# OpenRobotLab/EmbodiedScan

Measured on NVIDIA H100. Metric: training scans/sec mv-3ddet 20-view (ResNet-50/16 + MinkResNet34, 480x640, 100k pts), higher is better.
Workload: dtype bf16

## Files before the change

### embodiedscan_b200/_ffi.py

```python
import ctypes
import os

import torch

_HERE = os.path.dirname(os.path.abspath(__file__))
LIB_PATH = os.path.join(_HERE, 'libesb200.so')

_CT = {'p': ctypes.c_void_p, 'q': ctypes.c_longlong, 'i': ctypes.c_int, 'f': ctypes.c_float, 'z': ctypes.c_size_t}

SIGNATURES = {
    'esb_last_error': ('', 'p'),
    'esb_voxelize_points': ('pqiifpp', 'i'),
    'esb_hash_capacity': ('q', 'q'),
    'esb_coord_unique_workspace_bytes': ('q', 'z'),
    'esb_coord_unique': ('pqippqppppzp', 'i'),
    'esb_hash_build': ('pqppqp', 'i'),
    'esb_hash_lookup': ('pqppqpp', 'i'),
    'esb_interp_features': ('pqppqpiiipp', 'i'),
    'esb_kernel_map': ('pqpippqpp', 'i'),
    'esb_kernel_map_transpose': ('piqqpp', 'i'),
    'esb_kmap_pairs_workspace_bytes': ('iq', 'z'),
    'esb_kmap_pairs': ('piqppppzp', 'i'),
    'esb_generative_children': ('pqipp', 'i'),
    'esb_spconv_fwd': ('ppppqiiiiip', 'i'),
    'esb_spconv_wgrad': ('ppppppqiiiip', 'i'),
    'esb_kmap_tile_masks': ('piqpp', 'i'),
    'esb_spconv_tc_fwd': ('pppppqiiiip', 'i'),
    'esb_spconv_tc_wgrad': ('ppppppqiiip', 'i'),
    'esb_maxpool_fwd': ('ppppqiiip', 'i'),
    'esb_maxpool_bwd': ('pppqiip', 'i'),
    'esb_norm_fwd': ('ppppiqiippfppfipppip', 'i'),
    'esb_batchnorm_fwd_fused': ('ppqippfppfippip', 'i'),
    'esb_norm_apply': ('pppqippppipip', 'i'),
    'esb_norm_bwd': ('pppppiqiipppippppiip', 'i'),
    'esb_bias_act_fwd': ('ppppqiiip', 'i'),
    'esb_act_bwd': ('pppqiip', 'i'),
    'esb_gather2_rows': ('ppqpppqiip', 'i'),
    'esb_conv2d_tma_fwd': ('ppppp' + 'iiiiiiiiii' + 'p', 'i'),
    'esb_conv2d_tma_wgrad': ('ppp' + 'iiiiiiiii' + 'p', 'i'),
    'esb_conv2d_tma_dgrad': ('ppp' + 'iiiiiiiii' + 'p', 'i'),
    'esb_conv3d_tma_fwd': ('ppppp' + 'iiiiiiiiii' + 'p', 'i'),
    'esb_conv3d_tma_dgrad': ('ppp' + 'iiiiiiiii' + 'p', 'i'),
    'esb_conv3d_tma_wgrad': ('ppp' + 'iiiiiiiii' + 'p', 'i'),
    'esb_stem7x7_tc': ('pppp' + 'iiii' + 'p', 'i'),
    'esb_conv2d_direct_fwd': ('ppppp' + 'iiiiiiiiiii' + 'p', 'i'),
    'esb_conv2d_direct_dgrad': ('ppp' + 'iiiiiiiiii' + 'p', 'i'),
    'esb_conv2d_direct_wgrad': ('ppp' + 'iiiiiiiiii' + 'p', 'i'),
    'esb_maxpool2d_nhwc': ('pp' + 'iiiiiiii' + 'p', 'i'),
    'esb_attn_fwd': ('pppppp' + 'iiii' + 'f' + 'p', 'i'),
    'esb_attn_bwd': ('ppppppppppp' + 'iiii' + 'f' + 'p', 'i'),
    'esb_paint_meta_bytes': ('', 'i'),
    'esb_paint_fwd': ('pppqfppipiiiffppip', 'i'),
    'esb_paint_bwd': ('pppqfppipiiiffpip', 'i'),
    'esb_fcaf3d_targets_workspace_bytes': ('iii', 'z'),
    'esb_fcaf3d_targets': ('ppiippppp' + 'iiiii' + 'pppp' + 'pzp', 'i'),
    'esb_focal_loss_fwd': ('ppqiffppip', 'i'),
    'esb_focal_loss_bwd': ('ppqiffpppip', 'i'),
    'esb_bbox_cd_loss': ('pppppippp', 'i'),
    'esb_nms_bev_segmented': ('ppiifipp', 'i'),
    'esb_iou_bev_pairwise': ('pipiipp', 'i'),
    'esb_box3d_overlap': ('pipippp', 'i'),
    'esb_hungarian_batch': ('ppiiippp', 'i'),
    'esb_img_normalize': ('piiiiippiipip', 'i'),
    'esb_unproject_depth_workspace_bytes': ('iii', 'z'),
    'esb_unproject_depth': ('piiifpppppzp', 'i'),
    'esb_grad_clip_coef': ('pqffpp', 'i'),
    'esb_adamw_step': ('pppppqfffffifpp', 'i'),
    'esb_cast_f32_to_bf16': ('ppqp', 'i'),
}

_lib = None

KERNELS_PER_CALL = {
    'esb_voxelize_points': 1, 'esb_coord_unique': 6, 'esb_hash_build': 2, 'esb_hash_lookup': 1, 'esb_kernel_map': 1,
    'esb_kernel_map_transpose': 2, 'esb_kmap_pairs': 3, 'esb_generative_children': 1, 'esb_spconv_fwd': 1,
    'esb_spconv_wgrad': 1, 'esb_maxpool_fwd': 1, 'esb_maxpool_bwd': 1, 'esb_norm_fwd': 5, 'esb_norm_apply': 1,
    'esb_norm_bwd': 2, 'esb_batchnorm_fwd_fused': 2, 'esb_paint_fwd': 1, 'esb_paint_bwd': 1, 'esb_fcaf3d_targets': 5,
    'esb_focal_loss_fwd': 1, 'esb_focal_loss_bwd': 1, 'esb_nms_bev_segmented': 1, 'esb_iou_bev_pairwise': 1,
    'esb_img_normalize': 1, 'esb_unproject_depth': 3, 'esb_grad_clip_coef': 2, 'esb_adamw_step': 1,
    'esb_cast_f32_to_bf16': 1, 'esb_spconv_tc_fwd': 1, 'esb_spconv_tc_wgrad': 1, 'esb_kmap_tile_masks': 1,
}
launch_counter = {'kernels': 0, 'calls': 0, 'by_name': {}}


def exported_symbols():
    return list(SIGNATURES.keys())


def lib():
    global _lib
    if _lib is None:
        if not os.path.exists(LIB_PATH):
            raise RuntimeError(
                f'{LIB_PATH} is missing: run `python -c "import __graft_entry__ as g; g.build()"` '
                '(esb200 has no CPU fallback)')
        handle = ctypes.CDLL(LIB_PATH)
        for name, (args, ret) in SIGNATURES.items():
            fn = getattr(handle, name)
            fn.argtypes = [_CT[c] for c in args]
            fn.restype = _CT[ret]
        _lib = handle
    return _lib


def last_error():
    p = lib().esb_last_error()
    return ctypes.cast(p, ctypes.c_char_p).value.decode() if p else ''


def ptr(t):
    if t is None:
        return None
    return t.data_ptr()


def stream():
    return torch._C._cuda_getCurrentRawStream(torch._C._cuda_getDevice())


def call(name, *args):
    launch_counter['calls'] += 1
    launch_counter['kernels'] += KERNELS_PER_CALL.get(name, 1)
    launch_counter['by_name'][name] = launch_counter['by_name'].get(name, 0) + 1
    rc = getattr(lib(), name)(*args)
    if rc != 0:
        raise RuntimeError(f'{name} failed ({rc}): {last_error()}')


def query(name, *args):
    return getattr(lib(), name)(*args)


def dtype_code(dtype):
    if dtype == torch.float32:
        return 0
    if dtype == torch.bfloat16:
        return 1
    raise TypeError(f'esb200 kernels take float32 or bfloat16 features, got {dtype}')
```

### embodiedscan_b200/csrc/attn_tc.cu

```cuda
#include "tc_common.cuh"

using namespace esb_tc;

namespace {

constexpr int AT_D = 32;
constexpr int AT_CONS = 256;
constexpr int AT_THREADS = AT_CONS + 32;
constexpr float LOG2E = 1.4426950408889634f;

__device__ __forceinline__ uint32_t swz128(uint32_t row, uint32_t piece) { return row * 128u + ((piece ^ (row & 7u)) << 4); }
__device__ __forceinline__ uint32_t tile_off(int row, int col) {
  return (uint32_t)(col >> 6) * 16384u + swz128((uint32_t)row, (uint32_t)((col & 63) >> 3)) + (uint32_t)(col & 7) * 2u;
}

__global__ void __launch_bounds__(AT_THREADS, 1)
attn_fwd_kernel(const __grid_constant__ CUtensorMap tmq, const __grid_constant__ CUtensorMap tmk,
                const __grid_constant__ CUtensorMap tmv, const unsigned char* __restrict__ key_pad,
                __nv_bfloat16* __restrict__ o, float* __restrict__ lse, int H, int Lq, int Lk, float scale) {
  extern __shared__ __align__(1024) uint8_t smem_raw[];
  uint8_t* smem = (uint8_t*)(((uintptr_t)smem_raw + 1023) & ~(uintptr_t)1023);
  uint8_t* q_s = smem;
  uint8_t* k_s = smem + 8192;
  uint8_t* v_s = smem + 8192 * 3;
  uint8_t* p_s = smem + 8192 * 5;
  uint64_t* bars = (uint64_t*)(p_s + 32768);
  uint64_t *q_full = bars, *kv_full = bars + 1, *kv_empty = bars + 3;

  const int warp = threadIdx.x >> 5, lane = threadIdx.x & 31;
  const int bh = blockIdx.y, b = bh / H;
  const int q0 = blockIdx.x * 128;
  const int n_kt = (Lk + 127) / 128;

  if (threadIdx.x == 0) {
    mbar_init(q_full, 1);
    for (int s = 0; s < 2; ++s) { mbar_init(&kv_full[s], 1); mbar_init(&kv_empty[s], AT_CONS / 32); }
    asm volatile("fence.mbarrier_init.release.cluster;" ::: "memory");
    tma_prefetch_desc(&tmq); tma_prefetch_desc(&tmk); tma_prefetch_desc(&tmv);
  }
  __syncthreads();

  if (threadIdx.x >= AT_CONS) {
    if (lane == 0) {
      mbar_expect_tx(q_full, 8192);
      tma_load_2d(&tmq, q_full, smem_u32(q_s), 0, bh * Lq + q0);
      for (int j = 0; j < n_kt; ++j) {
        const int s = j & 1;
        mbar_wait(&kv_empty[s], ((j >> 1) & 1) ^ 1);
        mbar_expect_tx(&kv_full[s], 16384);
        tma_load_2d(&tmk, &kv_full[s], smem_u32(k_s + s * 8192), 0, bh * Lk + j * 128);
        tma_load_2d(&tmv, &kv_full[s], smem_u32(v_s + s * 8192), 0, bh * Lk + j * 128);
      }
    }
    return;
  }
  const int wg = threadIdx.x >> 7;
  const int ra = wg * 64 + 16 * (warp & 3) + (lane >> 2);
  const int cq = 2 * (lane & 3);
  const float sc2 = scale * LOG2E;
  float m[2] = {-INFINITY, -INFINITY}, l[2] = {0.f, 0.f};
  float acc[AT_D / 2], sacc[64], oacc[AT_D / 2];
#pragma unroll
  for (int e = 0; e < AT_D / 2; ++e) acc[e] = 0.f;
  mbar_wait(q_full, 0);
  const uint32_t qa = smem_u32(q_s) + wg * 4096, pa = smem_u32(p_s) + wg * 8192;
  for (int j = 0; j < n_kt; ++j) {
    const int s = j & 1;
    mbar_wait(&kv_full[s], (j >> 1) & 1);
    const uint32_t ka = smem_u32(k_s + s * 8192), va = smem_u32(v_s + s * 8192);
    wgmma_fence();
#pragma unroll
    for (int kk = 0; kk < 2; ++kk)
      wgmma_bf16<128, 0, 0>(sacc, make_desc_sw(qa + kk * 32, 16, 512, SW64), make_desc_sw(ka + kk * 32, 16, 512, SW64), kk > 0);
    wgmma_commit();
    wgmma_wait<0>();
    acc_fence<64>(sacc);
    uint32_t dead = 0;
#pragma unroll
    for (int jb = 0; jb < 16; ++jb)
#pragma unroll
      for (int u = 0; u < 2; ++u) {
        const int kj = j * 128 + 8 * jb + cq + u;
        if (kj >= Lk || (key_pad != nullptr && key_pad[(long long)b * Lk + kj])) dead |= 1u << (2 * jb + u);
      }
    float alpha[2], m_use[2];
#pragma unroll
    for (int h = 0; h < 2; ++h) {
      float mx = m[h];
#pragma unroll
      for (int jb = 0; jb < 16; ++jb)
#pragma unroll
        for (int u = 0; u < 2; ++u)
          if (!((dead >> (2 * jb + u)) & 1)) mx = fmaxf(mx, sacc[4 * jb + 2 * h + u] * sc2);
      mx = fmaxf(mx, __shfl_xor_sync(0xffffffffu, mx, 1));
      mx = fmaxf(mx, __shfl_xor_sync(0xffffffffu, mx, 2));
      m_use[h] = mx == -INFINITY ? 0.f : mx;
      alpha[h] = exp2f(m[h] - m_use[h]);
      m[h] = mx;
    }
    float rs[2] = {0.f, 0.f};
#pragma unroll
    for (int jb = 0; jb < 16; ++jb)
#pragma unroll
      for (int h = 0; h < 2; ++h) {
        const float p0 = ((dead >> (2 * jb)) & 1) ? 0.f : exp2f(sacc[4 * jb + 2 * h] * sc2 - m_use[h]);
        const float p1 = ((dead >> (2 * jb + 1)) & 1) ? 0.f : exp2f(sacc[4 * jb + 2 * h + 1] * sc2 - m_use[h]);
        rs[h] += p0 + p1;
        *reinterpret_cast<uint32_t*>(p_s + tile_off(ra + 8 * h, 8 * jb + cq)) = pack_bf16(__float_as_uint(p0), __float_as_uint(p1));
      }
#pragma unroll
    for (int h = 0; h < 2; ++h) l[h] = l[h] * alpha[h] + rs[h];
    fence_proxy_async();
    asm volatile("bar.sync %0, 128;" ::"r"(1 + wg) : "memory");
    wgmma_fence();
#pragma unroll
    for (int kk = 0; kk < 8; ++kk)
      wgmma_bf16<AT_D, 0, 1>(oacc, make_desc_sw(pa + (kk >> 2) * 16384 + (kk & 3) * 32, 16, 1024, SW128),
                             make_desc_sw(va + kk * 1024, 2048, 512, SW64), kk > 0);
    wgmma_commit();
    wgmma_wait<0>();
    acc_fence<AT_D / 2>(oacc);
    if (lane == 0) mbar_arrive(&kv_empty[s]);
#pragma unroll
    for (int e = 0; e < AT_D / 2; ++e) acc[e] = acc[e] * alpha[(e >> 1) & 1] + oacc[e];
  }
#pragma unroll
  for (int h = 0; h < 2; ++h) {
    l[h] += __shfl_xor_sync(0xffffffffu, l[h], 1);
    l[h] += __shfl_xor_sync(0xffffffffu, l[h], 2);
    const int qi = q0 + ra + 8 * h;
    if (qi < Lq) {
      const float inv = l[h] > 0.f ? 1.f / l[h] : 0.f;
      __nv_bfloat16* dst = o + ((long long)bh * Lq + qi) * AT_D;
#pragma unroll
      for (int jb = 0; jb < AT_D / 8; ++jb)
        *reinterpret_cast<uint32_t*>(dst + 8 * jb + cq) =
            pack_bf16(__float_as_uint(acc[4 * jb + 2 * h] * inv), __float_as_uint(acc[4 * jb + 2 * h + 1] * inv));
      if ((lane & 3) == 0) lse[(long long)bh * Lq + qi] = l[h] > 0.f ? (m[h] + log2f(l[h])) * 0.6931471805599453f : -INFINITY;
    }
  }
}

__global__ void attn_delta_kernel(const __nv_bfloat16* __restrict__ o, const __nv_bfloat16* __restrict__ dout,
                                  float* __restrict__ delta, long long rows) {
  const long long i = (long long)blockIdx.x * blockDim.x + threadIdx.x;
  if (i >= rows) return;
  float s = 0.f;
  const uint4* a = reinterpret_cast<const uint4*>(o + i * AT_D);
  const uint4* g = reinterpret_cast<const uint4*>(dout + i * AT_D);
#pragma unroll
  for (int h = 0; h < 4; ++h) {
    const uint4 x = a[h], y = g[h];
    const __nv_bfloat162* xp = reinterpret_cast<const __nv_bfloat162*>(&x);
    const __nv_bfloat162* yp = reinterpret_cast<const __nv_bfloat162*>(&y);
#pragma unroll
    for (int e = 0; e < 4; ++e) {
      const float2 xf = __bfloat1622float2(xp[e]), yf = __bfloat1622float2(yp[e]);
      s = fmaf(xf.x, yf.x, s);
      s = fmaf(xf.y, yf.y, s);
    }
  }
  delta[i] = s;
}

__global__ void __launch_bounds__(AT_THREADS, 1)
attn_bwd_kernel(const __grid_constant__ CUtensorMap tmq, const __grid_constant__ CUtensorMap tmk,
                const __grid_constant__ CUtensorMap tmv, const __grid_constant__ CUtensorMap tmdo,
                const unsigned char* __restrict__ key_pad, const float* __restrict__ lse, const float* __restrict__ delta,
                float* __restrict__ dq, __nv_bfloat16* __restrict__ dk, __nv_bfloat16* __restrict__ dv, int H, int Lq, int Lk,
                float scale) {
  extern __shared__ __align__(1024) uint8_t smem_raw[];
  uint8_t* smem = (uint8_t*)(((uintptr_t)smem_raw + 1023) & ~(uintptr_t)1023);
  uint8_t* k_s = smem;
  uint8_t* v_s = smem + 8192;
  uint8_t* q_s = smem + 16384;
  uint8_t* do_s = smem + 32768;
  uint8_t* pt_s = smem + 49152;
  uint8_t* ds_s = smem + 49152 + 32768;
  float* lse2_all = (float*)(smem + 49152 + 65536);
  float* delta_all = lse2_all + 256;
  uint64_t* bars = (uint64_t*)(delta_all + 256);
  uint64_t *kv_full = bars, *qd_full = bars + 1, *qd_empty = bars + 3;

  const int warp = threadIdx.x >> 5, lane = threadIdx.x & 31;
  const int bh = blockIdx.y, b = bh / H;
  const int k0 = blockIdx.x * 128;
  const int n_qt = (Lq + 127) / 128;

  if (threadIdx.x == 0) {
    mbar_init(kv_full, 1);
    for (int s = 0; s < 2; ++s) { mbar_init(&qd_full[s], 1); mbar_init(&qd_empty[s], AT_CONS / 32); }
    asm volatile("fence.mbarrier_init.release.cluster;" ::: "memory");
    tma_prefetch_desc(&tmq); tma_prefetch_desc(&tmk); tma_prefetch_desc(&tmv); tma_prefetch_desc(&tmdo);
  }
  __syncthreads();

  if (threadIdx.x >= AT_CONS) {
    if (lane == 0) {
      mbar_expect_tx(kv_full, 16384);
      tma_load_2d(&tmk, kv_full, smem_u32(k_s), 0, bh * Lk + k0);
      tma_load_2d(&tmv, kv_full, smem_u32(v_s), 0, bh * Lk + k0);
      for (int i = 0; i < n_qt; ++i) {
        const int s = i & 1;
        mbar_wait(&qd_empty[s], ((i >> 1) & 1) ^ 1);
        mbar_expect_tx(&qd_full[s], 16384);
        tma_load_2d(&tmq, &qd_full[s], smem_u32(q_s + s * 8192), 0, bh * Lq + i * 128);
        tma_load_2d(&tmdo, &qd_full[s], smem_u32(do_s + s * 8192), 0, bh * Lq + i * 128);
      }
    }
    return;
  }
  const int t = threadIdx.x, wg = t >> 7;
  const int ra = wg * 64 + 16 * (warp & 3) + (lane >> 2);
  const int cq = 2 * (lane & 3);
  bool k_dead[2];
#pragma unroll
  for (int h = 0; h < 2; ++h) {
    const int kj = k0 + ra + 8 * h;
    k_dead[h] = kj >= Lk || (key_pad != nullptr && key_pad[(long long)b * Lk + kj]);
  }
  const float sc2 = scale * LOG2E;
  float sacc[64], pacc[64], dvacc[AT_D / 2], dkacc[AT_D / 2], dqacc[AT_D / 2];
  const uint32_t ka = smem_u32(k_s), va = smem_u32(v_s), pa = smem_u32(pt_s), sa = smem_u32(ds_s);
  mbar_wait(kv_full, 0);
  for (int i = 0; i < n_qt; ++i) {
    const int s = i & 1;
    float* lse2_s = lse2_all + (i & 1) * 128;
    float* delta_s = delta_all + (i & 1) * 128;
    if (t < 128) {
      const int qi = i * 128 + t;
      lse2_s[t] = qi < Lq ? lse[(long long)bh * Lq + qi] * LOG2E : INFINITY;
      delta_s[t] = qi < Lq ? delta[(long long)bh * Lq + qi] : 0.f;
    }
    asm volatile("bar.sync 1, %0;" ::"n"(AT_CONS) : "memory");
    mbar_wait(&qd_full[s], (i >> 1) & 1);
    const uint32_t qa = smem_u32(q_s + s * 8192), da = smem_u32(do_s + s * 8192);
    wgmma_fence();
#pragma unroll
    for (int kk = 0; kk < 2; ++kk)
      wgmma_bf16<128, 0, 0>(sacc, make_desc_sw(ka + wg * 4096 + kk * 32, 16, 512, SW64), make_desc_sw(qa + kk * 32, 16, 512, SW64),
                            kk > 0);
#pragma unroll
    for (int kk = 0; kk < 2; ++kk)
      wgmma_bf16<128, 0, 0>(pacc, make_desc_sw(va + wg * 4096 + kk * 32, 16, 512, SW64), make_desc_sw(da + kk * 32, 16, 512, SW64),
                            kk > 0);
    wgmma_commit();
    wgmma_wait<0>();
    acc_fence<64>(sacc);
    acc_fence<64>(pacc);
#pragma unroll
    for (int jb = 0; jb < 16; ++jb)
#pragma unroll
      for (int h = 0; h < 2; ++h) {
        float p[2], ds[2];
#pragma unroll
        for (int u = 0; u < 2; ++u) {
          const int c = 8 * jb + cq + u, e = 4 * jb + 2 * h + u;
          const float ex = k_dead[h] ? 0.f : exp2f(sacc[e] * sc2 - lse2_s[c]);
          p[u] = ex;
          ds[u] = ex * (pacc[e] - delta_s[c]) * scale;
        }
        const uint32_t off = tile_off(ra + 8 * h, 8 * jb + cq);
        *reinterpret_cast<uint32_t*>(pt_s + off) = pack_bf16(__float_as_uint(p[0]), __float_as_uint(p[1]));
        *reinterpret_cast<uint32_t*>(ds_s + off) = pack_bf16(__float_as_uint(ds[0]), __float_as_uint(ds[1]));
      }
    fence_proxy_async();
    asm volatile("bar.sync 1, %0;" ::"n"(AT_CONS) : "memory");
    wgmma_fence();
#pragma unroll
    for (int kk = 0; kk < 8; ++kk) {
      const uint32_t a_off = wg * 8192 + (kk >> 2) * 16384 + (kk & 3) * 32;
      wgmma_bf16<AT_D, 0, 1>(dvacc, make_desc_sw(pa + a_off, 16, 1024, SW128), make_desc_sw(da + kk * 1024, 2048, 512, SW64),
                             i > 0 || kk > 0);
      wgmma_bf16<AT_D, 0, 1>(dkacc, make_desc_sw(sa + a_off, 16, 1024, SW128), make_desc_sw(qa + kk * 1024, 2048, 512, SW64),
                             i > 0 || kk > 0);
    }
#pragma unroll
    for (int kk = 0; kk < 8; ++kk)
      wgmma_bf16<AT_D, 1, 1>(dqacc, make_desc_sw(sa + wg * 16384 + kk * 2048, 16384, 1024, SW128),
                             make_desc_sw(ka + kk * 1024, 2048, 512, SW64), kk > 0);
    wgmma_commit();
    wgmma_wait<0>();
    acc_fence<AT_D / 2>(dvacc);
    acc_fence<AT_D / 2>(dkacc);
    acc_fence<AT_D / 2>(dqacc);
    if (lane == 0) mbar_arrive(&qd_empty[s]);
#pragma unroll
    for (int h = 0; h < 2; ++h) {
      const int qi = i * 128 + ra + 8 * h;
      if (qi < Lq) {
        float* dst = dq + (((long long)blockIdx.x * gridDim.y + bh) * Lq + qi) * AT_D;
#pragma unroll
        for (int jb = 0; jb < AT_D / 8; ++jb)
          *reinterpret_cast<float2*>(dst + 8 * jb + cq) = make_float2(dqacc[4 * jb + 2 * h], dqacc[4 * jb + 2 * h + 1]);
      }
    }
  }
#pragma unroll
  for (int h = 0; h < 2; ++h) {
    const int kj = k0 + ra + 8 * h;
    if (kj < Lk) {
      __nv_bfloat16* pv = dv + ((long long)bh * Lk + kj) * AT_D;
      __nv_bfloat16* pk = dk + ((long long)bh * Lk + kj) * AT_D;
#pragma unroll
      for (int jb = 0; jb < AT_D / 8; ++jb) {
        *reinterpret_cast<uint32_t*>(pv + 8 * jb + cq) =
            pack_bf16(__float_as_uint(dvacc[4 * jb + 2 * h]), __float_as_uint(dvacc[4 * jb + 2 * h + 1]));
        *reinterpret_cast<uint32_t*>(pk + 8 * jb + cq) =
            pack_bf16(__float_as_uint(dkacc[4 * jb + 2 * h]), __float_as_uint(dkacc[4 * jb + 2 * h + 1]));
      }
    }
  }
}

int rows32_map(CUtensorMap* tm, const void* base, long long rows) {
  unsigned long long dims[2] = {AT_D, (unsigned long long)(rows > 0 ? rows : 1)};
  unsigned long long str[1] = {AT_D * 2};
  unsigned box[2] = {AT_D, 128};
  return esb_tma_encode(tm, base, 2, dims, str, box, nullptr, 64);
}

}

extern "C" int esb_attn_fwd(const void* q, const void* k, const void* v, const unsigned char* key_pad, void* o, float* lse, int B,
                            int H, int Lq, int Lk, float scale, void* stream_) {
  ESB_CHECK_ARG(B > 0 && H > 0 && Lq > 0 && Lk > 0, "esb_attn_fwd: empty problem");
  CUtensorMap tmq, tmk, tmv;
  int rc = rows32_map(&tmq, q, (long long)B * H * Lq);
  if (rc == ESB_OK) rc = rows32_map(&tmk, k, (long long)B * H * Lk);
  if (rc == ESB_OK) rc = rows32_map(&tmv, v, (long long)B * H * Lk);
  if (rc != ESB_OK) return rc;
  const size_t smem = 8192 * 5 + 32768 + 8 * 8 + 1024;
  cudaError_t e = cudaFuncSetAttribute(attn_fwd_kernel, cudaFuncAttributeMaxDynamicSharedMemorySize, (int)smem);
  if (e != cudaSuccess) { esb_set_error("esb_attn_fwd: smem attr: %s", cudaGetErrorString(e)); return ESB_ECUDA; }
  dim3 grid((Lq + 127) / 128, B * H);
  attn_fwd_kernel<<<grid, AT_THREADS, smem, (cudaStream_t)stream_>>>(tmq, tmk, tmv, key_pad, (__nv_bfloat16*)o, lse, H, Lq, Lk, scale);
  ESB_CUDA_LAUNCH_CHECK("attn_fwd_kernel");
  return ESB_OK;
}

extern "C" int esb_attn_bwd(const void* q, const void* k, const void* v, const unsigned char* key_pad, const void* o,
                            const void* dout, const float* lse, float* delta, float* dq, void* dk, void* dv, int B, int H, int Lq,
                            int Lk, float scale, void* stream_) {
  cudaStream_t stream = (cudaStream_t)stream_;
  ESB_CHECK_ARG(B > 0 && H > 0 && Lq > 0 && Lk > 0, "esb_attn_bwd: empty problem");
  CUtensorMap tmq, tmk, tmv, tmdo;
  int rc = rows32_map(&tmq, q, (long long)B * H * Lq);
  if (rc == ESB_OK) rc = rows32_map(&tmk, k, (long long)B * H * Lk);
  if (rc == ESB_OK) rc = rows32_map(&tmv, v, (long long)B * H * Lk);
  if (rc == ESB_OK) rc = rows32_map(&tmdo, dout, (long long)B * H * Lq);
  if (rc != ESB_OK) return rc;
  const long long rows = (long long)B * H * Lq;
  attn_delta_kernel<<<esb_div_up(rows, 256), 256, 0, stream>>>((const __nv_bfloat16*)o, (const __nv_bfloat16*)dout, delta, rows);
  ESB_CUDA_LAUNCH_CHECK("attn_delta_kernel");
  const size_t smem = 49152 + 65536 + 2048 + 8 * 8 + 1024;
  cudaError_t e = cudaFuncSetAttribute(attn_bwd_kernel, cudaFuncAttributeMaxDynamicSharedMemorySize, (int)smem);
  if (e != cudaSuccess) { esb_set_error("esb_attn_bwd: smem attr: %s", cudaGetErrorString(e)); return ESB_ECUDA; }
  dim3 grid((Lk + 127) / 128, B * H);
  const long long width = rows * AT_D;
  float* part = nullptr;
  ESB_CUDA_CALL(esb_scratch_alloc((void**)&part, sizeof(float) * grid.x * width, stream));
  attn_bwd_kernel<<<grid, AT_THREADS, smem, stream>>>(tmq, tmk, tmv, tmdo, key_pad, lse, delta, part, (__nv_bfloat16*)dk,
                                                      (__nv_bfloat16*)dv, H, Lq, Lk, scale);
  ESB_CUDA_LAUNCH_CHECK("attn_bwd_kernel");
  rc = esb_sum_partial_rows(part, (int)grid.x, width, dq, 1, stream);
  ESB_CUDA_CALL(esb_scratch_free(part, stream));
  return rc;
}
```

### embodiedscan_b200/csrc/common.cuh

```cuda
#pragma once
#include <cuda_runtime.h>
#include <cuda_bf16.h>
#include <stdint.h>
#include <stdio.h>
#include <stdarg.h>
#include "../../include/esb200.h"

void esb_set_error(const char* fmt, ...);

#define ESB_CHECK_ARG(cond, ...)                      \
  do {                                                \
    if (!(cond)) {                                    \
      esb_set_error(__VA_ARGS__);                     \
      return ESB_EINVAL;                              \
    }                                                 \
  } while (0)

#define ESB_CUDA_LAUNCH_CHECK(name)                                        \
  do {                                                                     \
    cudaError_t _e = cudaPeekAtLastError();                                \
    if (_e != cudaSuccess) {                                               \
      esb_set_error("%s: CUDA error %s", name, cudaGetErrorString(_e));    \
      return ESB_ECUDA;                                                    \
    }                                                                      \
  } while (0)

#define ESB_CUDA_CALL(expr)                                                \
  do {                                                                     \
    cudaError_t _e = (expr);                                               \
    if (_e != cudaSuccess) {                                               \
      esb_set_error("%s: CUDA error %s", #expr, cudaGetErrorString(_e));   \
      return ESB_ECUDA;                                                    \
    }                                                                      \
  } while (0)

static inline int esb_div_up(long long a, long long b) { return (int)((a + b - 1) / b); }
static inline size_t esb_align(size_t x, size_t a = 256) { return (x + a - 1) / a * a; }
cudaError_t esb_scratch_alloc(void** p, size_t bytes, cudaStream_t s);
cudaError_t esb_scratch_free(void* p, cudaStream_t s);
int esb_sum_partial_rows(const float* part, int n_parts, long long width, float* out, int accumulate, cudaStream_t s);

int esb_sm_count();


#define ESB_EMPTY_KEY 0xFFFFFFFFFFFFFFFFull
#define ESB_COORD_BIAS 32768

__host__ __device__ __forceinline__ uint64_t esb_pack_key(int b, int x, int y, int z) {
  return ((uint64_t)(uint16_t)b << 48) | ((uint64_t)(uint16_t)(x + ESB_COORD_BIAS) << 32) |
         ((uint64_t)(uint16_t)(y + ESB_COORD_BIAS) << 16) | (uint64_t)(uint16_t)(z + ESB_COORD_BIAS);
}
__host__ __device__ __forceinline__ bool esb_coord_in_range(int b, int x, int y, int z) {
  return b >= 0 && b < 65535 && x >= -ESB_COORD_BIAS && x < ESB_COORD_BIAS && y >= -ESB_COORD_BIAS &&
         y < ESB_COORD_BIAS && z >= -ESB_COORD_BIAS && z < ESB_COORD_BIAS;
}
__host__ __device__ __forceinline__ uint32_t esb_hash64(uint64_t k) {
  k ^= k >> 33;
  k *= 0xff51afd7ed558ccdull;
  k ^= k >> 33;
  k *= 0xc4ceb9fe1a85ec53ull;
  k ^= k >> 33;
  return (uint32_t)k;
}

#ifdef __CUDACC__
__device__ __forceinline__ int esb_floor_div(int a, int d) {
  int q = a / d;
  return (a % d != 0 && a < 0) ? q - 1 : q;
}

__device__ __forceinline__ int esb_hash_find(const unsigned long long* __restrict__ keys,
                                             const int* __restrict__ vals, uint32_t mask, uint64_t key) {
  uint32_t slot = esb_hash64(key) & mask;
  for (uint32_t probe = 0; probe <= mask; ++probe) {
    unsigned long long k = keys[slot];
    if (k == key) return vals[slot];
    if (k == ESB_EMPTY_KEY) return -1;
    slot = (slot + 1) & mask;
  }
  return -1;
}

template <typename T>
__device__ __forceinline__ float esb_to_float(T v);
template <>
__device__ __forceinline__ float esb_to_float<float>(float v) { return v; }
template <>
__device__ __forceinline__ float esb_to_float<__nv_bfloat16>(__nv_bfloat16 v) { return __bfloat162float(v); }

template <typename T>
__device__ __forceinline__ T esb_from_float(float v);
template <>
__device__ __forceinline__ float esb_from_float<float>(float v) { return v; }
template <>
__device__ __forceinline__ __nv_bfloat16 esb_from_float<__nv_bfloat16>(float v) { return __float2bfloat16_rn(v); }

__device__ __forceinline__ float esb_warp_sum(float v) {
#pragma unroll
  for (int o = 16; o > 0; o >>= 1) v += __shfl_xor_sync(0xffffffffu, v, o);
  return v;
}
__device__ __forceinline__ float esb_warp_max(float v) {
#pragma unroll
  for (int o = 16; o > 0; o >>= 1) v = fmaxf(v, __shfl_xor_sync(0xffffffffu, v, o));
  return v;
}
#endif
```

### embodiedscan_b200/csrc/conv_tma.cu

```cuda
#include "tc_common.cuh"

using namespace esb_tc;

namespace {

struct ConvGeom {
  int tiles_w, tiles_h, tiles_d, tiles_n, n_blocks;
  int TW, TH, TD, TN;
  int Wo, Ho, Do, N;
  int stride;
  int cin, bc, nchunk, group;
  int cout, relu;
  int stages;
  int ntaps;
  short tap_dx[27], tap_dy[27], tap_dz[27], tap_w[27];
};

constexpr int EPI_THREADS = 128;
constexpr int NCONS = 256;
constexpr int PROD0 = NCONS, EPI0 = NCONS + 32;
constexpr int THREADS = EPI0 + EPI_THREADS;

__device__ __forceinline__ uint32_t swz(uint32_t off, uint32_t mask) { return off ^ (((off >> 7) & mask) << 4); }

// ... 399 lines not shown

extern "C" int esb_conv2d_tma_dgrad(const void* dy, const void* w_ohwi, void* dx, int n_img, int H, int W, int cin, int cout,
                                    int kh, int kw, int stride, int pad, void* stream_) {
  return conv_dgrad_any("esb_conv2d_tma_dgrad", dy, w_ohwi, dx, n_img, 1, H, W, cin, cout, 1, kh, kw, stride, pad,
                        (cudaStream_t)stream_);
}

extern "C" int esb_conv3d_tma_dgrad(const void* dy, const void* w_odhwi, void* dx, int n, int D, int H, int W, int cin, int cout,
                                    int k, int stride, int pad, void* stream_) {
  return conv_dgrad_any("esb_conv3d_tma_dgrad", dy, w_odhwi, dx, n, D, H, W, cin, cout, k, k, k, stride, pad,
                        (cudaStream_t)stream_);
}

namespace {

constexpr int ST_TW = 16, ST_TH = 8;
constexpr int ST_PW = 112, ST_PH = 2 * ST_TH + 5;
constexpr int ST_K = 147, ST_KPAD = 160;

__global__ void __launch_bounds__(128)
stem7x7_tc_kernel(const __nv_bfloat16* __restrict__ x, const __nv_bfloat16* __restrict__ w, const float* __restrict__ bias,
                  __nv_bfloat16* __restrict__ y, int n_img, int H, int W, int Ho, int Wo, int relu) {
  extern __shared__ __align__(1024) uint8_t smem_raw[];
  uint8_t* smem = (uint8_t*)(((uintptr_t)smem_raw + 1023) & ~(uintptr_t)1023);
  uint8_t* a_tile = smem;
  uint8_t* b_tile = smem + 3 * 16384;
  __nv_bfloat16* patch = (__nv_bfloat16*)(b_tile + 3 * 2048);
  float* acc_img = reinterpret_cast<float*>(a_tile);
  constexpr int PITCH = 20;

  const int t = threadIdx.x;
  for (int i = t; i < 16 * 24; i += 128) {
    const int n = i / 24, j = i - n * 24;
    uint32_t v[4] = {0u, 0u, 0u, 0u};
    __nv_bfloat16* vp = reinterpret_cast<__nv_bfloat16*>(v);
    for (int e = 0; e < 8; ++e) {
      const int k = j * 8 + e;
      if (k < ST_K) vp[e] = w[n * ST_K + k];
    }
    const int c = j >> 3, jj = j & 7;
    *reinterpret_cast<uint4*>(b_tile + c * 2048 + n * 128 + ((jj ^ (n & 7)) << 4)) = make_uint4(v[0], v[1], v[2], v[3]);
  }
  __syncthreads();

  const int tiles_w = (Wo + ST_TW - 1) / ST_TW, tiles_h = (Ho + ST_TH - 1) / ST_TH;
  const int n_tiles = tiles_w * tiles_h * n_img;
  const int tx = t & 15, ty = t >> 4;
  for (int tile = blockIdx.x; tile < n_tiles; tile += gridDim.x) {
    int r = tile;
    const int twi = r % tiles_w; r /= tiles_w;
    const int thi = r % tiles_h;
    const int img = r / tiles_h;
    const int ox0 = twi * ST_TW, oy0 = thi * ST_TH;
    const int g0 = (2 * ox0 - 3) * 3 - 1;
    const __nv_bfloat16* ximg = x + (long long)img * H * W * 3;
    for (int i = t; i < ST_PH * (ST_PW / 2); i += 128) {
      const int pr = i / (ST_PW / 2), pw = i - pr * (ST_PW / 2);
      const int iy = 2 * oy0 - 3 + pr, g = g0 + 2 * pw;
      uint32_t v = 0u;
      if (iy >= 0 && iy < H && g >= 0 && g + 1 < W * 3) v = *reinterpret_cast<const uint32_t*>(ximg + (long long)iy * W * 3 + g);
      reinterpret_cast<uint32_t*>(patch)[pr * (ST_PW / 2) + pw] = v;
    }
    __syncthreads();
    {
      const __nv_bfloat16* base = patch + (2 * ty) * ST_PW + 6 * tx + 1;
      const uint32_t row_off = (uint32_t)((t >> 3) * 1024 + (t & 7) * 128);
#pragma unroll
      for (int j = 0; j < ST_KPAD / 8; ++j) {
        uint32_t v[4];
#pragma unroll
        for (int h = 0; h < 4; ++h) {
          const int k0 = j * 8 + 2 * h, k1 = k0 + 1;
          const uint32_t lo = k0 < ST_K ? (uint32_t)__bfloat16_as_ushort(base[(k0 / 21) * ST_PW + (k0 % 21)]) : 0u;
          const uint32_t hi = k1 < ST_K ? (uint32_t)__bfloat16_as_ushort(base[(k1 / 21) * ST_PW + (k1 % 21)]) : 0u;
          v[h] = lo | (hi << 16);
        }
        const int c = j >> 3, jj = j & 7;
        *reinterpret_cast<uint4*>(a_tile + c * 16384 + row_off + ((jj ^ (t & 7)) << 4)) = make_uint4(v[0], v[1], v[2], v[3]);
      }
    }
    fence_proxy_async();
    __syncthreads();
    {
      const uint32_t a_addr = smem_u32(a_tile), b_addr = smem_u32(b_tile);
      float acc[2][8];
      wgmma_fence();
#pragma unroll
      for (int h = 0; h < 2; ++h)
#pragma unroll
        for (int kk = 0; kk < ST_KPAD / 16; ++kk)
          wgmma_bf16<16, 0, 0>(acc[h], make_desc(a_addr + h * 8192 + (kk >> 2) * 16384 + (kk & 3) * 32, 16, 1024),
                               make_desc(b_addr + (kk >> 2) * 2048 + (kk & 3) * 32, 16, 1024), kk > 0);
      wgmma_commit();
      wgmma_wait<0>();
      acc_fence<8>(acc[0]);
      acc_fence<8>(acc[1]);
      __syncthreads();
      acc_store<16>(acc[0], acc_img, PITCH, 0, t);
      acc_store<16>(acc[1], acc_img, PITCH, 64, t);
      __syncthreads();
    }
    uint32_t v[32];
    img_ld<16>(acc_img, PITCH, t, 0, v);
    const int ox = ox0 + tx, oy = oy0 + ty;
    if (ox < Wo && oy < Ho) {
      uint32_t o[8];
#pragma unroll
      for (int h = 0; h < 8; ++h) {
        float f0 = __uint_as_float(v[2 * h]) + bias[2 * h], f1 = __uint_as_float(v[2 * h + 1]) + bias[2 * h + 1];
        if (relu) { f0 = fmaxf(f0, 0.f); f1 = fmaxf(f1, 0.f); }
        o[h] = pack_bf16(__float_as_uint(f0), __float_as_uint(f1));
      }
      uint4* dst = reinterpret_cast<uint4*>(y + (((long long)img * Ho + oy) * Wo + ox) * 16);
      dst[0] = make_uint4(o[0], o[1], o[2], o[3]);
      dst[1] = make_uint4(o[4], o[5], o[6], o[7]);
    }
    __syncthreads();
  }
}

}

extern "C" int esb_stem7x7_tc(const void* x, const void* w_ohwi, const float* bias, void* y, int n_img, int H, int W, int relu,
                              void* stream_) {
  ESB_CHECK_ARG(n_img >= 0 && H > 0 && W > 0 && (W * 3) % 2 == 0, "esb_stem7x7_tc: W*3 must be even (4-byte patch loads)");
  ESB_CHECK_ARG(bias != nullptr, "esb_stem7x7_tc: bias (16 fp32) is required");
  if (n_img == 0) return ESB_OK;
  const int Ho = (H + 6 - 7) / 2 + 1, Wo = (W + 6 - 7) / 2 + 1;
  const size_t smem = 3 * 16384 + 3 * 2048 + ((ST_PH * ST_PW * 2 + 15) & ~15) + 1024;
  cudaError_t e = cudaFuncSetAttribute(stem7x7_tc_kernel, cudaFuncAttributeMaxDynamicSharedMemorySize, (int)smem);
  if (e != cudaSuccess) { esb_set_error("esb_stem7x7_tc: smem attr: %s", cudaGetErrorString(e)); return ESB_ECUDA; }
  const long long n_tiles = (long long)esb_div_up(Wo, ST_TW) * esb_div_up(Ho, ST_TH) * n_img;
  long long grid = (long long)esb_sm_count() * 3;
  if (grid > n_tiles) grid = n_tiles;
  stem7x7_tc_kernel<<<(unsigned)grid, 128, smem, (cudaStream_t)stream_>>>(
      (const __nv_bfloat16*)x, (const __nv_bfloat16*)w_ohwi, bias, (__nv_bfloat16*)y, n_img, H, W, Ho, Wo, relu);
  ESB_CUDA_LAUNCH_CHECK("stem7x7_tc_kernel");
  return ESB_OK;
}

namespace {

struct WgradGeom {
  int tiles_w, tiles_h, tiles_d, tiles_n;
  int TW, TH, TD, TN;
  int kd, kh, kw, stride, sd, pad, pd;
  int cin, cout, aw, atoms_per_slice, chunks_per_tap;
  int stages, tiles_per_cta;
};

template <int N_TILE>
__global__ void __launch_bounds__(THREADS, 1)
conv_tma_wgrad_kernel(const __grid_constant__ CUtensorMap tmx, const __grid_constant__ CUtensorMap tmdy,
                      float* __restrict__ dw, const WgradGeom g) {
  constexpr int NA = N_TILE < 64 ? N_TILE : 64;
  constexpr int A_BYTES = 64 * 256;
  constexpr int B_BYTES = 64 * N_TILE * 2;
  constexpr int STAGE_BYTES = A_BYTES + B_BYTES;
  constexpr int PITCH = N_TILE + 4;
  extern __shared__ __align__(1024) uint8_t smem_raw[];
  uint8_t* smem = (uint8_t*)(((uintptr_t)smem_raw + 1023) & ~(uintptr_t)1023);
  const int STAGES = g.stages;
  uint64_t* full_bar = (uint64_t*)(smem + STAGES * STAGE_BYTES);
  uint64_t* empty_bar = full_bar + STAGES;
  uint64_t* accum_bar = empty_bar + STAGES;
  float* img = reinterpret_cast<float*>(smem);

  const int lane = threadIdx.x & 31;
  const int taps = g.kd * g.kh * g.kw;
  const int n_tiles = g.tiles_w * g.tiles_h * g.tiles_d * g.tiles_n;
  const int t_beg = blockIdx.x * g.tiles_per_cta;
  const int t_end = min(n_tiles, t_beg + g.tiles_per_cta);
  if (t_beg >= n_tiles) return;
  const int total = t_end - t_beg;
  const int slice = blockIdx.y, co0 = blockIdx.z * N_TILE;
  const int awb = g.aw * 2;
  const int atom0 = slice * g.atoms_per_slice;
  const int n_atoms_total = taps * g.chunks_per_tap;
  const int n_valid = min(g.atoms_per_slice, n_atoms_total - atom0);
  const uint32_t a_atom_bytes = 64u * awb;

  if (threadIdx.x == 0) {
    for (int s = 0; s < STAGES; ++s) {
      mbar_init(&full_bar[s], 1);
      mbar_init(&empty_bar[s], NCONS / 32);
    }
    mbar_init(accum_bar, NCONS);
    asm volatile("fence.mbarrier_init.release.cluster;" ::: "memory");
    tma_prefetch_desc(&tmx);
    tma_prefetch_desc(&tmdy);
  }
  __syncthreads();

  if (threadIdx.x >= PROD0 && threadIdx.x < EPI0) {
    if (lane == 0) {
      for (int it = 0; it < total; ++it) {
        int t = t_beg + it;
        const int tw = t % g.tiles_w; t /= g.tiles_w;
        const int th = t % g.tiles_h; t /= g.tiles_h;
        const int td = t % g.tiles_d; t /= g.tiles_d;
        const int ox0 = tw * g.TW, oy0 = th * g.TH, oz0 = td * g.TD, img0 = t * g.TN;
        const int s = it % STAGES;
        mbar_wait(&empty_bar[s], ((it / STAGES) & 1) ^ 1);
        mbar_expect_tx(&full_bar[s], (uint32_t)n_valid * a_atom_bytes + B_BYTES);
        const uint32_t a_base = smem_u32(smem + s * STAGE_BYTES);
        const uint32_t b_base = a_base + A_BYTES;
        for (int a = 0; a < n_valid; ++a) {
          const int ga = atom0 + a;
          const int tap = ga / g.chunks_per_tap, ch0 = (ga - tap * g.chunks_per_tap) * g.aw;
          const int kz = tap / (g.kh * g.kw), kr = tap - kz * (g.kh * g.kw);
          const int ky = kr / g.kw, kx = kr - ky * g.kw;
          tma_load_5d(&tmx, &full_bar[s], a_base + a * a_atom_bytes, ch0, ox0 * g.stride - g.pad + kx, oy0 * g.stride - g.pad + ky,
                      oz0 * g.sd - g.pd + kz, img0);
        }
#pragma unroll
        for (int b = 0; b < N_TILE / NA; ++b)
          tma_load_5d(&tmdy, &full_bar[s], b_base + b * (64 * NA * 2), co0 + b * NA, ox0, oy0, oz0, img0);
      }
    }
  } else if (threadIdx.x < NCONS) {
    const int wg = threadIdx.x >> 7;
    const uint32_t a_layout = mma_layout_of(awb), b_layout = mma_layout_of(NA * 2);
    float acc[N_TILE / 2];
    for (int it = 0; it < total; ++it) {
      const int s = it % STAGES;
      mbar_wait(&full_bar[s], (it / STAGES) & 1);
      const uint32_t a_addr = smem_u32(smem + s * STAGE_BYTES) + wg * (64 / g.aw) * a_atom_bytes;
      const uint32_t b_addr = smem_u32(smem + s * STAGE_BYTES) + A_BYTES;
      wgmma_fence();
#pragma unroll
      for (int kk = 0; kk < 4; ++kk)
        wgmma_bf16<N_TILE, 1, 1>(acc, make_desc_sw(a_addr + kk * 16 * awb, a_atom_bytes, 8 * awb, a_layout),
                                 make_desc_sw(b_addr + kk * 16 * (NA * 2), 64 * NA * 2, 8 * (NA * 2), b_layout), it > 0 || kk > 0);
      wgmma_commit();
      wgmma_wait<1>();
      if (it > 0 && lane == 0) mbar_arrive(&empty_bar[(it - 1) % STAGES]);
    }
    wgmma_wait<0>();
    acc_fence<N_TILE / 2>(acc);
    asm volatile("bar.sync 2, %0;" ::"n"(NCONS) : "memory");
    acc_store<N_TILE>(acc, img, PITCH, wg * 64, threadIdx.x & 127);
    mbar_arrive(accum_bar);
  } else {
    const int quad = (threadIdx.x - EPI0) >> 5;
    mbar_wait(accum_bar, 0);
    const float* stg = img;
    const int rows_valid = n_valid * g.aw;
    for (int rr = 0; rr < 32; ++rr) {
      const int r = quad * 32 + rr;
      if (r >= rows_valid) break;
      const int ga = atom0 + r / g.aw;
      const int tap = ga / g.chunks_per_tap, ch = (ga - tap * g.chunks_per_tap) * g.aw + (r % g.aw);
      float* dwrow = dw + (((long long)blockIdx.x * g.kd * g.kh * g.kw + tap) * g.cin + ch) * g.cout + co0;
      for (int c = lane * 4; c < N_TILE; c += 128)
        *reinterpret_cast<float4*>(dwrow + c) = *reinterpret_cast<const float4*>(stg + r * PITCH + c);
    }
  }
}

template <int N_TILE>
int launch_wgrad_tma(const CUtensorMap& tmx, const CUtensorMap& tmdy, float* dw, WgradGeom g, int slices, int n_blocks,
                     cudaStream_t stream) {
  constexpr int STAGE_BYTES = 64 * 256 + 64 * N_TILE * 2;
  int stages = (100 * 1024) / STAGE_BYTES;
  const int need = (128 * (N_TILE + 4) * 4 + STAGE_BYTES - 1) / STAGE_BYTES;
  stages = stages < need ? need : stages > 6 ? 6 : stages;
  g.stages = stages;
  const size_t smem = (size_t)stages * STAGE_BYTES + (2 * stages + 1) * 8 + 16 + 1024;
  auto kern = conv_tma_wgrad_kernel<N_TILE>;
  cudaError_t e = cudaFuncSetAttribute(kern, cudaFuncAttributeMaxDynamicSharedMemorySize, (int)smem);
  if (e != cudaSuccess) { esb_set_error("conv_tma_wgrad: smem attr: %s", cudaGetErrorString(e)); return ESB_ECUDA; }
  const long long n_tiles = (long long)g.tiles_w * g.tiles_h * g.tiles_d * g.tiles_n;
  long long splits = (2LL * esb_sm_count() + (long long)slices * n_blocks - 1) / ((long long)slices * n_blocks);
  if (splits > n_tiles) splits = n_tiles;
  if (splits < 1) splits = 1;
  g.tiles_per_cta = (int)((n_tiles + splits - 1) / splits);
  dim3 grid((unsigned)((n_tiles + g.tiles_per_cta - 1) / g.tiles_per_cta), slices, n_blocks);
  const long long width = (long long)g.kd * g.kh * g.kw * g.cin * g.cout;
  float* part = nullptr;
  ESB_CUDA_CALL(esb_scratch_alloc((void**)&part, sizeof(float) * grid.x * width, stream));
  kern<<<grid, THREADS, smem, stream>>>(tmx, tmdy, part, g);
  int rc = esb_sum_partial_rows(part, (int)grid.x, width, dw, 1, stream);
  ESB_CUDA_CALL(esb_scratch_free(part, stream));
  return rc;
}

}

namespace {

int conv_wgrad_any(const char* who, const void* x, const void* dy, float* dw_t, int n_img, int D, int H, int W, int cin, int cout,
                   int kd, int kh, int kw, int stride, int pad, cudaStream_t stream) {
  if (!(channels_ok(cin) && channels_ok(cout))) { esb_set_error("%s: channels must be 16, 32 or a multiple of 64", who); return ESB_EINVAL; }
  if (!(kd >= 1 && kh >= 1 && kw >= 1 && stride >= 1 && stride <= 8 && pad >= 0)) { esb_set_error("%s: bad filter geometry", who); return ESB_EINVAL; }
  const int pd = kd > 1 ? pad : 0, sd = D > 1 ? stride : 1;
  const int Do = (D + 2 * pd - kd) / sd + 1, Ho = (H + 2 * pad - kh) / stride + 1, Wo = (W + 2 * pad - kw) / stride + 1;
  if (Do <= 0 || Ho <= 0 || Wo <= 0) { esb_set_error("%s: empty output", who); return ESB_EINVAL; }
  if (n_img == 0) return ESB_OK;
  WgradGeom g{};
  g.kd = kd; g.kh = kh; g.kw = kw; g.stride = stride; g.sd = sd; g.pad = pad; g.pd = pd; g.cin = cin; g.cout = cout;
  g.aw = cin < 64 ? cin : 64;
  g.atoms_per_slice = 128 / g.aw;
  g.chunks_per_tap = cin / g.aw;
  double best = -1.0;
  for (int tw = 1; tw <= 64; tw *= 2)
    for (int th = 1; tw * th <= 64; th *= 2)
      for (int td = 1; tw * th * td <= 64; td *= 2) {
        const int tn = 64 / (tw * th * td);
        if (tn > 1 && (tw < Wo || th < Ho || td < Do)) continue;
        if (td > 1 && Do == 1) continue;
        const double tiles = (double)esb_div_up(Wo, tw) * esb_div_up(Ho, th) * esb_div_up(Do, td) * esb_div_up(n_img, tn);
        const double eff = (double)Wo * Ho * Do * n_img / (tiles * 64.0) + 1e-6 * tw;
        if (eff > best) { best = eff; g.TW = tw; g.TH = th; g.TD = td; g.TN = tn; }
      }
  g.tiles_w = esb_div_up(Wo, g.TW); g.tiles_h = esb_div_up(Ho, g.TH); g.tiles_d = esb_div_up(Do, g.TD);
  g.tiles_n = esb_div_up(n_img, g.TN);
  const int n_tile = cout >= 128 ? 128 : cout;
  const int n_blocks = cout / n_tile;
  const int slices = esb_div_up(kd * kh * kw * g.chunks_per_tap, g.atoms_per_slice);
  CUtensorMap tmx, tmdy;
  {
    unsigned long long dims[5] = {(unsigned long long)cin, (unsigned long long)W, (unsigned long long)H, (unsigned long long)D,
                                  (unsigned long long)n_img};
    unsigned long long str[4] = {(unsigned long long)cin * 2, (unsigned long long)W * cin * 2, (unsigned long long)H * W * cin * 2,
                                 (unsigned long long)D * H * W * cin * 2};
    unsigned box[5] = {(unsigned)g.aw, (unsigned)((g.TW - 1) * stride + 1), (unsigned)((g.TH - 1) * stride + 1),
                       (unsigned)((g.TD - 1) * sd + 1), (unsigned)g.TN};
    unsigned es[5] = {1, (unsigned)stride, (unsigned)stride, (unsigned)sd, 1};
    int rc = esb_tma_encode(&tmx, x, 5, dims, str, box, es, g.aw * 2);
    if (rc != ESB_OK) return rc;
  }
  {
    const int na = n_tile < 64 ? n_tile : 64;
    unsigned long long dims[5] = {(unsigned long long)cout, (unsigned long long)Wo, (unsigned long long)Ho, (unsigned long long)Do,
                                  (unsigned long long)n_img};
    unsigned long long str[4] = {(unsigned long long)cout * 2, (unsigned long long)Wo * cout * 2,
                                 (unsigned long long)Ho * Wo * cout * 2, (unsigned long long)Do * Ho * Wo * cout * 2};
    unsigned box[5] = {(unsigned)na, (unsigned)g.TW, (unsigned)g.TH, (unsigned)g.TD, (unsigned)g.TN};
    int rc = esb_tma_encode(&tmdy, dy, 5, dims, str, box, nullptr, na * 2);
    if (rc != ESB_OK) return rc;
  }
  int rc;
  switch (n_tile) {
    case 16: rc = launch_wgrad_tma<16>(tmx, tmdy, dw_t, g, slices, n_blocks, stream); break;
    case 32: rc = launch_wgrad_tma<32>(tmx, tmdy, dw_t, g, slices, n_blocks, stream); break;
    case 64: rc = launch_wgrad_tma<64>(tmx, tmdy, dw_t, g, slices, n_blocks, stream); break;
    case 128: rc = launch_wgrad_tma<128>(tmx, tmdy, dw_t, g, slices, n_blocks, stream); break;
    default: esb_set_error("%s: unsupported Cout %d", who, cout); return ESB_EINVAL;
  }
  if (rc != ESB_OK) return rc;
  ESB_CUDA_LAUNCH_CHECK("conv_tma_wgrad_kernel");
  return ESB_OK;
}

}

extern "C" int esb_conv2d_tma_wgrad(const void* x, const void* dy, float* dw_t, int n_img, int H, int W, int cin, int cout,
                                    int kh, int kw, int stride, int pad, void* stream_) {
  return conv_wgrad_any("esb_conv2d_tma_wgrad", x, dy, dw_t, n_img, 1, H, W, cin, cout, 1, kh, kw, stride, pad,
                        (cudaStream_t)stream_);
}

extern "C" int esb_conv3d_tma_wgrad(const void* x, const void* dy, float* dw_t, int n, int D, int H, int W, int cin, int cout, int k,
                                    int stride, int pad, void* stream_) {
  return conv_wgrad_any("esb_conv3d_tma_wgrad", x, dy, dw_t, n, D, H, W, cin, cout, k, k, k, stride, pad, (cudaStream_t)stream_);
}
```

### embodiedscan_b200/csrc/head.cu

```cuda
#include "common.cuh"

namespace {

struct FaceDist { float d[6]; };

__device__ __forceinline__ FaceDist face_distances(const float* __restrict__ box, const float* __restrict__ R, float px,
                                                   float py, float pz) {
  float sx = __fsub_rn(px, box[0]), sy = __fsub_rn(py, box[1]), sz = __fsub_rn(pz, box[2]);
  float rx = __fadd_rn(__fadd_rn(__fmul_rn(sx, R[0]), __fmul_rn(sy, R[1])), __fmul_rn(sz, R[2]));
  float ry = __fadd_rn(__fadd_rn(__fmul_rn(sx, R[3]), __fmul_rn(sy, R[4])), __fmul_rn(sz, R[5]));
  float rz = __fadd_rn(__fadd_rn(__fmul_rn(sx, R[6]), __fmul_rn(sy, R[7])), __fmul_rn(sz, R[8]));
  float cx = __fadd_rn(box[0], rx), cy = __fadd_rn(box[1], ry), cz = __fadd_rn(box[2], rz);
  float hx = __fdiv_rn(box[3], 2.f), hy = __fdiv_rn(box[4], 2.f), hz = __fdiv_rn(box[5], 2.f);
  FaceDist f;
  f.d[0] = __fadd_rn(__fsub_rn(cx, box[0]), hx);
  f.d[1] = __fsub_rn(__fadd_rn(box[0], hx), cx);
  f.d[2] = __fadd_rn(__fsub_rn(cy, box[1]), hy);
  f.d[3] = __fsub_rn(__fadd_rn(box[1], hy), cy);
  f.d[4] = __fadd_rn(__fsub_rn(cz, box[2]), hz);
  f.d[5] = __fsub_rn(__fadd_rn(box[2], hz), cz);
  return f;
}
__device__ __forceinline__ bool inside_box(const FaceDist& f) {
  float m = fminf(fminf(fminf(f.d[0], f.d[1]), fminf(f.d[2], f.d[3])), fminf(f.d[4], f.d[5]));
// ... 34 lines not shown
  int b = blockIdx.x * blockDim.x + threadIdx.x;
  if (b >= Ng) return;
  int first = -1;
  for (int l = 0; l < L; ++l)
    if (counts[l * Ng + b] < assign_thr) { first = l; break; }
  int lower_index = (first < 0 ? 0 : first) - 1;
  if (lower_index < 0) lower_index = 0;
  best[b] = first < 0 ? L - 1 : lower_index;
}

constexpr int TOPK_CAP = 4096;

constexpr int TOPK_THREADS = 1024;

__global__ void __launch_bounds__(TOPK_THREADS)
topk_threshold_kernel(const float* __restrict__ pts, const int* __restrict__ level_off, const int* __restrict__ pt_batch,
                      const int* __restrict__ n_pts_of_scan, const float* __restrict__ boxes,
                      const float* __restrict__ rneg, const int* __restrict__ box_off, int B,
                      const int* __restrict__ best, int kth, float* __restrict__ top) {
  __shared__ float c_val[TOPK_CAP];
  __shared__ int c_idx[TOPK_CAP];
  __shared__ float s_val[TOPK_THREADS];
  __shared__ int s_idx[TOPK_THREADS];
  __shared__ float prev_v;
  __shared__ int prev_i;
  __shared__ int n_cand;
  const int g = blockIdx.x, tid = threadIdx.x;
  int scan = 0;
  while (scan + 1 < B && g >= box_off[scan + 1]) ++scan;
  const int lvl = best[g];
  const int p_beg = level_off[lvl], p_end = level_off[lvl + 1];
  const float* box = boxes + g * 9;
  const float* R = rneg + g * 9;
  const int k_eff = min(kth, n_pts_of_scan[scan]);
  if (tid == 0) { prev_v = INFINITY; prev_i = -1; n_cand = 0; }
  __syncthreads();
  for (int p = p_beg + tid; p < p_end; p += TOPK_THREADS) {
    if (pt_batch && pt_batch[p] != scan) continue;
    FaceDist f = face_distances(box, R, pts[3 * p], pts[3 * p + 1], pts[3 * p + 2]);
    if (!inside_box(f)) continue;
    int slot = atomicAdd(&n_cand, 1);
    if (slot < TOPK_CAP) { c_val[slot] = centerness_of(f); c_idx[slot] = p; }
  }
  __syncthreads();
  const int nc = n_cand;
  if (nc < k_eff) {
    if (tid == 0) top[g] = -1.f;
    return;
  }
  const bool in_smem = nc <= TOPK_CAP;
  for (int round = 0; round < k_eff; ++round) {
    float bv = -INFINITY;
    int bi = -1;
    const float pv = prev_v;
    const int pi = prev_i;
    if (in_smem) {
      for (int c = tid; c < nc; c += TOPK_THREADS) {
        float v = c_val[c];
        int p = c_idx[c];
        bool after = (v < pv) || (v == pv && p > pi);
        if (after && (bi < 0 || v > bv || (v == bv && p < bi))) { bv = v; bi = p; }
      }
    } else {
      for (int p = p_beg + tid; p < p_end; p += TOPK_THREADS) {
        if (pt_batch && pt_batch[p] != scan) continue;
        FaceDist f = face_distances(box, R, pts[3 * p], pts[3 * p + 1], pts[3 * p + 2]);
        if (!inside_box(f)) continue;
        float v = centerness_of(f);
        bool after = (v < pv) || (v == pv && p > pi);
        if (after && (bi < 0 || v > bv || (v == bv && p < bi))) { bv = v; bi = p; }
      }
    }
    s_val[tid] = bv;
    s_idx[tid] = bi;
    __syncthreads();
    for (int s = TOPK_THREADS / 2; s > 0; s >>= 1) {
      if (tid < s) {
        float ov = s_val[tid + s];
        int oi = s_idx[tid + s];
        bool take = oi >= 0 && (s_idx[tid] < 0 || ov > s_val[tid] || (ov == s_val[tid] && oi < s_idx[tid]));
        if (take) { s_val[tid] = ov; s_idx[tid] = oi; }
      }
      __syncthreads();
    }
    if (tid == 0) { prev_v = s_val[0]; prev_i = s_idx[0]; }
    __syncthreads();
  }
  if (tid == 0) top[g] = prev_v;
}

__global__ void count_scan_points_kernel(const int* __restrict__ pt_batch, int Np, int B, int* __restrict__ n_pts_of_scan) {
  __shared__ int hist[64];
  for (int i = threadIdx.x; i < 64; i += blockDim.x) hist[i] = 0;
  __syncthreads();
  int p = blockIdx.x * blockDim.x + threadIdx.x;
  if (p < Np) {
    int b = pt_batch ? pt_batch[p] : 0;
    if (b < 64) atomicAdd(&hist[b], 1); else atomicAdd(&n_pts_of_scan[b], 1);
  }
  __syncthreads();
  for (int i = threadIdx.x; i < min(B, 64); i += blockDim.x)
    if (hist[i]) atomicAdd(&n_pts_of_scan[i], hist[i]);
}

__global__ void assign_kernel(const float* __restrict__ pts, const int* __restrict__ level_off, int L, int Np,
                              const int* __restrict__ pt_batch, const float* __restrict__ boxes,
                              const float* __restrict__ rneg, const long long* __restrict__ labels,
                              const int* __restrict__ box_off, const int* __restrict__ best,
                              const float* __restrict__ top, float* __restrict__ center_t, float* __restrict__ bbox_t,
                              long long* __restrict__ cls_t, int* __restrict__ box_idx) {
  int p = blockIdx.x * blockDim.x + threadIdx.x;
  if (p >= Np) return;
  const int lvl = level_of(level_off, L, p);
  const int b = pt_batch ? pt_batch[p] : 0;
  const int g_beg = box_off[b], g_end = box_off[b + 1];
  float px = pts[3 * p], py = pts[3 * p + 1], pz = pts[3 * p + 2];
  const float FMAX = 1e8f;
  float min_vol = FMAX;
  int min_ind = g_beg;
  float cent_sel = -1.f, cent0 = -1.f;
  for (int g = g_beg; g < g_end; ++g) {
    const float* box = boxes + g * 9;
    FaceDist f = face_distances(box, rneg + g * 9, px, py, pz);
    bool in = inside_box(f);
    bool lv = best[g] == lvl;
    float c = (in && lv) ? centerness_of(f) : -1.f;
    if (g == g_beg) cent0 = c;
    if (in && lv && c > top[g]) {
      float vol = __fmul_rn(__fmul_rn(box[3], box[4]), box[5]);
      if (vol < min_vol) { min_vol = vol; min_ind = g; cent_sel = c; }
    }
  }
  bool pos = min_vol < FMAX;
  if (g_end == g_beg) {
    center_t[p] = 0.f;
#pragma unroll
    for (int j = 0; j < 9; ++j) bbox_t[p * 9 + j] = 0.f;
    cls_t[p] = -1;
    if (box_idx) box_idx[p] = -1;
    return;
  }
  center_t[p] = pos ? cent_sel : cent0;
#pragma unroll
  for (int j = 0; j < 9; ++j) bbox_t[p * 9 + j] = boxes[min_ind * 9 + j];
  cls_t[p] = pos ? labels[min_ind] : -1;
  if (box_idx) box_idx[p] = pos ? min_ind : -1;
}

__device__ __forceinline__ float sigmoidf(float x) { return 1.f / (1.f + expf(-x)); }
__device__ __forceinline__ float pow_gamma(float x, float gamma) { return gamma == 2.f ? x * x : powf(x, gamma); }

template <typename T>
__global__ void focal_fwd_kernel(const T* __restrict__ logits, const long long* __restrict__ target, long long n, int C,
                                 float gamma, float alpha, const float* __restrict__ row_w, float* __restrict__ loss_sum) {
  long long t = blockIdx.x * (long long)blockDim.x + threadIdx.x;
  float l = 0.f;
  if (t < n * C) {
    long long r = t / C;
    int c = (int)(t - r * C);
    float p = sigmoidf(esb_to_float<T>(logits[t]));
    if (target[r] == c)
      l = -alpha * pow_gamma(1.f - p, gamma) * logf(fmaxf(p, 1.17549435e-38f));
    else
      l = -(1.f - alpha) * pow_gamma(p, gamma) * logf(fmaxf(1.f - p, 1.17549435e-38f));
    if (row_w) l *= row_w[r];
  }
  l = esb_warp_sum(l);
  __shared__ float red[8];
  if ((threadIdx.x & 31) == 0) red[threadIdx.x >> 5] = l;
  __syncthreads();
  if (threadIdx.x == 0) {
    float s = 0.f;
    for (int i = 0; i < (int)(blockDim.x >> 5); ++i) s += red[i];
    loss_sum[blockIdx.x] = s;
  }
}

template <typename T>
__global__ void focal_bwd_kernel(const T* __restrict__ logits, const long long* __restrict__ target, long long n, int C,
                                 float gamma, float alpha, const float* __restrict__ row_w,
                                 const float* __restrict__ scale, T* __restrict__ grad) {
  long long t = blockIdx.x * (long long)blockDim.x + threadIdx.x;
  if (t >= n * C) return;
  long long r = t / C;
  int c = (int)(t - r * C);
  float p = sigmoidf(esb_to_float<T>(logits[t]));
  float g;
  if (target[r] == c)
    g = -alpha * pow_gamma(1.f - p, gamma) * (1.f - p - gamma * p * logf(fmaxf(p, 1.17549435e-38f)));
  else
    g = -(1.f - alpha) * pow_gamma(p, gamma) * (gamma * (1.f - p) * logf(fmaxf(1.f - p, 1.17549435e-38f)) - p);
  grad[t] = esb_from_float<T>(g * scale[0] * (row_w ? row_w[r] : 1.f));
}


struct Dual {
  float v;
  float d[12];
};
__device__ __forceinline__ Dual dconst(float v) {
  Dual r; r.v = v;
#pragma unroll
  for (int i = 0; i < 12; ++i) r.d[i] = 0.f;
  return r;
}
__device__ __forceinline__ Dual dvar(float v, int idx) { Dual r = dconst(v); r.d[idx] = 1.f; return r; }
__device__ __forceinline__ Dual operator+(const Dual& a, const Dual& b) {
  Dual r; r.v = a.v + b.v;
#pragma unroll
  for (int i = 0; i < 12; ++i) r.d[i] = a.d[i] + b.d[i];
  return r;
}
__device__ __forceinline__ Dual operator-(const Dual& a, const Dual& b) {
  Dual r; r.v = a.v - b.v;
#pragma unroll
  for (int i = 0; i < 12; ++i) r.d[i] = a.d[i] - b.d[i];
  return r;
}
__device__ __forceinline__ Dual operator-(const Dual& a) {
  Dual r; r.v = -a.v;
#pragma unroll
  for (int i = 0; i < 12; ++i) r.d[i] = -a.d[i];
  return r;
}
__device__ __forceinline__ Dual operator*(const Dual& a, const Dual& b) {
  Dual r; r.v = a.v * b.v;
#pragma unroll
  for (int i = 0; i < 12; ++i) r.d[i] = a.d[i] * b.v + a.v * b.d[i];
  return r;
}
__device__ __forceinline__ Dual operator*(const Dual& a, float s) {
  Dual r; r.v = a.v * s;
#pragma unroll
  for (int i = 0; i < 12; ++i) r.d[i] = a.d[i] * s;
  return r;
}
__device__ __forceinline__ Dual operator+(const Dual& a, float s) { Dual r = a; r.v += s; return r; }
__device__ __forceinline__ Dual operator/(const Dual& a, const Dual& b) {
  Dual r;
  float inv = 1.f / b.v;
  r.v = a.v * inv;
#pragma unroll
  for (int i = 0; i < 12; ++i) r.d[i] = (a.d[i] - r.v * b.d[i]) * inv;
  return r;
}
__device__ __forceinline__ Dual dsqrt(const Dual& a) {
  Dual r; r.v = sqrtf(a.v);
  float g = a.v > 0.f ? 0.5f / r.v : 0.f;
#pragma unroll
  for (int i = 0; i < 12; ++i) r.d[i] = a.d[i] * g;
  return r;
}
__device__ __forceinline__ Dual dsin(const Dual& a) { float c = cosf(a.v); Dual r = a * c; r.v = sinf(a.v); return r; }
__device__ __forceinline__ Dual dcos(const Dual& a) { float s = -sinf(a.v); Dual r = a * s; r.v = cosf(a.v); return r; }
__device__ __forceinline__ Dual dasin(const Dual& a) {
  float g = rsqrtf(fmaxf(1.f - a.v * a.v, 1e-12f));
  Dual r = a * g; r.v = asinf(a.v); return r;
}
__device__ __forceinline__ Dual datan2(const Dual& y, const Dual& x) {
  float inv = 1.f / fmaxf(x.v * x.v + y.v * y.v, 1e-30f);
  Dual r; r.v = atan2f(y.v, x.v);
#pragma unroll
  for (int i = 0; i < 12; ++i) r.d[i] = (x.v * y.d[i] - y.v * x.d[i]) * inv;
  return r;
}
struct Dual3 { Dual x, y, z; };
__device__ __forceinline__ Dual3 dcross(const Dual3& a, const Dual3& b) {
  Dual3 r;
  r.x = a.y * b.z - a.z * b.y;
  r.y = a.z * b.x - a.x * b.z;
  r.z = a.x * b.y - a.y * b.x;
  return r;
}
__device__ __forceinline__ Dual3 dnormalize(const Dual3& a) {
  Dual n = dsqrt(a.x * a.x + a.y * a.y + a.z * a.z) + 1e-8f;
  Dual3 r; r.x = a.x / n; r.y = a.y / n; r.z = a.z / n;
  return r;
}
__device__ __forceinline__ void euler_to_mat(const Dual& a, const Dual& b, const Dual& c, Dual m[9]) {
  Dual ca = dcos(a), sa = dsin(a), cb = dcos(b), sb = dsin(b), cc = dcos(c), sc = dsin(c);
  Dual a00 = ca, a01 = -(sa * cb), a02 = sa * sb;
  Dual a10 = sa, a11 = ca * cb, a12 = -(ca * sb);
  Dual a21 = sb, a22 = cb;
  m[0] = a00 * cc - a02 * sc; m[1] = a01; m[2] = a00 * sc + a02 * cc;
  m[3] = a10 * cc - a12 * sc; m[4] = a11; m[5] = a10 * sc + a12 * cc;
  m[6] = -(a22 * sc);         m[7] = a21; m[8] = a22 * cc;
}
__device__ __forceinline__ void euler_to_mat_f(float a, float b, float c, float m[9]) {
  float ca = cosf(a), sa = sinf(a), cb = cosf(b), sb = sinf(b), cc = cosf(c), sc = sinf(c);
  float a00 = ca, a01 = -sa * cb, a02 = sa * sb, a10 = sa, a11 = ca * cb, a12 = -ca * sb, a21 = sb, a22 = cb;
  m[0] = a00 * cc - a02 * sc; m[1] = a01; m[2] = a00 * sc + a02 * cc;
  m[3] = a10 * cc - a12 * sc; m[4] = a11; m[5] = a10 * sc + a12 * cc;
  m[6] = -a22 * sc;           m[7] = a21; m[8] = a22 * cc;
}
__device__ Dual corner_chamfer(const Dual ctr[3], const Dual size[3], const Dual eul[3], const float dst[24]) {
  Dual m[9];
  euler_to_mat(eul[0], eul[1], eul[2], m);
  Dual total = dconst(0.f);
  const float sx[8] = {1, 1, 1, 1, -1, -1, -1, -1}, sy[8] = {1, 1, -1, -1, 1, 1, -1, -1}, sz[8] = {1, -1, 1, -1, 1, -1, 1, -1};
#pragma unroll 1
  for (int i = 0; i < 8; ++i) {
    Dual hx = size[0] * (0.5f * sx[i]), hy = size[1] * (0.5f * sy[i]), hz = size[2] * (0.5f * sz[i]);
    Dual cx = ctr[0] + (hx * m[0] + hy * m[1] + hz * m[2]);
    Dual cy = ctr[1] + (hx * m[3] + hy * m[4] + hz * m[5]);
    Dual cz = ctr[2] + (hx * m[6] + hy * m[7] + hz * m[8]);
    float best = INFINITY;
    int bj = 0;
    for (int j = 0; j < 8; ++j) {
      float dsum = fabsf(cx.v - dst[3 * j]) + fabsf(cy.v - dst[3 * j + 1]) + fabsf(cz.v - dst[3 * j + 2]);
      if (dsum < best) { best = dsum; bj = j; }
    }
    float gx = cx.v > dst[3 * bj] ? 1.f : (cx.v < dst[3 * bj] ? -1.f : 0.f);
    float gy = cy.v > dst[3 * bj + 1] ? 1.f : (cy.v < dst[3 * bj + 1] ? -1.f : 0.f);
    float gz = cz.v > dst[3 * bj + 2] ? 1.f : (cz.v < dst[3 * bj + 2] ? -1.f : 0.f);
    total.v += best;
#pragma unroll
    for (int q = 0; q < 12; ++q) total.d[q] += gx * cx.d[q] + gy * cy.d[q] + gz * cz.d[q];
  }
  return total;
}

__global__ void __launch_bounds__(64)
bbox_cd_loss_kernel(const float* __restrict__ points, const float* __restrict__ bbox_pred, const float* __restrict__ tgt,
                    const float* __restrict__ row_w, float w0, float w1, float w2, float w3, int P,
                    float* __restrict__ loss_out, float* __restrict__ grad) {
  int p = blockIdx.x * blockDim.x + threadIdx.x;
  float lval = 0.f;
  if (p < P) {
    Dual in[12];
#pragma unroll
    for (int i = 0; i < 12; ++i) in[i] = dvar(bbox_pred[p * 12 + i], i);
    Dual3 shift;
    shift.x = (in[1] - in[0]) * 0.5f; shift.y = (in[3] - in[2]) * 0.5f; shift.z = (in[5] - in[4]) * 0.5f;
    Dual3 xr{in[6], in[7], in[8]}, yr{in[9], in[10], in[11]};
    Dual3 y = dnormalize(yr);
    Dual3 z = dnormalize(dcross(xr, y));
    Dual3 x = dcross(y, z);
    Dual eul[3];
    eul[1] = dasin(y.z);
    eul[0] = datan2(-y.x, y.y);
    eul[2] = datan2(-x.z, z.z);
    Dual m[9];
    euler_to_mat(eul[0], eul[1], eul[2], m);
    Dual pc[3], ps[3];
    pc[0] = (shift.x * m[0] + shift.y * m[1] + shift.z * m[2]) + points[3 * p];
    pc[1] = (shift.x * m[3] + shift.y * m[4] + shift.z * m[5]) + points[3 * p + 1];
    pc[2] = (shift.x * m[6] + shift.y * m[7] + shift.z * m[8]) + points[3 * p + 2];
    ps[0] = in[0] + in[1]; ps[1] = in[2] + in[3]; ps[2] = in[4] + in[5];
    const float* t = tgt + p * 9;
    float tm[9], dst[24];
    euler_to_mat_f(t[6], t[7], t[8], tm);
    const float sx[8] = {1, 1, 1, 1, -1, -1, -1, -1}, sy[8] = {1, 1, -1, -1, 1, 1, -1, -1}, sz[8] = {1, -1, 1, -1, 1, -1, 1, -1};
    for (int j = 0; j < 8; ++j) {
      float hx = 0.5f * sx[j] * t[3], hy = 0.5f * sy[j] * t[4], hz = 0.5f * sz[j] * t[5];
      dst[3 * j] = t[0] + hx * tm[0] + hy * tm[1] + hz * tm[2];
      dst[3 * j + 1] = t[1] + hx * tm[3] + hy * tm[4] + hz * tm[5];
      dst[3 * j + 2] = t[2] + hx * tm[6] + hy * tm[7] + hz * tm[8];
    }
    Dual tc[3] = {dconst(t[0]), dconst(t[1]), dconst(t[2])};
    Dual ts[3] = {dconst(t[3]), dconst(t[4]), dconst(t[5])};
    Dual te[3] = {dconst(t[6]), dconst(t[7]), dconst(t[8])};
    Dual acc = dconst(0.f);
    if (w0 != 0.f) acc = acc + corner_chamfer(pc, ts, te, dst) * w0;
    if (w1 != 0.f) acc = acc + corner_chamfer(tc, ps, te, dst) * w1;
    if (w2 != 0.f) acc = acc + corner_chamfer(tc, ts, eul, dst) * w2;
    if (w3 != 0.f) acc = acc + corner_chamfer(pc, ps, eul, dst) * w3;
    float w = row_w[p];
    lval = acc.v * w;
#pragma unroll
    for (int i = 0; i < 12; ++i) grad[p * 12 + i] = acc.d[i] * w;
  }
  lval = esb_warp_sum(lval);
  __shared__ float red[2];
  if ((threadIdx.x & 31) == 0) red[threadIdx.x >> 5] = lval;
  __syncthreads();
  if (threadIdx.x == 0) loss_out[blockIdx.x] = red[0] + red[1];
}

}

extern "C" size_t esb_fcaf3d_targets_workspace_bytes(int L, int NgT, int B) {
  return esb_align((size_t)L * NgT * 4) + 2 * esb_align((size_t)NgT * 4) + esb_align((size_t)B * 4);
}

extern "C" int esb_fcaf3d_targets(const float* points, const int* level_off, int L, int Np, const int* pt_batch,
                                  const float* boxes, const float* rneg, const long long* labels, const int* box_off,
                                  int B, int NgT, int max_ng, int assign_thr, int center_thr, float* center_t,
                                  float* bbox_t, long long* cls_t, int* box_idx, void* ws, size_t ws_bytes,
                                  void* stream_) {
  cudaStream_t stream = (cudaStream_t)stream_;
  ESB_CHECK_ARG(L >= 1 && Np >= 0 && B >= 1 && NgT >= 0, "esb_fcaf3d_targets: bad sizes");
  if (ws_bytes < esb_fcaf3d_targets_workspace_bytes(L, NgT, B)) {
    esb_set_error("esb_fcaf3d_targets: workspace too small");
    return ESB_ENOMEM;
  }
  if (Np == 0) return ESB_OK;
  char* p = (char*)ws;
  int* counts = (int*)p;      p += esb_align((size_t)L * NgT * 4);
  int* best = (int*)p;        p += esb_align((size_t)NgT * 4);
  float* top = (float*)p;     p += esb_align((size_t)NgT * 4);
  int* n_pts_of_scan = (int*)p;
  if (NgT > 0) {
    ESB_CUDA_CALL(cudaMemsetAsync(counts, 0, (size_t)L * NgT * 4, stream));
    ESB_CUDA_CALL(cudaMemsetAsync(n_pts_of_scan, 0, (size_t)B * 4, stream));
    dim3 g1(esb_div_up(Np, 256), max_ng > 0 ? max_ng : 1);
    count_inside_kernel<<<g1, 256, 0, stream>>>(points, level_off, L, Np, pt_batch, boxes, rneg, box_off, NgT, counts);
    count_scan_points_kernel<<<esb_div_up(Np, 1024), 1024, 0, stream>>>(pt_batch, Np, B, n_pts_of_scan);
    best_level_kernel<<<esb_div_up(NgT, 128), 128, 0, stream>>>(counts, L, NgT, assign_thr, best);
    topk_threshold_kernel<<<NgT, TOPK_THREADS, 0, stream>>>(points, level_off, pt_batch, n_pts_of_scan, boxes, rneg, box_off, B,
                                                    best, center_thr + 1, top);
  }
  assign_kernel<<<esb_div_up(Np, 128), 128, 0, stream>>>(points, level_off, L, Np, pt_batch, boxes, rneg, labels, box_off,
                                                          best, top, center_t, bbox_t, cls_t, box_idx);
  ESB_CUDA_LAUNCH_CHECK("esb_fcaf3d_targets");
  return ESB_OK;
}

extern "C" int esb_focal_loss_fwd(const void* logits, const long long* target, long long n, int C, float gamma,
                                  float alpha, const float* row_w, float* loss_sum, int dtype, void* stream) {
  if (n == 0) return ESB_OK;
  cudaStream_t s = (cudaStream_t)stream;
  int grid = esb_div_up(n * C, 256);
  float* part = nullptr;
  ESB_CUDA_CALL(esb_scratch_alloc((void**)&part, (size_t)grid * sizeof(float), s));
  if (dtype == ESB_F32)
    focal_fwd_kernel<float><<<grid, 256, 0, s>>>((const float*)logits, target, n, C, gamma, alpha, row_w, part);
  else
    focal_fwd_kernel<__nv_bfloat16><<<grid, 256, 0, s>>>((const __nv_bfloat16*)logits, target, n, C, gamma, alpha, row_w, part);
  ESB_CUDA_LAUNCH_CHECK("focal_fwd_kernel");
  int rc = esb_sum_partial_rows(part, grid, 1, loss_sum, 1, s);
  ESB_CUDA_CALL(esb_scratch_free(part, s));
  return rc;
}

extern "C" int esb_focal_loss_bwd(const void* logits, const long long* target, long long n, int C, float gamma,
                                  float alpha, const float* row_w, const float* scale_dev, void* grad, int dtype,
                                  void* stream) {
  if (n == 0) return ESB_OK;
  int grid = esb_div_up(n * C, 256);
  if (dtype == ESB_F32)
    focal_bwd_kernel<float><<<grid, 256, 0, (cudaStream_t)stream>>>((const float*)logits, target, n, C, gamma, alpha,
                                                                     row_w, scale_dev, (float*)grad);
  else
    focal_bwd_kernel<__nv_bfloat16><<<grid, 256, 0, (cudaStream_t)stream>>>((const __nv_bfloat16*)logits, target, n, C, gamma,
                                                                             alpha, row_w, scale_dev, (__nv_bfloat16*)grad);
  ESB_CUDA_LAUNCH_CHECK("focal_bwd_kernel");
  return ESB_OK;
}

extern "C" int esb_bbox_cd_loss(const float* points, const float* bbox_pred, const float* targets, const float* row_w,
                                const float* w4_host, int P, float* loss_out, float* grad, void* stream) {
  if (P == 0) return ESB_OK;
  cudaStream_t s = (cudaStream_t)stream;
  const int grid = esb_div_up(P, 64);
  float* part = nullptr;
  ESB_CUDA_CALL(esb_scratch_alloc((void**)&part, (size_t)grid * sizeof(float), s));
  bbox_cd_loss_kernel<<<grid, 64, 0, s>>>(points, bbox_pred, targets, row_w, w4_host[0], w4_host[1], w4_host[2], w4_host[3], P,
                                          part, grad);
  ESB_CUDA_LAUNCH_CHECK("bbox_cd_loss_kernel");
  int rc = esb_sum_partial_rows(part, grid, 1, loss_out, 1, s);
  ESB_CUDA_CALL(esb_scratch_free(part, s));
  return rc;
}
```

### embodiedscan_b200/csrc/optim.cu

```cuda
#include "common.cuh"

namespace {

__global__ void sumsq_kernel(const float* __restrict__ g, long long n, float* __restrict__ out) {
  float acc = 0.f;
  long long stride = (long long)gridDim.x * blockDim.x * 4;
  for (long long i = (blockIdx.x * (long long)blockDim.x + threadIdx.x) * 4; i < n; i += stride) {
    if (i + 3 < n) {
      float4 v = *reinterpret_cast<const float4*>(g + i);
      acc += v.x * v.x + v.y * v.y + v.z * v.z + v.w * v.w;
    } else {
      for (long long j = i; j < n; ++j) acc += g[j] * g[j];
    }
  }
  acc = esb_warp_sum(acc);
  __shared__ float red[32];
  if ((threadIdx.x & 31) == 0) red[threadIdx.x >> 5] = acc;
  __syncthreads();
  if (threadIdx.x < 32) {
    float v = threadIdx.x < (blockDim.x >> 5) ? red[threadIdx.x] : 0.f;
    v = esb_warp_sum(v);
    if (threadIdx.x == 0) out[blockIdx.x] = v;
  }
}

__global__ void clip_coef_kernel(float* state, float max_norm, float world_scale) {
  float norm = sqrtf(state[0]) * world_scale;
  state[1] = norm;
  float coef = max_norm / (norm + 1e-6f);
  state[2] = max_norm > 0.f ? fminf(coef, 1.f) : 1.f;
}

__global__ void adamw_kernel(float* __restrict__ p, const float* __restrict__ g, float* __restrict__ m,
                             float* __restrict__ v, const float* __restrict__ lr_mult, long long n, float lr, float beta1,
                             float beta2, float eps, float wd, float bc1, float bc2_sqrt, float grad_scale,
                             const float* __restrict__ state) {
  long long i = blockIdx.x * (long long)blockDim.x + threadIdx.x;
  if (i >= n) return;
  float scale = grad_scale * (state ? state[2] : 1.f);
  float lm = lr_mult ? lr_mult[i] : 1.f;
  if (lm == 0.f) return;
  float gi = g[i] * scale;
  float mi = beta1 * m[i] + (1.f - beta1) * gi;
  float vi = beta2 * v[i] + (1.f - beta2) * gi * gi;
  m[i] = mi;
  v[i] = vi;
  float l = lr * lm;
  float pi = p[i] * (1.f - l * wd);
  float denom = sqrtf(vi) / bc2_sqrt + eps;
  p[i] = pi - (l / bc1) * (mi / denom);
}

template <typename T>
__global__ void cast_kernel(const float* __restrict__ src, T* __restrict__ dst, long long n) {
  long long i = blockIdx.x * (long long)blockDim.x + threadIdx.x;
  if (i < n) dst[i] = esb_from_float<T>(src[i]);
}

}

extern "C" int esb_grad_clip_coef(const float* grad, long long n, float max_norm, float world_scale, float* state,
                                  void* stream_) {
  cudaStream_t stream = (cudaStream_t)stream_;
  ESB_CUDA_CALL(cudaMemsetAsync(state, 0, 3 * sizeof(float), stream));
  if (n > 0) {
    int grid = esb_div_up(n, 256 * 4 * 8);
    if (grid > esb_sm_count() * 8) grid = esb_sm_count() * 8;
    if (grid < 1) grid = 1;
    float* part = nullptr;
    ESB_CUDA_CALL(esb_scratch_alloc((void**)&part, (size_t)grid * sizeof(float), stream));
    sumsq_kernel<<<grid, 256, 0, stream>>>(grad, n, part);
    int rc = esb_sum_partial_rows(part, grid, 1, state, 0, stream);
    ESB_CUDA_CALL(esb_scratch_free(part, stream));
    if (rc != ESB_OK) return rc;
  }
  clip_coef_kernel<<<1, 1, 0, stream>>>(state, max_norm, world_scale);
  ESB_CUDA_LAUNCH_CHECK("esb_grad_clip_coef");
  return ESB_OK;
}

extern "C" int esb_adamw_step(float* param, const float* grad, float* exp_avg, float* exp_avg_sq, const float* lr_mult,
                              long long n, float lr, float beta1, float beta2, float eps, float weight_decay, int step,
                              float grad_scale, const float* clip_state, void* stream) {
  ESB_CHECK_ARG(step >= 1, "esb_adamw_step: step counts from 1");
  if (n == 0) return ESB_OK;
  float bc1 = 1.f - powf(beta1, (float)step);
  float bc2_sqrt = sqrtf(1.f - powf(beta2, (float)step));
  adamw_kernel<<<esb_div_up(n, 256), 256, 0, (cudaStream_t)stream>>>(param, grad, exp_avg, exp_avg_sq, lr_mult, n, lr, beta1,
                                                                      beta2, eps, weight_decay, bc1, bc2_sqrt,
                                                                      grad_scale, clip_state);
  ESB_CUDA_LAUNCH_CHECK("adamw_kernel");
  return ESB_OK;
}

extern "C" int esb_cast_f32_to_bf16(const float* src, void* dst, long long n, void* stream) {
  if (n == 0) return ESB_OK;
  cast_kernel<__nv_bfloat16><<<esb_div_up(n, 256), 256, 0, (cudaStream_t)stream>>>(src, (__nv_bfloat16*)dst, n);
  ESB_CUDA_LAUNCH_CHECK("cast_kernel");
  return ESB_OK;
}
```

### embodiedscan_b200/csrc/scratch.cu

```cuda
#include <mutex>

#include "common.cuh"

namespace {

__global__ void sum_partial_rows_kernel(const float* __restrict__ part, int n_parts, long long width, float* __restrict__ out,
                                        int accumulate) {
  const long long j = blockIdx.x * (long long)blockDim.x + threadIdx.x;
  if (j >= width) return;
  float s = accumulate ? out[j] : 0.f;
  for (int p = 0; p < n_parts; ++p) s += part[(long long)p * width + j];
  out[j] = s;
}

}

int esb_sm_count() {
  static int sms[64] = {};
  int dev = 0;
  cudaGetDevice(&dev);
  if (dev >= 64) return 132;
  if (sms[dev] == 0) {
    int n = 132;
    cudaDeviceGetAttribute(&n, cudaDevAttrMultiProcessorCount, dev);
    sms[dev] = n;
  }
  return sms[dev];
}

namespace {
constexpr unsigned long long kScratchKeepBytes = 512ull << 20;
std::mutex g_pool_mutex;
cudaMemPool_t g_pool[64] = {};

cudaMemPool_t scratch_pool(int dev, cudaStream_t s) {
  if (dev < 0 || dev >= 64) return nullptr;
  std::lock_guard<std::mutex> lock(g_pool_mutex);
  if (g_pool[dev] == nullptr) {
    cudaStreamCaptureStatus st = cudaStreamCaptureStatusNone;
    cudaStreamIsCapturing(s, &st);
    if (st != cudaStreamCaptureStatusNone) return nullptr;
    cudaMemPoolProps props = {};
    props.allocType = cudaMemAllocationTypePinned;
    props.location.type = cudaMemLocationTypeDevice;
    props.location.id = dev;
    cudaMemPool_t pool = nullptr;
    if (cudaMemPoolCreate(&pool, &props) != cudaSuccess) return nullptr;
    unsigned long long keep = kScratchKeepBytes;
    cudaMemPoolSetAttribute(pool, cudaMemPoolAttrReleaseThreshold, &keep);
    g_pool[dev] = pool;
  }
  return g_pool[dev];
}
}

cudaError_t esb_scratch_alloc(void** p, size_t bytes, cudaStream_t s) {
  int dev = 0;
  cudaGetDevice(&dev);
  const size_t n = bytes > 0 ? bytes : 16;
  cudaMemPool_t pool = scratch_pool(dev, s);
  return pool != nullptr ? cudaMallocFromPoolAsync(p, n, pool, s) : cudaMallocAsync(p, n, s);
}

cudaError_t esb_scratch_free(void* p, cudaStream_t s) { return cudaFreeAsync(p, s); }

int esb_sum_partial_rows(const float* part, int n_parts, long long width, float* out, int accumulate, cudaStream_t s) {
  if (width == 0) return ESB_OK;
  sum_partial_rows_kernel<<<esb_div_up(width, 256), 256, 0, s>>>(part, n_parts, width, out, accumulate);
  ESB_CUDA_LAUNCH_CHECK("sum_partial_rows_kernel");
  return ESB_OK;
}
```

### embodiedscan_b200/csrc/spconv.cu

```cuda
#include "common.cuh"

namespace {

constexpr int TM = 64;
constexpr int TN = 64;
constexpr int KC = 16;

template <typename T>
__device__ __forceinline__ void load4(const T* p, bool vec, int valid, float out[4]);

template <>
__device__ __forceinline__ void load4<float>(const float* p, bool vec, int valid, float out[4]) {
  if (vec && valid >= 4) {
    float4 v = *reinterpret_cast<const float4*>(p);
    out[0] = v.x; out[1] = v.y; out[2] = v.z; out[3] = v.w;
  } else {
#pragma unroll
    for (int j = 0; j < 4; ++j) out[j] = j < valid ? p[j] : 0.f;
  }
}
template <>
__device__ __forceinline__ void load4<__nv_bfloat16>(const __nv_bfloat16* p, bool vec, int valid, float out[4]) {
  if (vec && valid >= 4) {
    uint2 v = *reinterpret_cast<const uint2*>(p);
    __nv_bfloat162 a = *reinterpret_cast<__nv_bfloat162*>(&v.x);
    __nv_bfloat162 b = *reinterpret_cast<__nv_bfloat162*>(&v.y);
    out[0] = __low2float(a); out[1] = __high2float(a); out[2] = __low2float(b); out[3] = __high2float(b);
  } else {
#pragma unroll
    for (int j = 0; j < 4; ++j) out[j] = j < valid ? __bfloat162float(p[j]) : 0.f;
  }
}

template <typename T, bool WT>
__global__ void __launch_bounds__(256, WT ? 6 : 0)
spconv_fwd_kernel(const T* __restrict__ x, const T* __restrict__ w, const int* __restrict__ nbr, T* __restrict__ y,
                  int n_out, int cin, int cout, int K) {
  __shared__ __align__(16) float As[KC][TM + 4];
  __shared__ __align__(16) float Bs[KC][TN + 4];
  __shared__ int rows[TM];

  const int tid = threadIdx.x;
  const int tx = tid & 15, ty = tid >> 4;
  const int m0 = blockIdx.x * TM, n0 = blockIdx.y * TN;
  const bool vec_in = (cin & 3) == 0, vec_out = (cout & 3) == 0;

  float acc[4][4];
#pragma unroll
  for (int i = 0; i < 4; ++i)
#pragma unroll
    for (int j = 0; j < 4; ++j) acc[i][j] = 0.f;

  for (int k = 0; k < K; ++k) {
    int r = -1;
    if (tid < TM && m0 + tid < n_out) r = nbr[(long long)k * n_out + m0 + tid];
    if (tid < TM) rows[tid] = r;
    if (!__syncthreads_or(r >= 0)) continue;
    const T* wk = w + (long long)k * cin * cout;
    for (int c0 = 0; c0 < cin; c0 += KC) {
      {
        int row = tid >> 2, ch = (tid & 3) * 4;
        float v[4] = {0.f, 0.f, 0.f, 0.f};
        int src = rows[row];
        int valid = cin - (c0 + ch);
        if (src >= 0 && valid > 0) load4<T>(x + (long long)src * cin + c0 + ch, vec_in, valid, v);
#pragma unroll
        for (int j = 0; j < 4; ++j) As[ch + j][row] = v[j];
      }
      if (!WT) {
        int kc = tid >> 4, col = (tid & 15) * 4;
        float v[4] = {0.f, 0.f, 0.f, 0.f};
        int valid = cout - (n0 + col);
        if (c0 + kc < cin && valid > 0) load4<T>(wk + (long long)(c0 + kc) * cout + n0 + col, vec_out, valid, v);
#pragma unroll
        for (int j = 0; j < 4; ++j) Bs[kc][col + j] = v[j];
      } else {
        int col = tid >> 2, kc = (tid & 3) * 4;
        float v[4] = {0.f, 0.f, 0.f, 0.f};
        int valid = cin - (c0 + kc);
        if (n0 + col < cout && valid > 0) load4<T>(wk + (long long)(n0 + col) * cin + c0 + kc, vec_in, valid, v);
#pragma unroll
        for (int j = 0; j < 4; ++j) Bs[kc + j][col] = v[j];
      }
      __syncthreads();
#pragma unroll
      for (int kc = 0; kc < KC; ++kc) {
        float4 a = *reinterpret_cast<const float4*>(&As[kc][ty * 4]);
        float4 b = *reinterpret_cast<const float4*>(&Bs[kc][tx * 4]);
        float av[4] = {a.x, a.y, a.z, a.w}, bv[4] = {b.x, b.y, b.z, b.w};
#pragma unroll
        for (int i = 0; i < 4; ++i)
#pragma unroll
          for (int j = 0; j < 4; ++j) acc[i][j] = fmaf(av[i], bv[j], acc[i][j]);
      }
      __syncthreads();
    }
  }
#pragma unroll
  for (int i = 0; i < 4; ++i) {
    int row = m0 + ty * 4 + i;
    if (row >= n_out) continue;
#pragma unroll
    for (int j = 0; j < 4; ++j) {
      int col = n0 + tx * 4 + j;
      if (col < cout) y[(long long)row * cout + col] = esb_from_float<T>(acc[i][j]);
    }
  }
}

template <typename T>
__global__ void __launch_bounds__(256)
spconv_wgrad_kernel(const T* __restrict__ x, const T* __restrict__ dy, const int* __restrict__ pair_in,
                    const int* __restrict__ pair_out, const int* __restrict__ k_offsets, float* __restrict__ dw,
                    int cin, int cout, int splits) {
  __shared__ __align__(16) float As[KC][TM + 4];
  __shared__ __align__(16) float Bs[KC][TN + 4];
  const int tid = threadIdx.x;
  const int tx = tid & 15, ty = tid >> 4;
  const int k = blockIdx.x / splits, sp = blockIdx.x - k * splits;
  const int ci0 = blockIdx.y * TM, co0 = blockIdx.z * TN;
  const int p_beg = k_offsets[k], p_end = k_offsets[k + 1];
  const int np = p_end - p_beg;
  if (np <= 0) return;
  const int per = (np + splits - 1) / splits;
  const int s_beg = p_beg + sp * per;
  const int s_end = min(p_end, s_beg + per);
  if (s_beg >= s_end) return;
  const bool vec_in = (cin & 3) == 0, vec_out = (cout & 3) == 0;

  float acc[4][4];
#pragma unroll
  for (int i = 0; i < 4; ++i)
#pragma unroll
    for (int j = 0; j < 4; ++j) acc[i][j] = 0.f;

  for (int p0 = s_beg; p0 < s_end; p0 += KC) {
    {
      int pp = tid >> 4, ch = (tid & 15) * 4;
      float va[4] = {0.f, 0.f, 0.f, 0.f}, vb[4] = {0.f, 0.f, 0.f, 0.f};
      if (p0 + pp < s_end) {
        int ri = pair_in[p0 + pp], ro = pair_out[p0 + pp];
        int valid_a = cin - (ci0 + ch), valid_b = cout - (co0 + ch);
        if (valid_a > 0) load4<T>(x + (long long)ri * cin + ci0 + ch, vec_in, valid_a, va);
        if (valid_b > 0) load4<T>(dy + (long long)ro * cout + co0 + ch, vec_out, valid_b, vb);
      }
      *reinterpret_cast<float4*>(&As[pp][ch]) = make_float4(va[0], va[1], va[2], va[3]);
      *reinterpret_cast<float4*>(&Bs[pp][ch]) = make_float4(vb[0], vb[1], vb[2], vb[3]);
    }
    __syncthreads();
#pragma unroll
    for (int kc = 0; kc < KC; ++kc) {
      float4 a = *reinterpret_cast<const float4*>(&As[kc][ty * 4]);
      float4 b = *reinterpret_cast<const float4*>(&Bs[kc][tx * 4]);
      float av[4] = {a.x, a.y, a.z, a.w}, bv[4] = {b.x, b.y, b.z, b.w};
#pragma unroll
      for (int i = 0; i < 4; ++i)
#pragma unroll
        for (int j = 0; j < 4; ++j) acc[i][j] = fmaf(av[i], bv[j], acc[i][j]);
    }
    __syncthreads();
  }
  float* dwk = dw + ((long long)sp * gridDim.x / splits + k) * cin * cout;
#pragma unroll
  for (int i = 0; i < 4; ++i) {
    int ci = ci0 + ty * 4 + i;
    if (ci >= cin) continue;
#pragma unroll
    for (int j = 0; j < 4; ++j) {
      int co = co0 + tx * 4 + j;
      if (co < cout) dwk[(long long)ci * cout + co] = acc[i][j];
    }
  }
}

}

extern "C" int esb_spconv_fwd(const void* x, const void* w, const int* nbr, void* y, long long n_out, int cin, int cout,
                              int K, int w_transposed, int dtype, void* stream_) {
  cudaStream_t stream = (cudaStream_t)stream_;
  ESB_CHECK_ARG(cin > 0 && cout > 0 && K > 0, "esb_spconv_fwd: bad channel/kernel sizes");
  ESB_CHECK_ARG(dtype == ESB_F32 || dtype == ESB_BF16, "esb_spconv_fwd: dtype must be f32 or bf16");
  if (n_out == 0) return ESB_OK;
  dim3 grid(esb_div_up(n_out, TM), esb_div_up(cout, TN));
#define LAUNCH(T, WT) \
  spconv_fwd_kernel<T, WT><<<grid, 256, 0, stream>>>((const T*)x, (const T*)w, nbr, (T*)y, (int)n_out, cin, cout, K)
  if (dtype == ESB_F32) {
    if (w_transposed) LAUNCH(float, true); else LAUNCH(float, false);
  } else {
    if (w_transposed) LAUNCH(__nv_bfloat16, true); else LAUNCH(__nv_bfloat16, false);
  }
#undef LAUNCH
  ESB_CUDA_LAUNCH_CHECK("spconv_fwd_kernel");
  return ESB_OK;
}

extern "C" int esb_spconv_wgrad(const void* x, const void* dy, const int* pair_in, const int* pair_out,
                                const int* k_offsets, float* dw, long long n_pairs_hint, int cin, int cout, int K,
                                int dtype, void* stream_) {
  cudaStream_t stream = (cudaStream_t)stream_;
  ESB_CHECK_ARG(cin > 0 && cout > 0 && K > 0, "esb_spconv_wgrad: bad channel/kernel sizes");
  ESB_CHECK_ARG(dtype == ESB_F32 || dtype == ESB_BF16, "esb_spconv_wgrad: dtype must be f32 or bf16");
  int ci_t = esb_div_up(cin, TM), co_t = esb_div_up(cout, TN);
  long long per_k = n_pairs_hint / K + 1;
  int splits = (int)(4LL * esb_sm_count() / ((long long)K * ci_t * co_t));
  int max_by_pairs = (int)(per_k / 256) + 1;
  if (splits > max_by_pairs) splits = max_by_pairs;
  if (splits < 1) splits = 1;
  if (splits > 64) splits = 64;
  dim3 grid(K * splits, ci_t, co_t);
  const long long width = (long long)K * cin * cout;
  float* part = nullptr;
  ESB_CUDA_CALL(esb_scratch_alloc((void**)&part, sizeof(float) * splits * width, stream));
  ESB_CUDA_CALL(cudaMemsetAsync(part, 0, sizeof(float) * splits * width, stream));
  if (dtype == ESB_F32)
    spconv_wgrad_kernel<float><<<grid, 256, 0, stream>>>((const float*)x, (const float*)dy, pair_in, pair_out,
                                                          k_offsets, part, cin, cout, splits);
  else
    spconv_wgrad_kernel<__nv_bfloat16><<<grid, 256, 0, stream>>>((const __nv_bfloat16*)x, (const __nv_bfloat16*)dy,
                                                                  pair_in, pair_out, k_offsets, part, cin, cout, splits);
  ESB_CUDA_LAUNCH_CHECK("spconv_wgrad_kernel");
  int rc = esb_sum_partial_rows(part, splits, width, dw, 1, stream);
  ESB_CUDA_CALL(esb_scratch_free(part, stream));
  return rc;
}
```

### embodiedscan_b200/csrc/spconv_tc.cu

```cuda
#include "tc_common.cuh"

using namespace esb_tc;

namespace {

__global__ void tile_mask_kernel(const int* __restrict__ nbr, int K, int n, uint32_t* __restrict__ masks) {
  const int tile = blockIdx.x, r = threadIdx.x;
  const int row = tile * TC_M + r;
  uint32_t m = 0;
  if (row < n)
    for (int k = 0; k < K; ++k)
      if (nbr[(long long)k * n + row] >= 0) m |= 1u << k;
  m = __reduce_or_sync(0xffffffffu, m);
  __shared__ uint32_t s[4];
  if ((r & 31) == 0) s[r >> 5] = m;
  __syncthreads();
  if (r == 0) masks[tile] = s[0] | s[1] | s[2] | s[3];
}

template <int N_TILE, int STAGES, bool B_MN>
__global__ void __launch_bounds__(384, 1)
spconv_tc_fwd_kernel(const __nv_bfloat16* __restrict__ x, const __grid_constant__ CUtensorMap tmw,
                     const int* __restrict__ nbr, const uint32_t* __restrict__ masks, __nv_bfloat16* __restrict__ y,
                     int n_out, int cin, int cout, int K) {
  constexpr int A_BYTES = A_STAGE_BYTES;
  constexpr int B_STAGE_BYTES = N_TILE * 128;
  constexpr int STAGE_BYTES = A_BYTES + B_STAGE_BYTES;
  constexpr int LAG = STAGES - 2;
  constexpr int NPROD = 128;
  constexpr int NCONS = 256;
  constexpr int PITCH = N_TILE + 4;
  static_assert(TC_M * PITCH * 4 <= STAGES * STAGE_BYTES, "the accumulator image reuses the stage buffers");
  extern __shared__ __align__(1024) uint8_t smem_raw[];
  uint8_t* smem = (uint8_t*)(((uintptr_t)smem_raw + 1023) & ~(uintptr_t)1023);
  uint64_t* full_bar = (uint64_t*)(smem + STAGES * STAGE_BYTES);
  uint64_t* empty_bar = full_bar + STAGES;
  uint64_t* accum_bar = empty_bar + STAGES;
  float* img = reinterpret_cast<float*>(smem);
  __shared__ int idx_s[2][NPROD];

  const int tile = blockIdx.x;
  const int n0 = blockIdx.y * N_TILE;
  const uint32_t mask = masks[tile];
  const int nchunk = cin / TC_BK;
  const int total = __popc(mask) * nchunk;

  if (threadIdx.x == 0) {
    for (int s = 0; s < STAGES; ++s) {
      mbar_init(&full_bar[s], NPROD + 1);
      mbar_init(&empty_bar[s], NCONS / 32);
    }
    mbar_init(accum_bar, NCONS);
    asm volatile("fence.mbarrier_init.release.cluster;" ::: "memory");
    tma_prefetch_desc(&tmw);
  }
  __syncthreads();

  if (threadIdx.x >= NCONS) {
    const int t = threadIdx.x - NCONS;
    const int sub = t & 7, rgrp = t >> 3;
    const uint32_t sw = (uint32_t)(rgrp & 7);
    const uint32_t a_thread_off = (uint32_t)((rgrp >> 3) * 1024 + (rgrp & 7) * 128) + ((sub ^ sw) << 4);
    int it = 0, kcount = 0;
    const int my_row = tile * TC_M + t;
    int v_next = (mask && my_row < n_out) ? nbr[(long long)(__ffs(mask) - 1) * n_out + my_row] : -1;
    for (uint32_t mk = mask; mk; mk &= mk - 1, ++kcount) {
      const int k = __ffs(mk) - 1;
      int* idx_buf = idx_s[kcount & 1];
      idx_buf[t] = v_next;
      asm volatile("bar.sync 1, %0;" ::"n"(NPROD) : "memory");
      {
        const uint32_t rest = mk & (mk - 1);
        v_next = (rest && my_row < n_out) ? nbr[(long long)(__ffs(rest) - 1) * n_out + my_row] : -1;
      }
      int src[8];
#pragma unroll
      for (int i = 0; i < 8; ++i) src[i] = idx_buf[rgrp + 16 * i];
      for (int c = 0; c < nchunk; ++c, ++it) {
        const int s = it % STAGES;
        if (it >= STAGES) mbar_wait(&empty_bar[s], ((it / STAGES) - 1) & 1);
        const uint32_t stage_base = smem_u32(smem + s * STAGE_BYTES);
        if (t == 0) {
          mbar_expect_tx(&full_bar[s], B_STAGE_BYTES);
          const uint32_t b_base = stage_base + A_BYTES;
          if (B_MN) {
#pragma unroll
            for (int a = 0; a < N_TILE / 64; ++a) tma_load_2d(&tmw, &full_bar[s], b_base + a * 8192, n0 + a * 64, k * cin + c * TC_BK);
          } else {
            tma_load_2d(&tmw, &full_bar[s], b_base, c * TC_BK, k * cout + n0);
          }
        }
        const uint32_t a_base = stage_base + a_thread_off;
#pragma unroll
        for (int i = 0; i < 8; ++i)
          cp_async16_ca(a_base + i * 2048, x + (long long)(src[i] >= 0 ? src[i] : 0) * cin + c * TC_BK + sub * 8,
                        src[i] >= 0 ? 16 : 0);
        cp_async_commit();
        if (it >= LAG) {
          cp_async_wait<LAG>();
          fence_proxy_async();
          mbar_arrive(&full_bar[(it - LAG) % STAGES]);
        }
      }
    }
    cp_async_wait<0>();
    fence_proxy_async();
    for (int d = (total > LAG ? total - LAG : 0); d < total; ++d) mbar_arrive(&full_bar[d % STAGES]);

    const int row = tile * TC_M + t;
    if (total > 0) mbar_wait(accum_bar, 0);
    __nv_bfloat16* yrow = y + (long long)row * cout + n0;
#pragma unroll 1
    for (int c0 = 0; c0 < N_TILE; c0 += 32) {
      uint32_t v[32];
      if (total > 0) {
        img_ld<32>(img, PITCH, t, c0, v);
      } else {
#pragma unroll
        for (int i = 0; i < 32; ++i) v[i] = 0u;
      }
      if (row < n_out) {
#pragma unroll
        for (int q = 0; q < 4; ++q) {
          uint4 o;
          o.x = pack_bf16(v[8 * q + 0], v[8 * q + 1]);
          o.y = pack_bf16(v[8 * q + 2], v[8 * q + 3]);
          o.z = pack_bf16(v[8 * q + 4], v[8 * q + 5]);
          o.w = pack_bf16(v[8 * q + 6], v[8 * q + 7]);
          *reinterpret_cast<uint4*>(yrow + c0 + 8 * q) = o;
        }
      }
    }
  } else if (total > 0) {
    const int wg = threadIdx.x >> 7;
    float acc[N_TILE / 2];
    for (int it = 0; it < total; ++it) {
      const int s = it % STAGES;
      mbar_wait(&full_bar[s], (it / STAGES) & 1);
      const uint32_t a_addr = smem_u32(smem + s * STAGE_BYTES) + wg * 8192;
      const uint32_t b_addr = smem_u32(smem + s * STAGE_BYTES) + A_BYTES;
      wgmma_fence();
#pragma unroll
      for (int kk = 0; kk < TC_BK / 16; ++kk) {
        const uint64_t bd = B_MN ? make_desc(b_addr + kk * 2048, 8192, 1024) : make_desc(b_addr + kk * 32, 16, 1024);
        wgmma_bf16<N_TILE, 0, B_MN ? 1 : 0>(acc, make_desc(a_addr + kk * 32, 16, 1024), bd, it > 0 || kk > 0);
      }
      wgmma_commit();
      wgmma_wait<1>();
      if (it > 0 && (threadIdx.x & 31) == 0) mbar_arrive(&empty_bar[(it - 1) % STAGES]);
    }
    wgmma_wait<0>();
    acc_fence<N_TILE / 2>(acc);
    asm volatile("bar.sync 2, %0;" ::"n"(NCONS) : "memory");
    acc_store<N_TILE>(acc, img, PITCH, wg * 64, threadIdx.x & 127);
    mbar_arrive(accum_bar);
  }
}

template <int N_TILE, int STAGES>
__global__ void __launch_bounds__(384, 1)
spconv_tc_wgrad_kernel(const __nv_bfloat16* __restrict__ x, const __nv_bfloat16* __restrict__ dy,
                       const int* __restrict__ pair_in, const int* __restrict__ pair_out,
                       const int* __restrict__ k_offsets, float* __restrict__ part, int cin, int cout, int K,
                       int chunk_pairs) {
  constexpr int A_BYTES = 64 * 256;
  constexpr int B_BYTES = 64 * N_TILE * 2;
  constexpr int STAGE_BYTES = A_BYTES + B_BYTES;
  constexpr int LAG = STAGES - 2;
  constexpr int NCONS = 256;
  constexpr int PITCH = N_TILE + 4;
  static_assert(128 * PITCH * 4 <= STAGES * STAGE_BYTES, "the accumulator image reuses the stage buffers");
  extern __shared__ __align__(1024) uint8_t smem_raw[];
  uint8_t* smem = (uint8_t*)(((uintptr_t)smem_raw + 1023) & ~(uintptr_t)1023);
  uint64_t* full_bar = (uint64_t*)(smem + STAGES * STAGE_BYTES);
  uint64_t* empty_bar = full_bar + STAGES;
  uint64_t* accum_bar = empty_bar + STAGES;

  int k = 0, chunk = blockIdx.x, p_beg = 0, p_end = 0;
  for (; k < K; ++k) {
    p_beg = k_offsets[k];
    p_end = k_offsets[k + 1];
    const int nch = (p_end - p_beg + chunk_pairs - 1) / chunk_pairs;
    if (chunk < nch) break;
    chunk -= nch;
  }
  if (k >= K) return;
  const int ci0 = blockIdx.y * 128, co0 = blockIdx.z * N_TILE;
  const int s_beg = p_beg + chunk * chunk_pairs;
  const int s_end = min(p_end, s_beg + chunk_pairs);
  const int total = (s_end - s_beg + 63) / 64;

  if (threadIdx.x == 0) {
    for (int s = 0; s < STAGES; ++s) {
      mbar_init(&full_bar[s], 128);
      mbar_init(&empty_bar[s], NCONS / 32);
    }
    mbar_init(accum_bar, NCONS);
    asm volatile("fence.mbarrier_init.release.cluster;" ::: "memory");
  }
  __syncthreads();
  const int a_ch = min(128, cin - ci0);

  if (threadIdx.x >= NCONS) {
    const int t = threadIdx.x - NCONS;
    const int warp = t >> 5;
    const int mc = t & 15, kk0 = t >> 4;
    const bool a_ok_ch = mc * 8 < a_ch;
    int ri[8], ro[8];
#pragma unroll
    for (int q = 0; q < 8; ++q) {
      const int p = s_beg + kk0 + 8 * q;
      ri[q] = p < s_end ? pair_in[p] : -1;
      ro[q] = p < s_end ? pair_out[p] : -1;
    }
    for (int it = 0; it < total; ++it) {
      const int s = it % STAGES;
      if (it >= STAGES) mbar_wait(&empty_bar[s], ((it / STAGES) - 1) & 1);
      const uint32_t a_base = smem_u32(smem + s * STAGE_BYTES);
      const uint32_t b_base = a_base + A_BYTES;
#pragma unroll
      for (int q = 0; q < 8; ++q) {
        const int kk = kk0 + 8 * q;
        const bool ok = ri[q] >= 0 && a_ok_ch;
        const uint32_t dst = a_base + (mc >> 3) * 8192 + (kk >> 3) * 1024 + (kk & 7) * 128 + (((mc & 7) ^ (kk & 7)) << 4);
        cp_async16_cg(dst, x + (long long)(ok ? ri[q] : 0) * cin + ci0 + mc * 8, ok ? 16 : 0);
      }
#pragma unroll
      for (int q = 0; q < N_TILE / 16; ++q) {
        const int idx = q * 128 + t;
        const int kk = idx / (N_TILE / 8), nc = idx % (N_TILE / 8);
        int rr;
        if (N_TILE == 128) {
          rr = ro[q];
        } else {
          const int p = s_beg + it * 64 + kk;
          rr = p < s_end ? pair_out[p] : -1;
        }
        const uint32_t dst = b_base + (nc >> 3) * 8192 + (kk >> 3) * 1024 + (kk & 7) * 128 + (((nc & 7) ^ (kk & 7)) << 4);
        cp_async16_cg(dst, dy + (long long)(rr >= 0 ? rr : 0) * cout + co0 + nc * 8, rr >= 0 ? 16 : 0);
      }
      cp_async_commit();
      if (it + 1 < total) {
#pragma unroll
        for (int q = 0; q < 8; ++q) {
          const int p = s_beg + (it + 1) * 64 + kk0 + 8 * q;
          ri[q] = p < s_end ? pair_in[p] : -1;
          ro[q] = p < s_end ? pair_out[p] : -1;
        }
      }
      if (it >= LAG) {
        cp_async_wait<LAG>();
        fence_proxy_async();
        mbar_arrive(&full_bar[(it - LAG) % STAGES]);
      }
    }
    cp_async_wait<0>();
    fence_proxy_async();
    for (int d = (total > LAG ? total - LAG : 0); d < total; ++d) mbar_arrive(&full_bar[d % STAGES]);

    mbar_wait(accum_bar, 0);
    const float* stg = reinterpret_cast<const float*>(smem);
    const int lane = t & 31;
    for (int rr = 0; rr < 32; ++rr) {
      const int r = warp * 32 + rr;
      const int ci = ci0 + r;
      if (ci >= cin) break;
      float* dwrow = part + ((long long)blockIdx.x * cin + ci) * cout + co0;
#pragma unroll
      for (int c = lane * 4; c < N_TILE; c += 128)
        *reinterpret_cast<float4*>(dwrow + c) = *reinterpret_cast<const float4*>(stg + r * PITCH + c);
    }
  } else {
    const int wg = threadIdx.x >> 7;
    float acc[N_TILE / 2];
    for (int it = 0; it < total; ++it) {
      const int s = it % STAGES;
      mbar_wait(&full_bar[s], (it / STAGES) & 1);
      const uint32_t a_addr = smem_u32(smem + s * STAGE_BYTES) + wg * 8192;
      const uint32_t b_addr = smem_u32(smem + s * STAGE_BYTES) + A_BYTES;
      wgmma_fence();
#pragma unroll
      for (int kk = 0; kk < 4; ++kk)
        wgmma_bf16<N_TILE, 1, 1>(acc, make_desc(a_addr + kk * 2048, 8192, 1024), make_desc(b_addr + kk * 2048, 8192, 1024), it > 0 || kk > 0);
      wgmma_commit();
      wgmma_wait<1>();
      if (it > 0 && (threadIdx.x & 31) == 0) mbar_arrive(&empty_bar[(it - 1) % STAGES]);
    }
    wgmma_wait<0>();
    acc_fence<N_TILE / 2>(acc);
    asm volatile("bar.sync 2, %0;" ::"n"(NCONS) : "memory");
    acc_store<N_TILE>(acc, reinterpret_cast<float*>(smem), PITCH, wg * 64, threadIdx.x & 127);
    mbar_arrive(accum_bar);
  }
}

__global__ void spconv_wgrad_reduce_kernel(const float* __restrict__ part, const int* __restrict__ k_offsets, float* __restrict__ dw,
                                           int cin, int cout, int K, int chunk_pairs) {
  const long long e = blockIdx.x * (long long)blockDim.x + threadIdx.x;
  const long long per_k = (long long)cin * cout;
  if (e >= per_k * K) return;
  const int k = (int)(e / per_k);
  const long long j = e - k * per_k;
  int c0 = 0;
  for (int kk = 0; kk < k; ++kk) c0 += (k_offsets[kk + 1] - k_offsets[kk] + chunk_pairs - 1) / chunk_pairs;
  const int nch = (k_offsets[k + 1] - k_offsets[k] + chunk_pairs - 1) / chunk_pairs;
  float s = dw[e];
  for (int c = c0; c < c0 + nch; ++c) s += part[(long long)c * per_k + j];
  dw[e] = s;
}

template <int N_TILE, int STAGES, bool B_MN>
int launch_fwd(const void* x, const CUtensorMap& tmw, const int* nbr, const unsigned* masks, void* y, long long n_out, int cin,
               int cout, int K, cudaStream_t stream) {
  size_t smem = (size_t)STAGES * (A_STAGE_BYTES + N_TILE * 128) + 1024 + 256;
  auto kern = spconv_tc_fwd_kernel<N_TILE, STAGES, B_MN>;
  cudaError_t e = cudaFuncSetAttribute(kern, cudaFuncAttributeMaxDynamicSharedMemorySize, (int)smem);
  if (e != cudaSuccess) { esb_set_error("spconv_tc_fwd: smem attr: %s", cudaGetErrorString(e)); return ESB_ECUDA; }
  dim3 grid(esb_div_up(n_out, TC_M), cout / N_TILE);
  kern<<<grid, 384, smem, stream>>>((const __nv_bfloat16*)x, tmw, nbr, masks, (__nv_bfloat16*)y, (int)n_out, cin,
                                              cout, K);
  return ESB_OK;
}

template <int N_TILE, int STAGES>
int launch_wgrad(const void* x, const void* dy, const int* pin, const int* pout, const int* koff, float* part, int cin,
                 int cout, int K, int n_chunks, int chunk_pairs, cudaStream_t stream) {
  size_t smem = (size_t)STAGES * (64 * 256 + 64 * N_TILE * 2) + 1024 + 256;
  auto kern = spconv_tc_wgrad_kernel<N_TILE, STAGES>;
  cudaError_t e = cudaFuncSetAttribute(kern, cudaFuncAttributeMaxDynamicSharedMemorySize, (int)smem);
  if (e != cudaSuccess) { esb_set_error("spconv_tc_wgrad: smem attr: %s", cudaGetErrorString(e)); return ESB_ECUDA; }
  dim3 grid(n_chunks, esb_div_up(cin, 128), cout / N_TILE);
  kern<<<grid, 384, smem, stream>>>((const __nv_bfloat16*)x, (const __nv_bfloat16*)dy, pin, pout, koff, part, cin, cout, K,
                                    chunk_pairs);
  return ESB_OK;
}

}

extern "C" int esb_kmap_tile_masks(const int* nbr, int K, long long n, unsigned* masks, void* stream) {
  ESB_CHECK_ARG(K >= 1 && K <= 32, "esb_kmap_tile_masks: K must be in [1,32]");
  if (n == 0) return ESB_OK;
  tile_mask_kernel<<<esb_div_up(n, TC_M), 128, 0, (cudaStream_t)stream>>>(nbr, K, (int)n, masks);
  ESB_CUDA_LAUNCH_CHECK("tile_mask_kernel");
  return ESB_OK;
}

extern "C" int esb_spconv_tc_fwd(const void* x, const void* wt, const int* nbr, const unsigned* masks, void* y,
                                 long long n_out, int cin, int cout, int K, int w_layout, void* stream_) {
  cudaStream_t stream = (cudaStream_t)stream_;
  ESB_CHECK_ARG(cin % 64 == 0 && cout % 64 == 0 && cin > 0 && cout > 0, "esb_spconv_tc_fwd: channels must be multiples of 64");
  ESB_CHECK_ARG(K >= 1 && K <= 27, "esb_spconv_tc_fwd: K must be in [1,27]");
  if (n_out == 0) return ESB_OK;
  int rc;
  const int sms = esb_sm_count();
  long long row_tiles = (n_out + TC_M - 1) / TC_M;
  const int n_tile = (cout % 256 == 0 && row_tiles * (cout / 256) >= sms) ? 256
                     : (cout % 128 == 0 && row_tiles * (cout / 128) >= sms) ? 128 : 64;
  CUtensorMap tmw;
  {
    unsigned long long dims[2], str[1];
    unsigned box[2];
    if (w_layout) {
      dims[0] = (unsigned long long)cout; dims[1] = (unsigned long long)K * cin; str[0] = (unsigned long long)cout * 2;
      box[0] = 64; box[1] = 64;
    } else {
      dims[0] = (unsigned long long)cin; dims[1] = (unsigned long long)K * cout; str[0] = (unsigned long long)cin * 2;
      box[0] = 64; box[1] = (unsigned)n_tile;
    }
    rc = esb_tma_encode(&tmw, wt, 2, dims, str, box, nullptr, 128);
    if (rc != ESB_OK) return rc;
  }
#define ESB_TC_LAUNCH(NT, ST)                                                                       \
  (w_layout ? launch_fwd<NT, ST, true>(x, tmw, nbr, masks, y, n_out, cin, cout, K, stream)         \
            : launch_fwd<NT, ST, false>(x, tmw, nbr, masks, y, n_out, cin, cout, K, stream))
  if (n_tile == 256)
    rc = ESB_TC_LAUNCH(256, 4);
  else if (n_tile == 128)
    rc = ESB_TC_LAUNCH(128, 4);
  else
    rc = ESB_TC_LAUNCH(64, 4);
#undef ESB_TC_LAUNCH
  if (rc != ESB_OK) return rc;
  ESB_CUDA_LAUNCH_CHECK("spconv_tc_fwd_kernel");
  return ESB_OK;
}

extern "C" int esb_spconv_tc_wgrad(const void* x, const void* dy, const int* pair_in, const int* pair_out,
                                   const int* k_offsets, float* dw, long long n_pairs_hint, int cin, int cout, int K,
                                   void* stream_) {
  cudaStream_t stream = (cudaStream_t)stream_;
  ESB_CHECK_ARG(cin % 64 == 0 && cout % 64 == 0 && cin > 0 && cout > 0, "esb_spconv_tc_wgrad: channels must be multiples of 64");
  int n_tile = (cout % 128 == 0) ? 128 : 64;
  long long tiles = (long long)esb_div_up(cin, 128) * (cout / n_tile);
  long long target_chunks = (4LL * 2 * esb_sm_count() + tiles - 1) / tiles;
  long long cp = (n_pairs_hint / 2 + target_chunks - 1) / target_chunks;
  cp = (cp + 63) / 64 * 64;
  if (cp < 512) cp = 512;
  if (cp > 16384) cp = 16384;
  int chunk_pairs = (int)cp;
  int n_chunks = (int)(n_pairs_hint / chunk_pairs) + K + 1;
  float* part = nullptr;
  ESB_CUDA_CALL(esb_scratch_alloc((void**)&part, sizeof(float) * n_chunks * cin * cout, stream));
  int rc = n_tile == 128
               ? launch_wgrad<128, 3>(x, dy, pair_in, pair_out, k_offsets, part, cin, cout, K, n_chunks, chunk_pairs, stream)
               : launch_wgrad<64, 4>(x, dy, pair_in, pair_out, k_offsets, part, cin, cout, K, n_chunks, chunk_pairs, stream);
  if (rc == ESB_OK) {
    spconv_wgrad_reduce_kernel<<<esb_div_up((long long)K * cin * cout, 256), 256, 0, stream>>>(part, k_offsets, dw, cin, cout, K,
                                                                                             chunk_pairs);
  }
  ESB_CUDA_CALL(esb_scratch_free(part, stream));
  if (rc != ESB_OK) return rc;
  ESB_CUDA_LAUNCH_CHECK("spconv_tc_wgrad_kernel");
  return ESB_OK;
}
```

### embodiedscan_b200/csrc/spops.cu

```cuda
#include "common.cuh"

namespace {

template <typename T>
__global__ void maxpool_fwd_kernel(const T* __restrict__ x, const int* __restrict__ nbr, T* __restrict__ y,
                                   int* __restrict__ arg, long long n_out, int C, int K) {
  long long t = blockIdx.x * (long long)blockDim.x + threadIdx.x;
  if (t >= n_out * C) return;
  long long o = t / C;
  int c = (int)(t - o * C);
  float best = -INFINITY;
  int best_i = -1;
  for (int k = 0; k < K; ++k) {
    int i = nbr[(long long)k * n_out + o];
    if (i < 0) continue;
    float v = esb_to_float<T>(x[(long long)i * C + c]);
    if (best_i < 0 || v > best) {
      best = v;
      best_i = i;
    }
  }
  y[t] = esb_from_float<T>(best_i >= 0 ? best : 0.f);
  arg[t] = best_i;
}

template <typename T>
__global__ void maxpool_bwd_kernel(const T* __restrict__ dy, const int* __restrict__ arg, T* __restrict__ dx,
                                   long long n_out, int C) {
  long long t = blockIdx.x * (long long)blockDim.x + threadIdx.x;
  if (t >= n_out * C) return;
  int c = (int)(t % C);
  int i = arg[t];
  if (i >= 0) dx[(long long)i * C + c] = dy[t];
}

__device__ __forceinline__ int seg_begin(const int* __restrict__ seg_off, int s) { return seg_off ? seg_off[s] : 0; }
__device__ __forceinline__ int seg_end(const int* __restrict__ seg_off, int s, int n_total) {
  return seg_off ? seg_off[s + 1] : n_total;
}

template <typename T, int MODE>
__global__ void seg_colstat_kernel(const T* __restrict__ x, const int* __restrict__ seg_off, const float* __restrict__ mean,
                                   float* __restrict__ out, int C, int rows_per_block, int n_total) {
  __shared__ float red[8][33];
  const int s = blockIdx.y;
  const int c = blockIdx.z * 32 + threadIdx.x;
  const int r_beg = seg_begin(seg_off, s) + blockIdx.x * rows_per_block;
  const int r_end = min(seg_end(seg_off, s, n_total), r_beg + rows_per_block);
  float acc = 0.f;
  if (c < C) {
    float mu = MODE == 1 ? mean[s * C + c] : 0.f;
    for (int r = r_beg + threadIdx.y; r < r_end; r += 8) {
      float v = esb_to_float<T>(x[(long long)r * C + c]);
      if (MODE == 1) {
        v -= mu;
        acc = fmaf(v, v, acc);
      } else {
        acc += v;
      }
    }
  }
  red[threadIdx.y][threadIdx.x] = acc;
  __syncthreads();
  if (threadIdx.y == 0 && c < C) {
    float t = 0.f;
#pragma unroll
    for (int j = 0; j < 8; ++j) t += red[j][threadIdx.x];
    out[((long long)blockIdx.x * gridDim.y + s) * C + c] = t;
  }
}

__global__ void seg_finalize_mean_kernel(float* __restrict__ sum, const int* __restrict__ seg_off, int S, int C,
                                         int n_total) {
  int t = blockIdx.x * blockDim.x + threadIdx.x;
  if (t >= S * C) return;
  int s = t / C;
  int n = seg_end(seg_off, s, n_total) - seg_begin(seg_off, s);
  sum[t] = n > 0 ? sum[t] / (float)n : 0.f;
}
__global__ void seg_finalize_rstd_kernel(const float* __restrict__ mean, float* __restrict__ var_to_rstd,
                                         const int* __restrict__ seg_off, int S, int C, float eps,
                                         float* __restrict__ running_mean, float* __restrict__ running_var,
                                         float momentum, int n_total) {
  int t = blockIdx.x * blockDim.x + threadIdx.x;
  if (t >= S * C) return;
  int s = t / C;
  int n = seg_end(seg_off, s, n_total) - seg_begin(seg_off, s);
  float var = n > 0 ? var_to_rstd[t] / (float)n : 0.f;
  if (running_mean != nullptr && S == 1) {
    float unbiased = n > 1 ? var * (float)n / (float)(n - 1) : var;
    running_mean[t] = (1.f - momentum) * running_mean[t] + momentum * mean[t];
    running_var[t] = (1.f - momentum) * running_var[t] + momentum * unbiased;
  }
  var_to_rstd[t] = rsqrtf(var + eps);
}

__device__ __forceinline__ float act_fwd(float z, int act) {
  if (act == 1) return fmaxf(z, 0.f);
  if (act == 2) return z > 0.f ? z : expm1f(z);
  return z;
}
__device__ __forceinline__ float act_bwd_from_out(float y, int act) {
  if (act == 1) return y > 0.f ? 1.f : 0.f;
  if (act == 2) return y > 0.f ? 1.f : y + 1.f;
  return 1.f;
}

template <typename T>
__global__ void norm_apply_kernel(const T* __restrict__ x, const T* __restrict__ res, const int* __restrict__ row_seg,
                                  const float* __restrict__ mean, const float* __restrict__ rstd,
                                  const float* __restrict__ gamma, const float* __restrict__ beta, T* __restrict__ y,
                                  long long N, int C, int act) {
  long long t = blockIdx.x * (long long)blockDim.x + threadIdx.x;
  if (t >= N * C) return;
  long long r = t / C;
  int c = (int)(t - r * C);
  int s = row_seg ? row_seg[r] : 0;
  float g = gamma ? gamma[c] : 1.f, b = beta ? beta[c] : 0.f;
  float z = (esb_to_float<T>(x[t]) - mean[s * C + c]) * rstd[s * C + c] * g + b;
  if (res) z += esb_to_float<T>(res[t]);
  y[t] = esb_from_float<T>(act_fwd(z, act));
}

template <typename T>
__device__ __forceinline__ void load8(const T* p, float v[8]);
template <>
__device__ __forceinline__ void load8<float>(const float* p, float v[8]) {
  float4 a = reinterpret_cast<const float4*>(p)[0], b = reinterpret_cast<const float4*>(p)[1];
  v[0] = a.x; v[1] = a.y; v[2] = a.z; v[3] = a.w; v[4] = b.x; v[5] = b.y; v[6] = b.z; v[7] = b.w;
}
template <>
__device__ __forceinline__ void load8<__nv_bfloat16>(const __nv_bfloat16* p, float v[8]) {
  uint4 raw = *reinterpret_cast<const uint4*>(p);
  const __nv_bfloat162* h = reinterpret_cast<const __nv_bfloat162*>(&raw);
#pragma unroll
  for (int i = 0; i < 4; ++i) { v[2 * i] = __low2float(h[i]); v[2 * i + 1] = __high2float(h[i]); }
}
template <typename T>
__device__ __forceinline__ void store8(T* p, const float v[8]);
template <>
__device__ __forceinline__ void store8<float>(float* p, const float v[8]) {
  reinterpret_cast<float4*>(p)[0] = make_float4(v[0], v[1], v[2], v[3]);
  reinterpret_cast<float4*>(p)[1] = make_float4(v[4], v[5], v[6], v[7]);
}
template <>
__device__ __forceinline__ void store8<__nv_bfloat16>(__nv_bfloat16* p, const float v[8]) {
  uint4 o;
  __nv_bfloat162* h = reinterpret_cast<__nv_bfloat162*>(&o);
#pragma unroll
  for (int i = 0; i < 4; ++i) h[i] = __floats2bfloat162_rn(v[2 * i], v[2 * i + 1]);
  *reinterpret_cast<uint4*>(p) = o;
}

template <typename T>
__global__ void norm_apply_vec8_kernel(const T* __restrict__ x, const T* __restrict__ res, const int* __restrict__ row_seg,
                                       const float* __restrict__ mean, const float* __restrict__ rstd,
                                       const float* __restrict__ gamma, const float* __restrict__ beta, T* __restrict__ y,
                                       long long n_vec, int C, int act) {
  long long t = blockIdx.x * (long long)blockDim.x + threadIdx.x;
  if (t >= n_vec) return;
  const int cv = C >> 3;
  const long long r = t / cv;
  const int c0 = (int)(t - r * cv) << 3;
  const int s = row_seg ? row_seg[r] : 0;
  float v[8], rr[8];
  load8<T>(x + t * 8, v);
  if (res) load8<T>(res + t * 8, rr);
#pragma unroll
  for (int i = 0; i < 8; ++i) {
    const int c = c0 + i;
    float z = (v[i] - mean[s * C + c]) * rstd[s * C + c] * (gamma ? gamma[c] : 1.f) + (beta ? beta[c] : 0.f);
    if (res) z += rr[i];
    v[i] = act_fwd(z, act);
  }
  store8<T>(y + t * 8, v);
}

template <typename T>
__global__ void norm_bwd_apply_vec8_kernel(const T* __restrict__ x, const T* __restrict__ y, const T* __restrict__ dy,
                                           const int* __restrict__ row_seg, const int* __restrict__ seg_off,
                                           const float* __restrict__ mean, const float* __restrict__ rstd,
                                           const float* __restrict__ gamma, const float* __restrict__ sg,
                                           const float* __restrict__ sgx, T* __restrict__ dx, T* __restrict__ dres,
                                           long long N, long long n_vec, int C, int act) {
  long long t = blockIdx.x * (long long)blockDim.x + threadIdx.x;
  if (t >= n_vec) return;
  const int cv = C >> 3;
  const long long r = t / cv;
  const int c0 = (int)(t - r * cv) << 3;
  const int s = row_seg ? row_seg[r] : 0;
  const float inv_n = 1.f / (float)max(seg_end(seg_off, s, (int)N) - seg_begin(seg_off, s), 1);
  float xv[8], yv[8], gv[8], ov[8];
  load8<T>(x + t * 8, xv);
  load8<T>(y + t * 8, yv);
  load8<T>(dy + t * 8, gv);
#pragma unroll
  for (int i = 0; i < 8; ++i) {
    const int c = c0 + i;
    float g = gv[i] * act_bwd_from_out(yv[i], act);
    float rs = rstd[s * C + c];
    float xh = (xv[i] - mean[s * C + c]) * rs;
    ov[i] = (gamma ? gamma[c] : 1.f) * rs * (g - sg[s * C + c] * inv_n - xh * sgx[s * C + c] * inv_n);
    gv[i] = g;
  }
  store8<T>(dx + t * 8, ov);
  if (dres) store8<T>(dres + t * 8, gv);
}

template <typename T>
__global__ void norm_bwd_reduce_kernel(const T* __restrict__ x, const T* __restrict__ y, const T* __restrict__ dy,
                                       const int* __restrict__ seg_off, const float* __restrict__ mean,
                                       const float* __restrict__ rstd, float* __restrict__ sg, float* __restrict__ sgx,
                                       int C, int rows_per_block, int act, int n_total) {
  __shared__ float red0[8][33];
  __shared__ float red1[8][33];
  const int s = blockIdx.y;
  const int c = blockIdx.z * 32 + threadIdx.x;
  const int r_beg = seg_begin(seg_off, s) + blockIdx.x * rows_per_block;
  const int r_end = min(seg_end(seg_off, s, n_total), r_beg + rows_per_block);
  float a0 = 0.f, a1 = 0.f;
  if (c < C) {
    float mu = mean[s * C + c], rs = rstd[s * C + c];
    for (int r = r_beg + threadIdx.y; r < r_end; r += 8) {
      long long idx = (long long)r * C + c;
      float g = esb_to_float<T>(dy[idx]) * act_bwd_from_out(esb_to_float<T>(y[idx]), act);
      float xh = (esb_to_float<T>(x[idx]) - mu) * rs;
      a0 += g;
      a1 = fmaf(g, xh, a1);
    }
  }
  red0[threadIdx.y][threadIdx.x] = a0;
  red1[threadIdx.y][threadIdx.x] = a1;
  __syncthreads();
  if (threadIdx.y == 0 && c < C) {
    float t0 = 0.f, t1 = 0.f;
#pragma unroll
    for (int j = 0; j < 8; ++j) {
      t0 += red0[j][threadIdx.x];
      t1 += red1[j][threadIdx.x];
    }
    sg[((long long)blockIdx.x * gridDim.y + s) * C + c] = t0;
    sgx[((long long)blockIdx.x * gridDim.y + s) * C + c] = t1;
  }
}

template <typename T>
__global__ void norm_bwd_apply_kernel(const T* __restrict__ x, const T* __restrict__ y, const T* __restrict__ dy,
                                      const int* __restrict__ row_seg, const int* __restrict__ seg_off,
                                      const float* __restrict__ mean, const float* __restrict__ rstd,
                                      const float* __restrict__ gamma, const float* __restrict__ sg,
                                      const float* __restrict__ sgx, T* __restrict__ dx, T* __restrict__ dres,
                                      long long N, int C, int act) {
  long long t = blockIdx.x * (long long)blockDim.x + threadIdx.x;
  if (t >= N * C) return;
  long long r = t / C;
  int c = (int)(t - r * C);
  int s = row_seg ? row_seg[r] : 0;
  float inv_n = 1.f / (float)max(seg_end(seg_off, s, (int)N) - seg_begin(seg_off, s), 1);
  float g = esb_to_float<T>(dy[t]) * act_bwd_from_out(esb_to_float<T>(y[t]), act);
  float rs = rstd[s * C + c];
  float xh = (esb_to_float<T>(x[t]) - mean[s * C + c]) * rs;
  float gm = gamma ? gamma[c] : 1.f;
  float v = gm * rs * (g - sg[s * C + c] * inv_n - xh * sgx[s * C + c] * inv_n);
  dx[t] = esb_from_float<T>(v);
  if (dres) dres[t] = esb_from_float<T>(g);
}

template <typename T>
__global__ void bias_act_kernel(const T* __restrict__ x, const float* __restrict__ bias, const T* __restrict__ res,
                                T* __restrict__ y, long long n_vec, int C, int act) {
  long long t = blockIdx.x * (long long)blockDim.x + threadIdx.x;
  if (t >= n_vec) return;
  const int cv = C / 8;
  const int c0 = (int)(t % cv) * 8;
  float v[8], r[8];
  if (sizeof(T) == 2) {
    uint4 raw = reinterpret_cast<const uint4*>(x)[t];
    const __nv_bfloat162* h = reinterpret_cast<const __nv_bfloat162*>(&raw);
#pragma unroll
    for (int i = 0; i < 4; ++i) { v[2 * i] = __low2float(h[i]); v[2 * i + 1] = __high2float(h[i]); }
    if (res) {
      uint4 rr = reinterpret_cast<const uint4*>(res)[t];
      const __nv_bfloat162* g = reinterpret_cast<const __nv_bfloat162*>(&rr);
#pragma unroll
      for (int i = 0; i < 4; ++i) { r[2 * i] = __low2float(g[i]); r[2 * i + 1] = __high2float(g[i]); }
    }
  } else {
#pragma unroll
    for (int i = 0; i < 8; ++i) { v[i] = esb_to_float<T>(x[t * 8 + i]); r[i] = res ? esb_to_float<T>(res[t * 8 + i]) : 0.f; }
  }
#pragma unroll
  for (int i = 0; i < 8; ++i) v[i] = act_fwd(v[i] + (bias ? bias[c0 + i] : 0.f) + (res ? r[i] : 0.f), act);
  if (sizeof(T) == 2) {
    uint4 o;
    __nv_bfloat162* h = reinterpret_cast<__nv_bfloat162*>(&o);
#pragma unroll
    for (int i = 0; i < 4; ++i) h[i] = __floats2bfloat162_rn(v[2 * i], v[2 * i + 1]);
    reinterpret_cast<uint4*>(y)[t] = o;
  } else {
#pragma unroll
    for (int i = 0; i < 8; ++i) y[t * 8 + i] = esb_from_float<T>(v[i]);
  }
}

template <typename T>
__global__ void act_bwd_kernel(const T* __restrict__ dy, const T* __restrict__ y, T* __restrict__ dx, long long n,
                               int act) {
  long long t = (blockIdx.x * (long long)blockDim.x + threadIdx.x) * 8;
  if (t + 8 <= n) {
    float g[8], o[8];
    load8<T>(dy + t, g);
    load8<T>(y + t, o);
#pragma unroll
    for (int i = 0; i < 8; ++i) g[i] *= act_bwd_from_out(o[i], act);
    store8<T>(dx + t, g);
  } else {
    for (int i = 0; i < 8; ++i)
      if (t + i < n)
        dx[t + i] = esb_from_float<T>(esb_to_float<T>(dy[t + i]) * act_bwd_from_out(esb_to_float<T>(y[t + i]), act));
  }
}

template <typename T>
__global__ void bn_stats_kernel(const T* __restrict__ x, long long N, int C, int rows_per_block, float* __restrict__ part) {
  extern __shared__ float sh[];
  const int tpr = C / 8;
  const int c = (threadIdx.x % tpr) * 8;
  const int rsub = threadIdx.x / tpr, rstep = blockDim.x / tpr;
  const long long r_beg = (long long)blockIdx.x * rows_per_block;
  const long long r_end = r_beg + rows_per_block < N ? r_beg + rows_per_block : N;
  float piv[8], sum[8], sq[8];
  load8<T>(x + c, piv);
#pragma unroll
  for (int e = 0; e < 8; ++e) sum[e] = sq[e] = 0.f;
  if (rsub < rstep) {
    for (long long r = r_beg + rsub; r < r_end; r += rstep) {
      float v[8];
      load8<T>(x + r * C + c, v);
#pragma unroll
      for (int e = 0; e < 8; ++e) {
        const float d = v[e] - piv[e];
        sum[e] += d;
        sq[e] = fmaf(d, d, sq[e]);
      }
    }
#pragma unroll
    for (int e = 0; e < 8; ++e) {
      sh[(2 * rsub) * C + c + e] = sum[e];
      sh[(2 * rsub + 1) * C + c + e] = sq[e];
    }
  }
  __syncthreads();
  for (int i = threadIdx.x; i < 2 * C; i += blockDim.x) {
    const int k = i < C ? 0 : 1, ci = i < C ? i : i - C;
    float t = 0.f;
    for (int r = 0; r < rstep; ++r) t += sh[(2 * r + k) * C + ci];
    part[(long long)blockIdx.x * 2 * C + i] = t;
  }
}

template <typename T>
__global__ void bn_apply_fused_kernel(const T* __restrict__ x, const T* __restrict__ res, long long N, int C,
                                      const float* __restrict__ gamma, const float* __restrict__ beta, float eps,
                                      float* __restrict__ running_mean, float* __restrict__ running_var, float momentum, int act,
                                      float* __restrict__ stats, T* __restrict__ y) {
  const float inv_n = 1.f / (float)N;
  if (blockIdx.x == 0) {
    for (int i = threadIdx.x; i < C; i += blockDim.x) {
      const float m = stats[i] * inv_n;
      const float var = fmaxf(stats[C + i] * inv_n - m * m, 0.f);
      const float mean = esb_to_float<T>(x[i]) + m;
      stats[2 * C + i] = mean;
      stats[3 * C + i] = rsqrtf(var + eps);
      if (running_mean != nullptr) {
        const float unbiased = N > 1 ? var * (float)N / (float)(N - 1) : var;
        running_mean[i] = (1.f - momentum) * running_mean[i] + momentum * mean;
        running_var[i] = (1.f - momentum) * running_var[i] + momentum * unbiased;
      }
    }
  }
  const long long t = blockIdx.x * (long long)blockDim.x + threadIdx.x;
  const int cv = C / 8;
  if (t >= N * cv) return;
  const long long r = t / cv;
  const int c = (int)(t - r * cv) * 8;
  float v[8], piv[8], rs[8];
  load8<T>(x + r * C + c, v);
  load8<T>(x + c, piv);
  if (res != nullptr) load8<T>(res + r * C + c, rs);
#pragma unroll
  for (int e = 0; e < 8; ++e) {
    const float m = stats[c + e] * inv_n;
    const float var = fmaxf(stats[C + c + e] * inv_n - m * m, 0.f);
    const float g = gamma ? gamma[c + e] : 1.f, b = beta ? beta[c + e] : 0.f;
    float z = (v[e] - (piv[e] + m)) * rsqrtf(var + eps) * g + b;
    if (res != nullptr) z += rs[e];
    v[e] = act_fwd(z, act);
  }
  store8<T>(y + r * C + c, v);
}

template <typename T>
__global__ void gather2_rows_kernel(const T* __restrict__ a, const int* __restrict__ ia, long long na, const T* __restrict__ b,
                                    const int* __restrict__ ib, T* __restrict__ out, long long n_vec, int C) {
  const long long i = (long long)blockIdx.x * blockDim.x + threadIdx.x;
  if (i >= n_vec) return;
  const int cv = C / 8;
  const long long r = i / cv;
  const int c = (int)(i - r * cv) * 8;
  const long long ra = ia ? (long long)ia[r] : (r < na ? r : -1);
  float v[8];
#pragma unroll
  for (int e = 0; e < 8; ++e) v[e] = 0.f;
  if (ra >= 0) load8<T>(a + ra * C + c, v);
  if (b != nullptr) {
    const int rb = ib[r];
    if (rb >= 0) {
      float w[8];
      load8<T>(b + (long long)rb * C + c, w);
#pragma unroll
      for (int e = 0; e < 8; ++e) v[e] += w[e];
    }
  }
  store8<T>(out + r * C + c, v);
}

}

#define DISPATCH_T(dtype, ...)                         \
  if (dtype == ESB_F32) {                              \
    using T = float;                                   \
    __VA_ARGS__;                                       \
  } else {                                             \
    using T = __nv_bfloat16;                           \
    __VA_ARGS__;                                       \
  }

extern "C" int esb_maxpool_fwd(const void* x, const int* nbr, void* y, int* arg, long long n_out, int C, int K,
                               int dtype, void* stream) {
  if (n_out == 0) return ESB_OK;
  DISPATCH_T(dtype, (maxpool_fwd_kernel<T><<<esb_div_up(n_out * C, 256), 256, 0, (cudaStream_t)stream>>>(
                        (const T*)x, nbr, (T*)y, arg, n_out, C, K)));
  ESB_CUDA_LAUNCH_CHECK("maxpool_fwd_kernel");
  return ESB_OK;
}

extern "C" int esb_maxpool_bwd(const void* dy, const int* arg, void* dx, long long n_out, int C, int dtype,
                               void* stream) {
  if (n_out == 0) return ESB_OK;
  DISPATCH_T(dtype, (maxpool_bwd_kernel<T><<<esb_div_up(n_out * C, 256), 256, 0, (cudaStream_t)stream>>>(
                        (const T*)dy, arg, (T*)dx, n_out, C)));
  ESB_CUDA_LAUNCH_CHECK("maxpool_bwd_kernel");
  return ESB_OK;
}

extern "C" int esb_norm_fwd(const void* x, const void* res, const int* seg_off, const int* row_seg, int S,
                            long long N, int max_seg_rows, int C, const float* gamma, const float* beta, float eps,
                            float* running_mean, float* running_var, float momentum, int act, float* mean, float* rstd,
                            void* y, int dtype, void* stream_) {
  cudaStream_t stream = (cudaStream_t)stream_;
  ESB_CHECK_ARG(S >= 1 && C >= 1, "esb_norm_fwd: bad S/C");
  ESB_CHECK_ARG(seg_off != nullptr || S == 1, "esb_norm_fwd: seg_off may be NULL only for a single segment");
  ESB_CUDA_CALL(cudaMemsetAsync(mean, 0, sizeof(float) * S * C, stream));
  ESB_CUDA_CALL(cudaMemsetAsync(rstd, 0, sizeof(float) * S * C, stream));
  if (N == 0) return ESB_OK;
  const int rpb = 256;
  dim3 grid(esb_div_up(max_seg_rows > 0 ? max_seg_rows : 1, rpb), S, esb_div_up(C, 32)), block(32, 8);
  int fin = esb_div_up(S * C, 256);
  float* part = nullptr;
  ESB_CUDA_CALL(esb_scratch_alloc((void**)&part, sizeof(float) * grid.x * S * C, stream));
  int rc = ESB_OK;
  DISPATCH_T(dtype, {
    seg_colstat_kernel<T, 0><<<grid, block, 0, stream>>>((const T*)x, seg_off, nullptr, part, C, rpb, (int)N);
    rc = esb_sum_partial_rows(part, (int)grid.x, (long long)S * C, mean, 0, stream);
    seg_finalize_mean_kernel<<<fin, 256, 0, stream>>>(mean, seg_off, S, C, (int)N);
    seg_colstat_kernel<T, 1><<<grid, block, 0, stream>>>((const T*)x, seg_off, mean, part, C, rpb, (int)N);
    if (rc == ESB_OK) rc = esb_sum_partial_rows(part, (int)grid.x, (long long)S * C, rstd, 0, stream);
    seg_finalize_rstd_kernel<<<fin, 256, 0, stream>>>(mean, rstd, seg_off, S, C, eps, running_mean, running_var, momentum,
                                                      (int)N);
    if (C % 8 == 0)
      norm_apply_vec8_kernel<T><<<esb_div_up(N * (C / 8), 256), 256, 0, stream>>>(
          (const T*)x, (const T*)res, row_seg, mean, rstd, gamma, beta, (T*)y, N * (C / 8), C, act);
    else
      norm_apply_kernel<T><<<esb_div_up(N * C, 256), 256, 0, stream>>>((const T*)x, (const T*)res, row_seg, mean, rstd,
                                                                       gamma, beta, (T*)y, N, C, act);
  });
  ESB_CUDA_CALL(esb_scratch_free(part, stream));
  if (rc != ESB_OK) return rc;
  ESB_CUDA_LAUNCH_CHECK("esb_norm_fwd");
  return ESB_OK;
}

extern "C" int esb_norm_apply(const void* x, const void* res, const int* row_seg, long long N, int C,
                              const float* mean, const float* rstd, const float* gamma, const float* beta, int act,
                              void* y, int dtype, void* stream) {
  if (N == 0) return ESB_OK;
  DISPATCH_T(dtype, (norm_apply_kernel<T><<<esb_div_up(N * C, 256), 256, 0, (cudaStream_t)stream>>>(
                        (const T*)x, (const T*)res, row_seg, mean, rstd, gamma, beta, (T*)y, N, C, act)));
  ESB_CUDA_LAUNCH_CHECK("norm_apply_kernel");
  return ESB_OK;
}

extern "C" int esb_norm_bwd(const void* x, const void* y, const void* dy, const int* seg_off, const int* row_seg, int S,
                            long long N, int max_seg_rows, int C, const float* mean, const float* rstd,
                            const float* gamma, int act, float* sg, float* sgx, void* dx, void* dres, int zero_sums,
                            int dtype, void* stream_) {
  cudaStream_t stream = (cudaStream_t)stream_;
  if (zero_sums) {
    ESB_CUDA_CALL(cudaMemsetAsync(sg, 0, sizeof(float) * S * C, stream));
    ESB_CUDA_CALL(cudaMemsetAsync(sgx, 0, sizeof(float) * S * C, stream));
  }
  if (N == 0) return ESB_OK;
  const int rpb = 256;
  dim3 grid(esb_div_up(max_seg_rows > 0 ? max_seg_rows : 1, rpb), S, esb_div_up(C, 32)), block(32, 8);
  const long long width = (long long)S * C;
  float* part = nullptr;
  ESB_CUDA_CALL(esb_scratch_alloc((void**)&part, sizeof(float) * 2 * grid.x * width, stream));
  int rc = ESB_OK;
  DISPATCH_T(dtype, {
    norm_bwd_reduce_kernel<T><<<grid, block, 0, stream>>>((const T*)x, (const T*)y, (const T*)dy, seg_off, mean, rstd,
                                                          part, part + grid.x * width, C, rpb, act, (int)N);
    rc = esb_sum_partial_rows(part, (int)grid.x, width, sg, 1, stream);
    if (rc == ESB_OK) rc = esb_sum_partial_rows(part + grid.x * width, (int)grid.x, width, sgx, 1, stream);
    if (C % 8 == 0)
      norm_bwd_apply_vec8_kernel<T><<<esb_div_up(N * (C / 8), 256), 256, 0, stream>>>(
          (const T*)x, (const T*)y, (const T*)dy, row_seg, seg_off, mean, rstd, gamma, sg, sgx, (T*)dx, (T*)dres, N,
          N * (C / 8), C, act);
    else
      norm_bwd_apply_kernel<T><<<esb_div_up(N * C, 256), 256, 0, stream>>>(
          (const T*)x, (const T*)y, (const T*)dy, row_seg, seg_off, mean, rstd, gamma, sg, sgx, (T*)dx, (T*)dres, N, C, act);
  });
  ESB_CUDA_CALL(esb_scratch_free(part, stream));
  if (rc != ESB_OK) return rc;
  ESB_CUDA_LAUNCH_CHECK("esb_norm_bwd");
  return ESB_OK;
}

extern "C" int esb_bias_act_fwd(const void* x, const float* bias, const void* res, void* y, long long rows, int C, int act,
                                int dtype, void* stream) {
  ESB_CHECK_ARG(C % 8 == 0, "esb_bias_act_fwd: C must be a multiple of 8");
  long long n_vec = rows * (C / 8);
  if (n_vec == 0) return ESB_OK;
  DISPATCH_T(dtype, (bias_act_kernel<T><<<esb_div_up(n_vec, 256), 256, 0, (cudaStream_t)stream>>>(
                        (const T*)x, bias, (const T*)res, (T*)y, n_vec, C, act)));
  ESB_CUDA_LAUNCH_CHECK("bias_act_kernel");
  return ESB_OK;
}

extern "C" int esb_act_bwd(const void* dy, const void* y, void* dx, long long n, int act, int dtype, void* stream) {
  if (n == 0) return ESB_OK;
  DISPATCH_T(dtype, (act_bwd_kernel<T><<<esb_div_up(n, 256 * 8), 256, 0, (cudaStream_t)stream>>>(
                        (const T*)dy, (const T*)y, (T*)dx, n, act)));
  ESB_CUDA_LAUNCH_CHECK("act_bwd_kernel");
  return ESB_OK;
}

extern "C" int esb_gather2_rows(const void* a, const int* ia, long long na, const void* b, const int* ib, void* out, long long n,
                                int C, int dtype, void* stream) {
  ESB_CHECK_ARG(C > 0 && C % 8 == 0, "esb_gather2_rows: C must be a positive multiple of 8");
  ESB_CHECK_ARG((b == nullptr) == (ib == nullptr), "esb_gather2_rows: b and ib go together");
  const long long n_vec = n * (C / 8);
  if (n_vec == 0) return ESB_OK;
  DISPATCH_T(dtype, (gather2_rows_kernel<T><<<esb_div_up(n_vec, 256), 256, 0, (cudaStream_t)stream>>>(
                        (const T*)a, ia, na, (const T*)b, ib, (T*)out, n_vec, C)));
  ESB_CUDA_LAUNCH_CHECK("gather2_rows_kernel");
  return ESB_OK;
}

extern "C" int esb_batchnorm_fwd_fused(const void* x, const void* res, long long N, int C, const float* gamma, const float* beta,
                                       float eps, float* running_mean, float* running_var, float momentum, int act, float* stats,
                                       void* y, int dtype, void* stream_) {
  cudaStream_t stream = (cudaStream_t)stream_;
  ESB_CHECK_ARG(C % 8 == 0 && C >= 8 && C <= 2048, "esb_batchnorm_fwd_fused: C must be a multiple of 8 in [8, 2048]");
  ESB_CUDA_CALL(cudaMemsetAsync(stats, 0, sizeof(float) * 2 * C, stream));
  if (N == 0) return ESB_OK;
  long long rpb = (N + 2 * esb_sm_count() - 1) / (2 * esb_sm_count());
  if (rpb < 64) rpb = 64;
  const int grid_a = esb_div_up(N, rpb);
  const long long n_vec = N * (C / 8);
  const int rstep = 256 / (C / 8);
  float* part = nullptr;
  ESB_CUDA_CALL(esb_scratch_alloc((void**)&part, sizeof(float) * 2 * C * grid_a, stream));
  DISPATCH_T(dtype, (bn_stats_kernel<T><<<grid_a, 256, 2 * rstep * C * sizeof(float), stream>>>((const T*)x, N, C, (int)rpb, part)));
  ESB_CUDA_LAUNCH_CHECK("bn_stats_kernel");
  int rc = esb_sum_partial_rows(part, grid_a, 2LL * C, stats, 0, stream);
  ESB_CUDA_CALL(esb_scratch_free(part, stream));
  if (rc != ESB_OK) return rc;
  DISPATCH_T(dtype, (bn_apply_fused_kernel<T><<<esb_div_up(n_vec, 256), 256, 0, stream>>>(
                        (const T*)x, (const T*)res, N, C, gamma, beta, eps, running_mean, running_var, momentum, act, stats,
                        (T*)y)));
  ESB_CUDA_LAUNCH_CHECK("bn_apply_fused_kernel");
  return ESB_OK;
}
```

Before: 54.07.

## Fuse split-K partial reductions into producer kernels via last-block-arrives counters

Replaces the separate esb_sum_partial_rows reduction launches (and finalize kernels) in attention backward, conv wgrad, norm forward/backward and batchnorm stats with an in-kernel last-block reduction. Each block writes its partial, then atomically increments a per-group counter; the last block sums all partials in a fixed order into the output. This removes several kernel launches and memsets per norm/conv call. The cost is that the final summation is serialized onto one block per group and relies on threadfence/atomic ordering.

```diff
diff --git a/embodiedscan_b200/_ffi.py b/embodiedscan_b200/_ffi.py
--- a/embodiedscan_b200/_ffi.py
+++ b/embodiedscan_b200/_ffi.py
@@ -74,7 +74,7 @@
 KERNELS_PER_CALL = {
     'esb_voxelize_points': 1, 'esb_coord_unique': 6, 'esb_hash_build': 2, 'esb_hash_lookup': 1, 'esb_kernel_map': 1,
     'esb_kernel_map_transpose': 2, 'esb_kmap_pairs': 3, 'esb_generative_children': 1, 'esb_spconv_fwd': 1,
-    'esb_spconv_wgrad': 1, 'esb_maxpool_fwd': 1, 'esb_maxpool_bwd': 1, 'esb_norm_fwd': 5, 'esb_norm_apply': 1,
+    'esb_spconv_wgrad': 1, 'esb_maxpool_fwd': 1, 'esb_maxpool_bwd': 1, 'esb_norm_fwd': 3, 'esb_norm_apply': 1,
     'esb_norm_bwd': 2, 'esb_batchnorm_fwd_fused': 2, 'esb_paint_fwd': 1, 'esb_paint_bwd': 1, 'esb_fcaf3d_targets': 5,
     'esb_focal_loss_fwd': 1, 'esb_focal_loss_bwd': 1, 'esb_nms_bev_segmented': 1, 'esb_iou_bev_pairwise': 1,
     'esb_img_normalize': 1, 'esb_unproject_depth': 3, 'esb_grad_clip_coef': 2, 'esb_adamw_step': 1,
diff --git a/embodiedscan_b200/csrc/attn_tc.cu b/embodiedscan_b200/csrc/attn_tc.cu
--- a/embodiedscan_b200/csrc/attn_tc.cu
+++ b/embodiedscan_b200/csrc/attn_tc.cu
@@ -167,8 +167,8 @@
 attn_bwd_kernel(const __grid_constant__ CUtensorMap tmq, const __grid_constant__ CUtensorMap tmk,
                 const __grid_constant__ CUtensorMap tmv, const __grid_constant__ CUtensorMap tmdo,
                 const unsigned char* __restrict__ key_pad, const float* __restrict__ lse, const float* __restrict__ delta,
-                float* __restrict__ dq, __nv_bfloat16* __restrict__ dk, __nv_bfloat16* __restrict__ dv, int H, int Lq, int Lk,
-                float scale) {
+                float* __restrict__ part, unsigned* __restrict__ counters, float* __restrict__ dq, __nv_bfloat16* __restrict__ dk,
+                __nv_bfloat16* __restrict__ dv, int H, int Lq, int Lk, float scale) {
   extern __shared__ __align__(1024) uint8_t smem_raw[];
   uint8_t* smem = (uint8_t*)(((uintptr_t)smem_raw + 1023) & ~(uintptr_t)1023);
   uint8_t* k_s = smem;
@@ -208,108 +208,114 @@
         tma_load_2d(&tmdo, &qd_full[s], smem_u32(do_s + s * 8192), 0, bh * Lq + i * 128);
       }
     }
-    return;
-  }
-  const int t = threadIdx.x, wg = t >> 7;
-  const int ra = wg * 64 + 16 * (warp & 3) + (lane >> 2);
-  const int cq = 2 * (lane & 3);
-  bool k_dead[2];
-#pragma unroll
-  for (int h = 0; h < 2; ++h) {
-    const int kj = k0 + ra + 8 * h;
-    k_dead[h] = kj >= Lk || (key_pad != nullptr && key_pad[(long long)b * Lk + kj]);
-  }
-  const float sc2 = scale * LOG2E;
-  float sacc[64], pacc[64], dvacc[AT_D / 2], dkacc[AT_D / 2], dqacc[AT_D / 2];
-  const uint32_t ka = smem_u32(k_s), va = smem_u32(v_s), pa = smem_u32(pt_s), sa = smem_u32(ds_s);
-  mbar_wait(kv_full, 0);
-  for (int i = 0; i < n_qt; ++i) {
-    const int s = i & 1;
-    float* lse2_s = lse2_all + (i & 1) * 128;
-    float* delta_s = delta_all + (i & 1) * 128;
-    if (t < 128) {
-      const int qi = i * 128 + t;
-      lse2_s[t] = qi < Lq ? lse[(long long)bh * Lq + qi] * LOG2E : INFINITY;
-      delta_s[t] = qi < Lq ? delta[(long long)bh * Lq + qi] : 0.f;
-    }
-    asm volatile("bar.sync 1, %0;" ::"n"(AT_CONS) : "memory");
-    mbar_wait(&qd_full[s], (i >> 1) & 1);
-    const uint32_t qa = smem_u32(q_s + s * 8192), da = smem_u32(do_s + s * 8192);
-    wgmma_fence();
-#pragma unroll
-    for (int kk = 0; kk < 2; ++kk)
-      wgmma_bf16<128, 0, 0>(sacc, make_desc_sw(ka + wg * 4096 + kk * 32, 16, 512, SW64), make_desc_sw(qa + kk * 32, 16, 512, SW64),
-                            kk > 0);
-#pragma unroll
-    for (int kk = 0; kk < 2; ++kk)
-      wgmma_bf16<128, 0, 0>(pacc, make_desc_sw(va + wg * 4096 + kk * 32, 16, 512, SW64), make_desc_sw(da + kk * 32, 16, 512, SW64),
-                            kk > 0);
-    wgmma_commit();
-    wgmma_wait<0>();
-    acc_fence<64>(sacc);
-    acc_fence<64>(pacc);
-#pragma unroll
-    for (int jb = 0; jb < 16; ++jb)
+  } else {
+    const int t = threadIdx.x, wg = t >> 7;
+    const int ra = wg * 64 + 16 * (warp & 3) + (lane >> 2);
+    const int cq = 2 * (lane & 3);
+    bool k_dead[2];
+#pragma unroll
+    for (int h = 0; h < 2; ++h) {
+      const int kj = k0 + ra + 8 * h;
+      k_dead[h] = kj >= Lk || (key_pad != nullptr && key_pad[(long long)b * Lk + kj]);
+    }
+    const float sc2 = scale * LOG2E;
+    float sacc[64], pacc[64], dvacc[AT_D / 2], dkacc[AT_D / 2], dqacc[AT_D / 2];
+    const uint32_t ka = smem_u32(k_s), va = smem_u32(v_s), pa = smem_u32(pt_s), sa = smem_u32(ds_s);
+    mbar_wait(kv_full, 0);
+    for (int i = 0; i < n_qt; ++i) {
+      const int s = i & 1;
+      float* lse2_s = lse2_all + (i & 1) * 128;
+      float* delta_s = delta_all + (i & 1) * 128;
+      if (t < 128) {
+        const int qi = i * 128 + t;
+        lse2_s[t] = qi < Lq ? lse[(long long)bh * Lq + qi] * LOG2E : INFINITY;
+        delta_s[t] = qi < Lq ? delta[(long long)bh * Lq + qi] : 0.f;
+      }
+      asm volatile("bar.sync 1, %0;" ::"n"(AT_CONS) : "memory");
+      mbar_wait(&qd_full[s], (i >> 1) & 1);
+      const uint32_t qa = smem_u32(q_s + s * 8192), da = smem_u32(do_s + s * 8192);
+      wgmma_fence();
+#pragma unroll
+      for (int kk = 0; kk < 2; ++kk)
+        wgmma_bf16<128, 0, 0>(sacc, make_desc_sw(ka + wg * 4096 + kk * 32, 16, 512, SW64), make_desc_sw(qa + kk * 32, 16, 512, SW64),
+                              kk > 0);
+#pragma unroll
+      for (int kk = 0; kk < 2; ++kk)
+        wgmma_bf16<128, 0, 0>(pacc, make_desc_sw(va + wg * 4096 + kk * 32, 16, 512, SW64), make_desc_sw(da + kk * 32, 16, 512, SW64),
+                              kk > 0);
+      wgmma_commit();
+      wgmma_wait<0>();
+      acc_fence<64>(sacc);
+      acc_fence<64>(pacc);
+#pragma unroll
+      for (int jb = 0; jb < 16; ++jb)
+#pragma unroll
+        for (int h = 0; h < 2; ++h) {
+          float p[2], ds[2];
+#pragma unroll
+          for (int u = 0; u < 2; ++u) {
+            const int c = 8 * jb + cq + u, e = 4 * jb + 2 * h + u;
+            const float ex = k_dead[h] ? 0.f : exp2f(sacc[e] * sc2 - lse2_s[c]);
+            p[u] = ex;
+            ds[u] = ex * (pacc[e] - delta_s[c]) * scale;
+          }
+          const uint32_t off = tile_off(ra + 8 * h, 8 * jb + cq);
+          *reinterpret_cast<uint32_t*>(pt_s + off) = pack_bf16(__float_as_uint(p[0]), __float_as_uint(p[1]));
+          *reinterpret_cast<uint32_t*>(ds_s + off) = pack_bf16(__float_as_uint(ds[0]), __float_as_uint(ds[1]));
+        }
+      fence_proxy_async();
+      asm volatile("bar.sync 1, %0;" ::"n"(AT_CONS) : "memory");
+      wgmma_fence();
+#pragma unroll
+      for (int kk = 0; kk < 8; ++kk) {
+        const uint32_t a_off = wg * 8192 + (kk >> 2) * 16384 + (kk & 3) * 32;
+        wgmma_bf16<AT_D, 0, 1>(dvacc, make_desc_sw(pa + a_off, 16, 1024, SW128), make_desc_sw(da + kk * 1024, 2048, 512, SW64),
+                               i > 0 || kk > 0);
+        wgmma_bf16<AT_D, 0, 1>(dkacc, make_desc_sw(sa + a_off, 16, 1024, SW128), make_desc_sw(qa + kk * 1024, 2048, 512, SW64),
+                               i > 0 || kk > 0);
+      }
+#pragma unroll
+      for (int kk = 0; kk < 8; ++kk)
+        wgmma_bf16<AT_D, 1, 1>(dqacc, make_desc_sw(sa + wg * 16384 + kk * 2048, 16384, 1024, SW128),
+                               make_desc_sw(ka + kk * 1024, 2048, 512, SW64), kk > 0);
+      wgmma_commit();
+      wgmma_wait<0>();
+      acc_fence<AT_D / 2>(dvacc);
+      acc_fence<AT_D / 2>(dkacc);
+      acc_fence<AT_D / 2>(dqacc);
+      if (lane == 0) mbar_arrive(&qd_empty[s]);
 #pragma unroll
       for (int h = 0; h < 2; ++h) {
-        float p[2], ds[2];
-#pragma unroll
-        for (int u = 0; u < 2; ++u) {
-          const int c = 8 * jb + cq + u, e = 4 * jb + 2 * h + u;
-          const float ex = k_dead[h] ? 0.f : exp2f(sacc[e] * sc2 - lse2_s[c]);
-          p[u] = ex;
-          ds[u] = ex * (pacc[e] - delta_s[c]) * scale;
+        const int qi = i * 128 + ra + 8 * h;
+        if (qi < Lq) {
+          float* dst = part + (((long long)blockIdx.x * gridDim.y + bh) * Lq + qi) * AT_D;
+#pragma unroll
+          for (int jb = 0; jb < AT_D / 8; ++jb)
+            *reinterpret_cast<float2*>(dst + 8 * jb + cq) = make_float2(dqacc[4 * jb + 2 * h], dqacc[4 * jb + 2 * h + 1]);
         }
-        const uint32_t off = tile_off(ra + 8 * h, 8 * jb + cq);
-        *reinterpret_cast<uint32_t*>(pt_s + off) = pack_bf16(__float_as_uint(p[0]), __float_as_uint(p[1]));
-        *reinterpret_cast<uint32_t*>(ds_s + off) = pack_bf16(__float_as_uint(ds[0]), __float_as_uint(ds[1]));
-      }
-    fence_proxy_async();
-    asm volatile("bar.sync 1, %0;" ::"n"(AT_CONS) : "memory");
-    wgmma_fence();
-#pragma unroll
-    for (int kk = 0; kk < 8; ++kk) {
-      const uint32_t a_off = wg * 8192 + (kk >> 2) * 16384 + (kk & 3) * 32;
-      wgmma_bf16<AT_D, 0, 1>(dvacc, make_desc_sw(pa + a_off, 16, 1024, SW128), make_desc_sw(da + kk * 1024, 2048, 512, SW64),
-                             i > 0 || kk > 0);
-      wgmma_bf16<AT_D, 0, 1>(dkacc, make_desc_sw(sa + a_off, 16, 1024, SW128), make_desc_sw(qa + kk * 1024, 2048, 512, SW64),
-                             i > 0 || kk > 0);
-    }
-#pragma unroll
-    for (int kk = 0; kk < 8; ++kk)
-      wgmma_bf16<AT_D, 1, 1>(dqacc, make_desc_sw(sa + wg * 16384 + kk * 2048, 16384, 1024, SW128),
-                             make_desc_sw(ka + kk * 1024, 2048, 512, SW64), kk > 0);
-    wgmma_commit();
-    wgmma_wait<0>();
-    acc_fence<AT_D / 2>(dvacc);
-    acc_fence<AT_D / 2>(dkacc);
-    acc_fence<AT_D / 2>(dqacc);
-    if (lane == 0) mbar_arrive(&qd_empty[s]);
+      }
+    }
 #pragma unroll
     for (int h = 0; h < 2; ++h) {
-      const int qi = i * 128 + ra + 8 * h;
-      if (qi < Lq) {
-        float* dst = dq + (((long long)blockIdx.x * gridDim.y + bh) * Lq + qi) * AT_D;
-#pragma unroll
-        for (int jb = 0; jb < AT_D / 8; ++jb)
-          *reinterpret_cast<float2*>(dst + 8 * jb + cq) = make_float2(dqacc[4 * jb + 2 * h], dqacc[4 * jb + 2 * h + 1]);
-      }
-    }
-  }
-#pragma unroll
-  for (int h = 0; h < 2; ++h) {
-    const int kj = k0 + ra + 8 * h;
-    if (kj < Lk) {
-      __nv_bfloat16* pv = dv + ((long long)bh * Lk + kj) * AT_D;
-      __nv_bfloat16* pk = dk + ((long long)bh * Lk + kj) * AT_D;
-#pragma unroll
-      for (int jb = 0; jb < AT_D / 8; ++jb) {
-        *reinterpret_cast<uint32_t*>(pv + 8 * jb + cq) =
-            pack_bf16(__float_as_uint(dvacc[4 * jb + 2 * h]), __float_as_uint(dvacc[4 * jb + 2 * h + 1]));
-        *reinterpret_cast<uint32_t*>(pk + 8 * jb + cq) =
-            pack_bf16(__float_as_uint(dkacc[4 * jb + 2 * h]), __float_as_uint(dkacc[4 * jb + 2 * h + 1]));
-      }
-    }
+      const int kj = k0 + ra + 8 * h;
+      if (kj < Lk) {
+        __nv_bfloat16* pv = dv + ((long long)bh * Lk + kj) * AT_D;
+        __nv_bfloat16* pk = dk + ((long long)bh * Lk + kj) * AT_D;
+#pragma unroll
+        for (int jb = 0; jb < AT_D / 8; ++jb) {
+          *reinterpret_cast<uint32_t*>(pv + 8 * jb + cq) =
+              pack_bf16(__float_as_uint(dvacc[4 * jb + 2 * h]), __float_as_uint(dvacc[4 * jb + 2 * h + 1]));
+          *reinterpret_cast<uint32_t*>(pk + 8 * jb + cq) =
+              pack_bf16(__float_as_uint(dkacc[4 * jb + 2 * h]), __float_as_uint(dkacc[4 * jb + 2 * h + 1]));
+        }
+      }
+    }
+  }
+  if (!esb_arrive_last(&counters[bh], gridDim.x)) return;
+  const long long width = (long long)Lq * AT_D;
+  for (long long i = 4 * threadIdx.x; i < width; i += 4 * blockDim.x) {
+    float4* d = reinterpret_cast<float4*>(dq + bh * width + i);
+    *d = esb_add_parts4(*d, part, gridDim.x, gridDim.y * width, bh * width + i);
   }
 }
 
@@ -357,13 +363,12 @@
   cudaError_t e = cudaFuncSetAttribute(attn_bwd_kernel, cudaFuncAttributeMaxDynamicSharedMemorySize, (int)smem);
   if (e != cudaSuccess) { esb_set_error("esb_attn_bwd: smem attr: %s", cudaGetErrorString(e)); return ESB_ECUDA; }
   dim3 grid((Lk + 127) / 128, B * H);
-  const long long width = rows * AT_D;
   float* part = nullptr;
-  ESB_CUDA_CALL(esb_scratch_alloc((void**)&part, sizeof(float) * grid.x * width, stream));
-  attn_bwd_kernel<<<grid, AT_THREADS, smem, stream>>>(tmq, tmk, tmv, tmdo, key_pad, lse, delta, part, (__nv_bfloat16*)dk,
-                                                      (__nv_bfloat16*)dv, H, Lq, Lk, scale);
+  unsigned* counters = nullptr;
+  ESB_CUDA_CALL(esb_split_alloc(&part, &counters, (size_t)grid.x * rows * AT_D, B * H, stream));
+  attn_bwd_kernel<<<grid, AT_THREADS, smem, stream>>>(tmq, tmk, tmv, tmdo, key_pad, lse, delta, part, counters, dq,
+                                                      (__nv_bfloat16*)dk, (__nv_bfloat16*)dv, H, Lq, Lk, scale);
   ESB_CUDA_LAUNCH_CHECK("attn_bwd_kernel");
-  rc = esb_sum_partial_rows(part, (int)grid.x, width, dq, 1, stream);
   ESB_CUDA_CALL(esb_scratch_free(part, stream));
-  return rc;
-}
+  return ESB_OK;
+}
diff --git a/embodiedscan_b200/csrc/common.cuh b/embodiedscan_b200/csrc/common.cuh
--- a/embodiedscan_b200/csrc/common.cuh
+++ b/embodiedscan_b200/csrc/common.cuh
@@ -38,7 +38,7 @@
 static inline size_t esb_align(size_t x, size_t a = 256) { return (x + a - 1) / a * a; }
 cudaError_t esb_scratch_alloc(void** p, size_t bytes, cudaStream_t s);
 cudaError_t esb_scratch_free(void* p, cudaStream_t s);
-int esb_sum_partial_rows(const float* part, int n_parts, long long width, float* out, int accumulate, cudaStream_t s);
+cudaError_t esb_split_alloc(float** part, unsigned** counters, size_t part_floats, int n_groups, cudaStream_t s);
 
 int esb_sm_count();
 
@@ -105,4 +105,53 @@
   for (int o = 16; o > 0; o >>= 1) v = fmaxf(v, __shfl_xor_sync(0xffffffffu, v, o));
   return v;
 }
+
+__device__ __forceinline__ bool esb_arrive_last(unsigned* counter, unsigned n_blocks) {
+  __shared__ bool last;
+  __threadfence();
+  __syncthreads();
+  if (threadIdx.x == 0 && threadIdx.y == 0 && threadIdx.z == 0) {
+    last = atomicAdd(counter, 1u) == n_blocks - 1;
+    if (last) *counter = 0u;
+  }
+  __syncthreads();
+  if (last) __threadfence();
+  return last;
+}
+
+__device__ __forceinline__ float4 esb_add_parts4(float4 acc, const float* part, int n_parts, long long stride, long long off) {
+  int p = 0;
+  for (; p + 8 <= n_parts; p += 8) {
+    float4 v[8];
+#pragma unroll
+    for (int q = 0; q < 8; ++q) v[q] = __ldcg(reinterpret_cast<const float4*>(part + (long long)(p + q) * stride + off));
+#pragma unroll
+    for (int q = 0; q < 8; ++q) {
+      acc.x += v[q].x; acc.y += v[q].y; acc.z += v[q].z; acc.w += v[q].w;
+    }
+  }
+  for (; p < n_parts; ++p) {
+    const float4 v = __ldcg(reinterpret_cast<const float4*>(part + (long long)p * stride + off));
+    acc.x += v.x; acc.y += v.y; acc.z += v.z; acc.w += v.w;
+  }
+  return acc;
+}
+
+__device__ __forceinline__ void esb_ordered_sum(const float* part, int n_parts, long long stride, int width, float* out,
+                                                bool accumulate) {
+  const int nt = blockDim.x * blockDim.y, tid = threadIdx.y * blockDim.x + threadIdx.x;
+  for (int j = tid; j < width; j += nt) {
+    float s = accumulate ? out[j] : 0.f;
+    int p = 0;
+    for (; p + 16 <= n_parts; p += 16) {
+      float v[16];
+#pragma unroll
+      for (int q = 0; q < 16; ++q) v[q] = __ldcg(part + (long long)(p + q) * stride + j);
+#pragma unroll
+      for (int q = 0; q < 16; ++q) s += v[q];
+    }
+    for (; p < n_parts; ++p) s += __ldcg(part + (long long)p * stride + j);
+    out[j] = s;
+  }
+}
 #endif
diff --git a/embodiedscan_b200/csrc/conv_tma.cu b/embodiedscan_b200/csrc/conv_tma.cu
--- a/embodiedscan_b200/csrc/conv_tma.cu
+++ b/embodiedscan_b200/csrc/conv_tma.cu
@@ -575,7 +575,7 @@
 template <int N_TILE>
 __global__ void __launch_bounds__(THREADS, 1)
 conv_tma_wgrad_kernel(const __grid_constant__ CUtensorMap tmx, const __grid_constant__ CUtensorMap tmdy,
-                      float* __restrict__ dw, const WgradGeom g) {
+                      float* __restrict__ part, unsigned* __restrict__ counters, float* __restrict__ dw, const WgradGeom g) {
   constexpr int NA = N_TILE < 64 ? N_TILE : 64;
   constexpr int A_BYTES = 64 * 256;
   constexpr int B_BYTES = 64 * N_TILE * 2;
@@ -674,10 +674,22 @@
       if (r >= rows_valid) break;
       const int ga = atom0 + r / g.aw;
       const int tap = ga / g.chunks_per_tap, ch = (ga - tap * g.chunks_per_tap) * g.aw + (r % g.aw);
-      float* dwrow = dw + (((long long)blockIdx.x * g.kd * g.kh * g.kw + tap) * g.cin + ch) * g.cout + co0;
+      float* dwrow = part + (((long long)blockIdx.x * taps + tap) * g.cin + ch) * g.cout + co0;
       for (int c = lane * 4; c < N_TILE; c += 128)
         *reinterpret_cast<float4*>(dwrow + c) = *reinterpret_cast<const float4*>(stg + r * PITCH + c);
     }
+  }
+
+  if (!esb_arrive_last(&counters[blockIdx.y * gridDim.z + blockIdx.z], gridDim.x)) return;
+  const long long width = (long long)taps * g.cin * g.cout;
+  constexpr int V4 = N_TILE / 4;
+  for (int i = threadIdx.x; i < n_valid * g.aw * V4; i += blockDim.x) {
+    const int r = i / V4;
+    const int ga = atom0 + r / g.aw;
+    const int tap = ga / g.chunks_per_tap, ch = (ga - tap * g.chunks_per_tap) * g.aw + (r % g.aw);
+    const long long off = ((long long)tap * g.cin + ch) * g.cout + co0 + (i % V4) * 4;
+    float4* d = reinterpret_cast<float4*>(dw + off);
+    *d = esb_add_parts4(*d, part, gridDim.x, width, off);
   }
 }
 
@@ -701,11 +713,11 @@
   dim3 grid((unsigned)((n_tiles + g.tiles_per_cta - 1) / g.tiles_per_cta), slices, n_blocks);
   const long long width = (long long)g.kd * g.kh * g.kw * g.cin * g.cout;
   float* part = nullptr;
-  ESB_CUDA_CALL(esb_scratch_alloc((void**)&part, sizeof(float) * grid.x * width, stream));
-  kern<<<grid, THREADS, smem, stream>>>(tmx, tmdy, part, g);
-  int rc = esb_sum_partial_rows(part, (int)grid.x, width, dw, 1, stream);
+  unsigned* counters = nullptr;
+  ESB_CUDA_CALL(esb_split_alloc(&part, &counters, (size_t)grid.x * width, slices * n_blocks, stream));
+  kern<<<grid, THREADS, smem, stream>>>(tmx, tmdy, part, counters, dw, g);
   ESB_CUDA_CALL(esb_scratch_free(part, stream));
-  return rc;
+  return ESB_OK;
 }
 
 }
diff --git a/embodiedscan_b200/csrc/head.cu b/embodiedscan_b200/csrc/head.cu
--- a/embodiedscan_b200/csrc/head.cu
+++ b/embodiedscan_b200/csrc/head.cu
@@ -210,18 +210,21 @@
 
 template <typename T>
 __global__ void focal_fwd_kernel(const T* __restrict__ logits, const long long* __restrict__ target, long long n, int C,
-                                 float gamma, float alpha, const float* __restrict__ row_w, float* __restrict__ loss_sum) {
-  long long t = blockIdx.x * (long long)blockDim.x + threadIdx.x;
+                                 float gamma, float alpha, const float* __restrict__ row_w, float* __restrict__ part,
+                                 unsigned* __restrict__ counter, float* __restrict__ loss_sum) {
   float l = 0.f;
-  if (t < n * C) {
+  const long long total = n * C;
+  for (long long t = blockIdx.x * (long long)blockDim.x + threadIdx.x; t < total; t += (long long)gridDim.x * blockDim.x) {
     long long r = t / C;
     int c = (int)(t - r * C);
     float p = sigmoidf(esb_to_float<T>(logits[t]));
+    float lt;
     if (target[r] == c)
-      l = -alpha * pow_gamma(1.f - p, gamma) * logf(fmaxf(p, 1.17549435e-38f));
+      lt = -alpha * pow_gamma(1.f - p, gamma) * logf(fmaxf(p, 1.17549435e-38f));
     else
-      l = -(1.f - alpha) * pow_gamma(p, gamma) * logf(fmaxf(1.f - p, 1.17549435e-38f));
-    if (row_w) l *= row_w[r];
+      lt = -(1.f - alpha) * pow_gamma(p, gamma) * logf(fmaxf(1.f - p, 1.17549435e-38f));
+    if (row_w) lt *= row_w[r];
+    l += lt;
   }
   l = esb_warp_sum(l);
   __shared__ float red[8];
@@ -230,8 +233,10 @@
   if (threadIdx.x == 0) {
     float s = 0.f;
     for (int i = 0; i < (int)(blockDim.x >> 5); ++i) s += red[i];
-    loss_sum[blockIdx.x] = s;
-  }
+    part[blockIdx.x] = s;
+  }
+  if (!esb_arrive_last(counter, gridDim.x)) return;
+  esb_ordered_sum(part, gridDim.x, 1, 1, loss_sum, true);
 }
 
 template <typename T>
@@ -381,7 +386,8 @@
 __global__ void __launch_bounds__(64)
 bbox_cd_loss_kernel(const float* __restrict__ points, const float* __restrict__ bbox_pred, const float* __restrict__ tgt,
                     const float* __restrict__ row_w, float w0, float w1, float w2, float w3, int P,
-                    float* __restrict__ loss_out, float* __restrict__ grad) {
+                    float* __restrict__ part, unsigned* __restrict__ counter, float* __restrict__ loss_out,
+                    float* __restrict__ grad) {
   int p = blockIdx.x * blockDim.x + threadIdx.x;
   float lval = 0.f;
   if (p < P) {
@@ -432,7 +438,9 @@
   __shared__ float red[2];
   if ((threadIdx.x & 31) == 0) red[threadIdx.x >> 5] = lval;
   __syncthreads();
-  if (threadIdx.x == 0) loss_out[blockIdx.x] = red[0] + red[1];
+  if (threadIdx.x == 0) part[blockIdx.x] = red[0] + red[1];
+  if (!esb_arrive_last(counter, gridDim.x)) return;
+  esb_ordered_sum(part, gridDim.x, 1, 1, loss_out, true);
 }
 
 }
@@ -479,16 +487,18 @@
   if (n == 0) return ESB_OK;
   cudaStream_t s = (cudaStream_t)stream;
   int grid = esb_div_up(n * C, 256);
+  if (grid > 8 * esb_sm_count()) grid = 8 * esb_sm_count();
   float* part = nullptr;
-  ESB_CUDA_CALL(esb_scratch_alloc((void**)&part, (size_t)grid * sizeof(float), s));
+  unsigned* counter = nullptr;
+  ESB_CUDA_CALL(esb_split_alloc(&part, &counter, grid, 1, s));
   if (dtype == ESB_F32)
-    focal_fwd_kernel<float><<<grid, 256, 0, s>>>((const float*)logits, target, n, C, gamma, alpha, row_w, part);
+    focal_fwd_kernel<float><<<grid, 256, 0, s>>>((const float*)logits, target, n, C, gamma, alpha, row_w, part, counter, loss_sum);
   else
-    focal_fwd_kernel<__nv_bfloat16><<<grid, 256, 0, s>>>((const __nv_bfloat16*)logits, target, n, C, gamma, alpha, row_w, part);
+    focal_fwd_kernel<__nv_bfloat16><<<grid, 256, 0, s>>>((const __nv_bfloat16*)logits, target, n, C, gamma, alpha, row_w, part,
+                                                          counter, loss_sum);
   ESB_CUDA_LAUNCH_CHECK("focal_fwd_kernel");
-  int rc = esb_sum_partial_rows(part, grid, 1, loss_sum, 1, s);
   ESB_CUDA_CALL(esb_scratch_free(part, s));
-  return rc;
+  return ESB_OK;
 }
 
 extern "C" int esb_focal_loss_bwd(const void* logits, const long long* target, long long n, int C, float gamma,
@@ -512,11 +522,11 @@
   cudaStream_t s = (cudaStream_t)stream;
   const int grid = esb_div_up(P, 64);
   float* part = nullptr;
-  ESB_CUDA_CALL(esb_scratch_alloc((void**)&part, (size_t)grid * sizeof(float), s));
+  unsigned* counter = nullptr;
+  ESB_CUDA_CALL(esb_split_alloc(&part, &counter, grid, 1, s));
   bbox_cd_loss_kernel<<<grid, 64, 0, s>>>(points, bbox_pred, targets, row_w, w4_host[0], w4_host[1], w4_host[2], w4_host[3], P,
-                                          part, grad);
+                                          part, counter, loss_out, grad);
   ESB_CUDA_LAUNCH_CHECK("bbox_cd_loss_kernel");
-  int rc = esb_sum_partial_rows(part, grid, 1, loss_out, 1, s);
   ESB_CUDA_CALL(esb_scratch_free(part, s));
-  return rc;
-}
+  return ESB_OK;
+}
diff --git a/embodiedscan_b200/csrc/optim.cu b/embodiedscan_b200/csrc/optim.cu
--- a/embodiedscan_b200/csrc/optim.cu
+++ b/embodiedscan_b200/csrc/optim.cu
@@ -2,7 +2,8 @@
 
 namespace {
 
-__global__ void sumsq_kernel(const float* __restrict__ g, long long n, float* __restrict__ out) {
+__global__ void sumsq_kernel(const float* __restrict__ g, long long n, float* __restrict__ part, unsigned* __restrict__ counter,
+                             float* __restrict__ state) {
   float acc = 0.f;
   long long stride = (long long)gridDim.x * blockDim.x * 4;
   for (long long i = (blockIdx.x * (long long)blockDim.x + threadIdx.x) * 4; i < n; i += stride) {
@@ -20,8 +21,10 @@
   if (threadIdx.x < 32) {
     float v = threadIdx.x < (blockDim.x >> 5) ? red[threadIdx.x] : 0.f;
     v = esb_warp_sum(v);
-    if (threadIdx.x == 0) out[blockIdx.x] = v;
+    if (threadIdx.x == 0) part[blockIdx.x] = v;
   }
+  if (!esb_arrive_last(counter, gridDim.x)) return;
+  esb_ordered_sum(part, gridDim.x, 1, 1, state, false);
 }
 
 __global__ void clip_coef_kernel(float* state, float max_norm, float world_scale) {
@@ -68,11 +71,10 @@
     if (grid > esb_sm_count() * 8) grid = esb_sm_count() * 8;
     if (grid < 1) grid = 1;
     float* part = nullptr;
-    ESB_CUDA_CALL(esb_scratch_alloc((void**)&part, (size_t)grid * sizeof(float), stream));
-    sumsq_kernel<<<grid, 256, 0, stream>>>(grad, n, part);
-    int rc = esb_sum_partial_rows(part, grid, 1, state, 0, stream);
+    unsigned* counter = nullptr;
+    ESB_CUDA_CALL(esb_split_alloc(&part, &counter, grid, 1, stream));
+    sumsq_kernel<<<grid, 256, 0, stream>>>(grad, n, part, counter, state);
     ESB_CUDA_CALL(esb_scratch_free(part, stream));
-    if (rc != ESB_OK) return rc;
   }
   clip_coef_kernel<<<1, 1, 0, stream>>>(state, max_norm, world_scale);
   ESB_CUDA_LAUNCH_CHECK("esb_grad_clip_coef");
diff --git a/embodiedscan_b200/csrc/scratch.cu b/embodiedscan_b200/csrc/scratch.cu
--- a/embodiedscan_b200/csrc/scratch.cu
+++ b/embodiedscan_b200/csrc/scratch.cu
@@ -1,19 +1,6 @@
 #include <mutex>
 
 #include "common.cuh"
-
-namespace {
-
-__global__ void sum_partial_rows_kernel(const float* __restrict__ part, int n_parts, long long width, float* __restrict__ out,
-                                        int accumulate) {
-  const long long j = blockIdx.x * (long long)blockDim.x + threadIdx.x;
-  if (j >= width) return;
-  float s = accumulate ? out[j] : 0.f;
-  for (int p = 0; p < n_parts; ++p) s += part[(long long)p * width + j];
-  out[j] = s;
-}
-
-}
 
 int esb_sm_count() {
   static int sms[64] = {};
@@ -64,9 +51,12 @@
 
 cudaError_t esb_scratch_free(void* p, cudaStream_t s) { return cudaFreeAsync(p, s); }
 
-int esb_sum_partial_rows(const float* part, int n_parts, long long width, float* out, int accumulate, cudaStream_t s) {
-  if (width == 0) return ESB_OK;
-  sum_partial_rows_kernel<<<esb_div_up(width, 256), 256, 0, s>>>(part, n_parts, width, out, accumulate);
-  ESB_CUDA_LAUNCH_CHECK("sum_partial_rows_kernel");
-  return ESB_OK;
+cudaError_t esb_split_alloc(float** part, unsigned** counters, size_t part_floats, int n_groups, cudaStream_t s) {
+  const size_t pb = esb_align(part_floats * sizeof(float));
+  uint8_t* p = nullptr;
+  cudaError_t e = esb_scratch_alloc((void**)&p, pb + (size_t)n_groups * sizeof(unsigned), s);
+  if (e != cudaSuccess) return e;
+  *part = (float*)p;
+  *counters = (unsigned*)(p + pb);
+  return cudaMemsetAsync(*counters, 0, (size_t)n_groups * sizeof(unsigned), s);
 }
diff --git a/embodiedscan_b200/csrc/spconv.cu b/embodiedscan_b200/csrc/spconv.cu
--- a/embodiedscan_b200/csrc/spconv.cu
+++ b/embodiedscan_b200/csrc/spconv.cu
@@ -111,8 +111,8 @@
 template <typename T>
 __global__ void __launch_bounds__(256)
 spconv_wgrad_kernel(const T* __restrict__ x, const T* __restrict__ dy, const int* __restrict__ pair_in,
-                    const int* __restrict__ pair_out, const int* __restrict__ k_offsets, float* __restrict__ dw,
-                    int cin, int cout, int splits) {
+                    const int* __restrict__ pair_out, const int* __restrict__ k_offsets, float* __restrict__ part,
+                    unsigned* __restrict__ counters, float* __restrict__ dw, int cin, int cout, int splits) {
   __shared__ __align__(16) float As[KC][TM + 4];
   __shared__ __align__(16) float Bs[KC][TN + 4];
   const int tid = threadIdx.x;
@@ -126,6 +126,7 @@
   const int s_beg = p_beg + sp * per;
   const int s_end = min(p_end, s_beg + per);
   if (s_beg >= s_end) return;
+  const int n_split = (np + per - 1) / per;
   const bool vec_in = (cin & 3) == 0, vec_out = (cout & 3) == 0;
 
   float acc[4][4];
@@ -160,7 +161,8 @@
     }
     __syncthreads();
   }
-  float* dwk = dw + ((long long)sp * gridDim.x / splits + k) * cin * cout;
+  const long long per_k = (long long)cin * cout;
+  float* dwk = part + ((long long)sp * (gridDim.x / splits) + k) * per_k;
 #pragma unroll
   for (int i = 0; i < 4; ++i) {
     int ci = ci0 + ty * 4 + i;
@@ -169,6 +171,20 @@
     for (int j = 0; j < 4; ++j) {
       int co = co0 + tx * 4 + j;
       if (co < cout) dwk[(long long)ci * cout + co] = acc[i][j];
+    }
+  }
+  if (!esb_arrive_last(&counters[((long long)k * gridDim.y + blockIdx.y) * gridDim.z + blockIdx.z], n_split)) return;
+  const long long stride = (long long)(gridDim.x / splits) * per_k;
+  for (int i = 0; i < 4; ++i) {
+    const int ci = ci0 + ty * 4 + i;
+    if (ci >= cin) continue;
+    for (int j = 0; j < 4; ++j) {
+      const int co = co0 + tx * 4 + j;
+      if (co >= cout) continue;
+      const long long off = k * per_k + (long long)ci * cout + co;
+      float s = dw[off];
+      for (int q = 0; q < n_split; ++q) s += __ldcg(part + q * stride + off);
+      dw[off] = s;
     }
   }
 }
@@ -208,18 +224,17 @@
   if (splits < 1) splits = 1;
   if (splits > 64) splits = 64;
   dim3 grid(K * splits, ci_t, co_t);
-  const long long width = (long long)K * cin * cout;
   float* part = nullptr;
-  ESB_CUDA_CALL(esb_scratch_alloc((void**)&part, sizeof(float) * splits * width, stream));
-  ESB_CUDA_CALL(cudaMemsetAsync(part, 0, sizeof(float) * splits * width, stream));
+  unsigned* counters = nullptr;
+  ESB_CUDA_CALL(esb_split_alloc(&part, &counters, (size_t)splits * K * cin * cout, K * ci_t * co_t, stream));
   if (dtype == ESB_F32)
     spconv_wgrad_kernel<float><<<grid, 256, 0, stream>>>((const float*)x, (const float*)dy, pair_in, pair_out,
-                                                          k_offsets, part, cin, cout, splits);
+                                                          k_offsets, part, counters, dw, cin, cout, splits);
   else
     spconv_wgrad_kernel<__nv_bfloat16><<<grid, 256, 0, stream>>>((const __nv_bfloat16*)x, (const __nv_bfloat16*)dy,
-                                                                  pair_in, pair_out, k_offsets, part, cin, cout, splits);
+                                                                  pair_in, pair_out, k_offsets, part, counters, dw, cin, cout,
+                                                                  splits);
   ESB_CUDA_LAUNCH_CHECK("spconv_wgrad_kernel");
-  int rc = esb_sum_partial_rows(part, splits, width, dw, 1, stream);
   ESB_CUDA_CALL(esb_scratch_free(part, stream));
-  return rc;
-}
+  return ESB_OK;
+}
diff --git a/embodiedscan_b200/csrc/spconv_tc.cu b/embodiedscan_b200/csrc/spconv_tc.cu
--- a/embodiedscan_b200/csrc/spconv_tc.cu
+++ b/embodiedscan_b200/csrc/spconv_tc.cu
@@ -161,8 +161,8 @@
 __global__ void __launch_bounds__(384, 1)
 spconv_tc_wgrad_kernel(const __nv_bfloat16* __restrict__ x, const __nv_bfloat16* __restrict__ dy,
                        const int* __restrict__ pair_in, const int* __restrict__ pair_out,
-                       const int* __restrict__ k_offsets, float* __restrict__ part, int cin, int cout, int K,
-                       int chunk_pairs) {
+                       const int* __restrict__ k_offsets, float* __restrict__ part, unsigned* __restrict__ counters,
+                       float* __restrict__ dw, int cin, int cout, int K, int chunk_pairs) {
   constexpr int A_BYTES = 64 * 256;
   constexpr int B_BYTES = 64 * N_TILE * 2;
   constexpr int STAGE_BYTES = A_BYTES + B_BYTES;
@@ -292,21 +292,17 @@
     acc_store<N_TILE>(acc, reinterpret_cast<float*>(smem), PITCH, wg * 64, threadIdx.x & 127);
     mbar_arrive(accum_bar);
   }
-}
-
-__global__ void spconv_wgrad_reduce_kernel(const float* __restrict__ part, const int* __restrict__ k_offsets, float* __restrict__ dw,
-                                           int cin, int cout, int K, int chunk_pairs) {
-  const long long e = blockIdx.x * (long long)blockDim.x + threadIdx.x;
+
+  const int nch = (p_end - p_beg + chunk_pairs - 1) / chunk_pairs;
+  if (!esb_arrive_last(&counters[((long long)k * gridDim.y + blockIdx.y) * gridDim.z + blockIdx.z], nch)) return;
   const long long per_k = (long long)cin * cout;
-  if (e >= per_k * K) return;
-  const int k = (int)(e / per_k);
-  const long long j = e - k * per_k;
-  int c0 = 0;
-  for (int kk = 0; kk < k; ++kk) c0 += (k_offsets[kk + 1] - k_offsets[kk] + chunk_pairs - 1) / chunk_pairs;
-  const int nch = (k_offsets[k + 1] - k_offsets[k] + chunk_pairs - 1) / chunk_pairs;
-  float s = dw[e];
-  for (int c = c0; c < c0 + nch; ++c) s += part[(long long)c * per_k + j];
-  dw[e] = s;
+  const long long c0 = blockIdx.x - chunk;
+  constexpr int V4 = N_TILE / 4;
+  for (int i = threadIdx.x; i < a_ch * V4; i += blockDim.x) {
+    const long long off = (long long)(ci0 + i / V4) * cout + co0 + (i % V4) * 4;
+    float4* d = reinterpret_cast<float4*>(dw + k * per_k + off);
+    *d = esb_add_parts4(*d, part + c0 * per_k, nch, per_k, off);
+  }
 }
 
 template <int N_TILE, int STAGES, bool B_MN>
@@ -323,15 +319,15 @@
 }
 
 template <int N_TILE, int STAGES>
-int launch_wgrad(const void* x, const void* dy, const int* pin, const int* pout, const int* koff, float* part, int cin,
-                 int cout, int K, int n_chunks, int chunk_pairs, cudaStream_t stream) {
+int launch_wgrad(const void* x, const void* dy, const int* pin, const int* pout, const int* koff, float* part, unsigned* counters,
+                 float* dw, int cin, int cout, int K, int n_chunks, int chunk_pairs, cudaStream_t stream) {
   size_t smem = (size_t)STAGES * (64 * 256 + 64 * N_TILE * 2) + 1024 + 256;
   auto kern = spconv_tc_wgrad_kernel<N_TILE, STAGES>;
   cudaError_t e = cudaFuncSetAttribute(kern, cudaFuncAttributeMaxDynamicSharedMemorySize, (int)smem);
   if (e != cudaSuccess) { esb_set_error("spconv_tc_wgrad: smem attr: %s", cudaGetErrorString(e)); return ESB_ECUDA; }
   dim3 grid(n_chunks, esb_div_up(cin, 128), cout / N_TILE);
-  kern<<<grid, 384, smem, stream>>>((const __nv_bfloat16*)x, (const __nv_bfloat16*)dy, pin, pout, koff, part, cin, cout, K,
-                                    chunk_pairs);
+  kern<<<grid, 384, smem, stream>>>((const __nv_bfloat16*)x, (const __nv_bfloat16*)dy, pin, pout, koff, part, counters, dw, cin,
+                                    cout, K, chunk_pairs);
   return ESB_OK;
 }
 
@@ -400,14 +396,14 @@
   int chunk_pairs = (int)cp;
   int n_chunks = (int)(n_pairs_hint / chunk_pairs) + K + 1;
   float* part = nullptr;
-  ESB_CUDA_CALL(esb_scratch_alloc((void**)&part, sizeof(float) * n_chunks * cin * cout, stream));
+  unsigned* counters = nullptr;
+  ESB_CUDA_CALL(esb_split_alloc(&part, &counters, (size_t)n_chunks * cin * cout, K * esb_div_up(cin, 128) * (cout / n_tile),
+                                stream));
   int rc = n_tile == 128
-               ? launch_wgrad<128, 3>(x, dy, pair_in, pair_out, k_offsets, part, cin, cout, K, n_chunks, chunk_pairs, stream)
-               : launch_wgrad<64, 4>(x, dy, pair_in, pair_out, k_offsets, part, cin, cout, K, n_chunks, chunk_pairs, stream);
-  if (rc == ESB_OK) {
-    spconv_wgrad_reduce_kernel<<<esb_div_up((long long)K * cin * cout, 256), 256, 0, stream>>>(part, k_offsets, dw, cin, cout, K,
-                                                                                             chunk_pairs);
-  }
+               ? launch_wgrad<128, 3>(x, dy, pair_in, pair_out, k_offsets, part, counters, dw, cin, cout, K, n_chunks, chunk_pairs,
+                                      stream)
+               : launch_wgrad<64, 4>(x, dy, pair_in, pair_out, k_offsets, part, counters, dw, cin, cout, K, n_chunks, chunk_pairs,
+                                     stream);
   ESB_CUDA_CALL(esb_scratch_free(part, stream));
   if (rc != ESB_OK) return rc;
   ESB_CUDA_LAUNCH_CHECK("spconv_tc_wgrad_kernel");
diff --git a/embodiedscan_b200/csrc/spops.cu b/embodiedscan_b200/csrc/spops.cu
--- a/embodiedscan_b200/csrc/spops.cu
+++ b/embodiedscan_b200/csrc/spops.cu
@@ -41,7 +41,9 @@
 
 template <typename T, int MODE>
 __global__ void seg_colstat_kernel(const T* __restrict__ x, const int* __restrict__ seg_off, const float* __restrict__ mean,
-                                   float* __restrict__ out, int C, int rows_per_block, int n_total) {
+                                   float* __restrict__ part, unsigned* __restrict__ counters, float* __restrict__ out, int C,
+                                   int rows_per_block, int n_total, float eps, float* __restrict__ running_mean,
+                                   float* __restrict__ running_var, float momentum) {
   __shared__ float red[8][33];
   const int s = blockIdx.y;
   const int c = blockIdx.z * 32 + threadIdx.x;
@@ -66,33 +68,27 @@
     float t = 0.f;
 #pragma unroll
     for (int j = 0; j < 8; ++j) t += red[j][threadIdx.x];
-    out[((long long)blockIdx.x * gridDim.y + s) * C + c] = t;
-  }
-}
-
-__global__ void seg_finalize_mean_kernel(float* __restrict__ sum, const int* __restrict__ seg_off, int S, int C,
-                                         int n_total) {
-  int t = blockIdx.x * blockDim.x + threadIdx.x;
-  if (t >= S * C) return;
-  int s = t / C;
-  int n = seg_end(seg_off, s, n_total) - seg_begin(seg_off, s);
-  sum[t] = n > 0 ? sum[t] / (float)n : 0.f;
-}
-__global__ void seg_finalize_rstd_kernel(const float* __restrict__ mean, float* __restrict__ var_to_rstd,
-                                         const int* __restrict__ seg_off, int S, int C, float eps,
-                                         float* __restrict__ running_mean, float* __restrict__ running_var,
-                                         float momentum, int n_total) {
-  int t = blockIdx.x * blockDim.x + threadIdx.x;
-  if (t >= S * C) return;
-  int s = t / C;
-  int n = seg_end(seg_off, s, n_total) - seg_begin(seg_off, s);
-  float var = n > 0 ? var_to_rstd[t] / (float)n : 0.f;
-  if (running_mean != nullptr && S == 1) {
-    float unbiased = n > 1 ? var * (float)n / (float)(n - 1) : var;
-    running_mean[t] = (1.f - momentum) * running_mean[t] + momentum * mean[t];
-    running_var[t] = (1.f - momentum) * running_var[t] + momentum * unbiased;
-  }
-  var_to_rstd[t] = rsqrtf(var + eps);
+    part[((long long)blockIdx.x * gridDim.y + s) * C + c] = t;
+  }
+  if (!esb_arrive_last(&counters[s * gridDim.z + blockIdx.z], gridDim.x)) return;
+  const int c0 = blockIdx.z * 32, w = min(32, C - c0);
+  esb_ordered_sum(part + (long long)s * C + c0, gridDim.x, (long long)gridDim.y * C, w, out + s * C + c0, false);
+  const int tid = threadIdx.y * 32 + threadIdx.x;
+  if (tid < w) {
+    const int i = s * C + c0 + tid;
+    const int n = seg_end(seg_off, s, n_total) - seg_begin(seg_off, s);
+    if (MODE == 0) {
+      out[i] = n > 0 ? out[i] / (float)n : 0.f;
+    } else {
+      const float var = n > 0 ? out[i] / (float)n : 0.f;
+      if (running_mean != nullptr && gridDim.y == 1) {
+        const float unbiased = n > 1 ? var * (float)n / (float)(n - 1) : var;
+        running_mean[i] = (1.f - momentum) * running_mean[i] + momentum * mean[i];
+        running_var[i] = (1.f - momentum) * running_var[i] + momentum * unbiased;
+      }
+      out[i] = rsqrtf(var + eps);
+    }
+  }
 }
 
 __device__ __forceinline__ float act_fwd(float z, int act) {
@@ -210,8 +206,9 @@
 template <typename T>
 __global__ void norm_bwd_reduce_kernel(const T* __restrict__ x, const T* __restrict__ y, const T* __restrict__ dy,
                                        const int* __restrict__ seg_off, const float* __restrict__ mean,
-                                       const float* __restrict__ rstd, float* __restrict__ sg, float* __restrict__ sgx,
-                                       int C, int rows_per_block, int act, int n_total) {
+                                       const float* __restrict__ rstd, float* __restrict__ part, unsigned* __restrict__ counters,
+                                       float* __restrict__ sg, float* __restrict__ sgx, int C, int rows_per_block, int act,
+                                       int n_total) {
   __shared__ float red0[8][33];
   __shared__ float red1[8][33];
   const int s = blockIdx.y;
@@ -232,6 +229,7 @@
   red0[threadIdx.y][threadIdx.x] = a0;
   red1[threadIdx.y][threadIdx.x] = a1;
   __syncthreads();
+  const long long width = (long long)gridDim.y * C;
   if (threadIdx.y == 0 && c < C) {
     float t0 = 0.f, t1 = 0.f;
 #pragma unroll
@@ -239,9 +237,13 @@
       t0 += red0[j][threadIdx.x];
       t1 += red1[j][threadIdx.x];
     }
-    sg[((long long)blockIdx.x * gridDim.y + s) * C + c] = t0;
-    sgx[((long long)blockIdx.x * gridDim.y + s) * C + c] = t1;
-  }
+    part[blockIdx.x * width + s * C + c] = t0;
+    part[(gridDim.x + blockIdx.x) * width + s * C + c] = t1;
+  }
+  if (!esb_arrive_last(&counters[s * gridDim.z + blockIdx.z], gridDim.x)) return;
+  const int c0 = blockIdx.z * 32, w = min(32, C - c0);
+  esb_ordered_sum(part + s * C + c0, gridDim.x, width, w, sg + s * C + c0, true);
+  esb_ordered_sum(part + gridDim.x * width + s * C + c0, gridDim.x, width, w, sgx + s * C + c0, true);
 }
 
 template <typename T>
@@ -322,7 +324,8 @@
 }
 
 template <typename T>
-__global__ void bn_stats_kernel(const T* __restrict__ x, long long N, int C, int rows_per_block, float* __restrict__ part) {
+__global__ void bn_stats_kernel(const T* __restrict__ x, long long N, int C, int rows_per_block, float* __restrict__ part,
+                                unsigned* __restrict__ counter, float* __restrict__ stats) {
   extern __shared__ float sh[];
   const int tpr = C / 8;
   const int c = (threadIdx.x % tpr) * 8;
@@ -357,6 +360,8 @@
     for (int r = 0; r < rstep; ++r) t += sh[(2 * r + k) * C + ci];
     part[(long long)blockIdx.x * 2 * C + i] = t;
   }
+  if (!esb_arrive_last(counter, gridDim.x)) return;
+  esb_ordered_sum(part, gridDim.x, 2 * C, 2 * C, stats, false);
 }
 
 template <typename T>
@@ -427,6 +432,13 @@
 
 }
 
+namespace {
+int bn_rows_per_block(long long N) {
+  const long long per = (N + 2 * esb_sm_count() - 1) / (2 * esb_sm_count());
+  return (int)(per < 64 ? 64 : per);
+}
+}
+
 #define DISPATCH_T(dtype, ...)                         \
   if (dtype == ESB_F32) {                              \
     using T = float;                                   \
@@ -461,23 +473,22 @@
   cudaStream_t stream = (cudaStream_t)stream_;
   ESB_CHECK_ARG(S >= 1 && C >= 1, "esb_norm_fwd: bad S/C");
   ESB_CHECK_ARG(seg_off != nullptr || S == 1, "esb_norm_fwd: seg_off may be NULL only for a single segment");
-  ESB_CUDA_CALL(cudaMemsetAsync(mean, 0, sizeof(float) * S * C, stream));
-  ESB_CUDA_CALL(cudaMemsetAsync(rstd, 0, sizeof(float) * S * C, stream));
-  if (N == 0) return ESB_OK;
+  if (N == 0) {
+    ESB_CUDA_CALL(cudaMemsetAsync(mean, 0, sizeof(float) * S * C, stream));
+    ESB_CUDA_CALL(cudaMemsetAsync(rstd, 0, sizeof(float) * S * C, stream));
+    return ESB_OK;
+  }
   const int rpb = 256;
   dim3 grid(esb_div_up(max_seg_rows > 0 ? max_seg_rows : 1, rpb), S, esb_div_up(C, 32)), block(32, 8);
-  int fin = esb_div_up(S * C, 256);
+  const int groups = S * grid.z;
   float* part = nullptr;
-  ESB_CUDA_CALL(esb_scratch_alloc((void**)&part, sizeof(float) * grid.x * S * C, stream));
-  int rc = ESB_OK;
+  unsigned* counters = nullptr;
+  ESB_CUDA_CALL(esb_split_alloc(&part, &counters, (size_t)grid.x * S * C, 2 * groups, stream));
   DISPATCH_T(dtype, {
-    seg_colstat_kernel<T, 0><<<grid, block, 0, stream>>>((const T*)x, seg_off, nullptr, part, C, rpb, (int)N);
-    rc = esb_sum_partial_rows(part, (int)grid.x, (long long)S * C, mean, 0, stream);
-    seg_finalize_mean_kernel<<<fin, 256, 0, stream>>>(mean, seg_off, S, C, (int)N);
-    seg_colstat_kernel<T, 1><<<grid, block, 0, stream>>>((const T*)x, seg_off, mean, part, C, rpb, (int)N);
-    if (rc == ESB_OK) rc = esb_sum_partial_rows(part, (int)grid.x, (long long)S * C, rstd, 0, stream);
-    seg_finalize_rstd_kernel<<<fin, 256, 0, stream>>>(mean, rstd, seg_off, S, C, eps, running_mean, running_var, momentum,
-                                                      (int)N);
+    seg_colstat_kernel<T, 0><<<grid, block, 0, stream>>>((const T*)x, seg_off, nullptr, part, counters, mean, C, rpb, (int)N, eps,
+                                                         nullptr, nullptr, momentum);
+    seg_colstat_kernel<T, 1><<<grid, block, 0, stream>>>((const T*)x, seg_off, mean, part, counters + groups, rstd, C, rpb, (int)N,
+                                                         eps, running_mean, running_var, momentum);
     if (C % 8 == 0)
       norm_apply_vec8_kernel<T><<<esb_div_up(N * (C / 8), 256), 256, 0, stream>>>(
           (const T*)x, (const T*)res, row_seg, mean, rstd, gamma, beta, (T*)y, N * (C / 8), C, act);
@@ -486,7 +497,6 @@
                                                                        gamma, beta, (T*)y, N, C, act);
   });
   ESB_CUDA_CALL(esb_scratch_free(part, stream));
-  if (rc != ESB_OK) return rc;
   ESB_CUDA_LAUNCH_CHECK("esb_norm_fwd");
   return ESB_OK;
 }
@@ -513,15 +523,12 @@
   if (N == 0) return ESB_OK;
   const int rpb = 256;
   dim3 grid(esb_div_up(max_seg_rows > 0 ? max_seg_rows : 1, rpb), S, esb_div_up(C, 32)), block(32, 8);
-  const long long width = (long long)S * C;
   float* part = nullptr;
-  ESB_CUDA_CALL(esb_scratch_alloc((void**)&part, sizeof(float) * 2 * grid.x * width, stream));
-  int rc = ESB_OK;
+  unsigned* counters = nullptr;
+  ESB_CUDA_CALL(esb_split_alloc(&part, &counters, (size_t)2 * grid.x * S * C, S * grid.z, stream));
+  DISPATCH_T(dtype, (norm_bwd_reduce_kernel<T><<<grid, block, 0, stream>>>((const T*)x, (const T*)y, (const T*)dy, seg_off, mean,
+                                                                           rstd, part, counters, sg, sgx, C, rpb, act, (int)N)));
   DISPATCH_T(dtype, {
-    norm_bwd_reduce_kernel<T><<<grid, block, 0, stream>>>((const T*)x, (const T*)y, (const T*)dy, seg_off, mean, rstd,
-                                                          part, part + grid.x * width, C, rpb, act, (int)N);
-    rc = esb_sum_partial_rows(part, (int)grid.x, width, sg, 1, stream);
-    if (rc == ESB_OK) rc = esb_sum_partial_rows(part + grid.x * width, (int)grid.x, width, sgx, 1, stream);
     if (C % 8 == 0)
       norm_bwd_apply_vec8_kernel<T><<<esb_div_up(N * (C / 8), 256), 256, 0, stream>>>(
           (const T*)x, (const T*)y, (const T*)dy, row_seg, seg_off, mean, rstd, gamma, sg, sgx, (T*)dx, (T*)dres, N,
@@ -531,7 +538,6 @@
           (const T*)x, (const T*)y, (const T*)dy, row_seg, seg_off, mean, rstd, gamma, sg, sgx, (T*)dx, (T*)dres, N, C, act);
   });
   ESB_CUDA_CALL(esb_scratch_free(part, stream));
-  if (rc != ESB_OK) return rc;
   ESB_CUDA_LAUNCH_CHECK("esb_norm_bwd");
   return ESB_OK;
 }
@@ -572,20 +578,21 @@
                                        void* y, int dtype, void* stream_) {
   cudaStream_t stream = (cudaStream_t)stream_;
   ESB_CHECK_ARG(C % 8 == 0 && C >= 8 && C <= 2048, "esb_batchnorm_fwd_fused: C must be a multiple of 8 in [8, 2048]");
-  ESB_CUDA_CALL(cudaMemsetAsync(stats, 0, sizeof(float) * 2 * C, stream));
-  if (N == 0) return ESB_OK;
-  long long rpb = (N + 2 * esb_sm_count() - 1) / (2 * esb_sm_count());
-  if (rpb < 64) rpb = 64;
+  if (N == 0) {
+    ESB_CUDA_CALL(cudaMemsetAsync(stats, 0, sizeof(float) * 2 * C, stream));
+    return ESB_OK;
+  }
+  const int rpb = bn_rows_per_block(N);
   const int grid_a = esb_div_up(N, rpb);
   const long long n_vec = N * (C / 8);
   const int rstep = 256 / (C / 8);
   float* part = nullptr;
-  ESB_CUDA_CALL(esb_scratch_alloc((void**)&part, sizeof(float) * 2 * C * grid_a, stream));
-  DISPATCH_T(dtype, (bn_stats_kernel<T><<<grid_a, 256, 2 * rstep * C * sizeof(float), stream>>>((const T*)x, N, C, (int)rpb, part)));
+  unsigned* counter = nullptr;
+  ESB_CUDA_CALL(esb_split_alloc(&part, &counter, (size_t)2 * C * grid_a, 1, stream));
+  DISPATCH_T(dtype, (bn_stats_kernel<T><<<grid_a, 256, 2 * rstep * C * sizeof(float), stream>>>((const T*)x, N, C, rpb, part,
+                                                                                               counter, stats)));
   ESB_CUDA_LAUNCH_CHECK("bn_stats_kernel");
-  int rc = esb_sum_partial_rows(part, grid_a, 2LL * C, stats, 0, stream);
   ESB_CUDA_CALL(esb_scratch_free(part, stream));
-  if (rc != ESB_OK) return rc;
   DISPATCH_T(dtype, (bn_apply_fused_kernel<T><<<esb_div_up(n_vec, 256), 256, 0, stream>>>(
                         (const T*)x, (const T*)res, N, C, gamma, beta, eps, running_mean, running_var, momentum, act, stats,
                         (T*)y)));
```

New measurement: 62.03 (median of 6 runs). +14.7%, better.
